# schmidtjonathan/pnmol-experiments

Measured on AMD Instinct MI355X. Metric: filter steps/sec, 1D heat N=512 nu=2 (white-noise EK1 predict+update), higher is better.
Workload: dtype f64; 1 GPU; 1-D heat equation, N=512 mesh, IWP(nu=2) EK1, Dirichlet, dt=2^-7, one problem per GPU (kappa sweep), D=1536, m=514; steps_in_one_call=4975, valid=True, problems_per_gpu=1

## Files before the change

### include/pnmol_hip.h

```cpp
#ifndef PNMOL_HIP_H
#define PNMOL_HIP_H

#ifdef __cplusplus
extern "C" {
#endif

typedef struct pnmol_ctx pnmol_ctx;
typedef struct pnmol_filter pnmol_filter;
typedef struct pnmol_state pnmol_state;
typedef struct pnmol_samples pnmol_samples;
typedef struct pnmol_bridge pnmol_bridge;

int pnmol_abi_version(void);
int pnmol_device_count(int* count);
int pnmol_ctx_create(int device, pnmol_ctx** out);
int pnmol_ctx_destroy(pnmol_ctx* ctx);
int pnmol_ctx_synchronize(pnmol_ctx* ctx);
const char* pnmol_last_error(pnmol_ctx* ctx);

int pnmol_fd_solve_batched(pnmol_ctx* ctx, const double* gram_nss, const double* lk_ns, const double* llk_n, int N, int s,
                           double* weights_ns, double* uncertainty_n);
int pnmol_cholesky_lower(pnmol_ctx* ctx, const double* A_nn, int n, double* L_nn);

typedef struct pnmol_filter_desc {
    int d;
    int num_derivatives;
    int nB;
    const double* L;
    const double* B;
    const double* E_sqrtm;
    const double* R_sqrtm;
    const double* Gamma;
    int d_state;
    int dtype;
    const double* K;
} pnmol_filter_desc;

int pnmol_filter_create(pnmol_ctx* ctx, const pnmol_filter_desc* desc, pnmol_filter** out);
int pnmol_filter_destroy(pnmol_filter* f);
int pnmol_filter_sweep_layout(const pnmol_filter* f, int* kernel, int* xcd_home);

int pnmol_filter_set_error_model(pnmol_filter* f, double dt, const double* Sq_inv,
                                 const double* Sq_diag);
int pnmol_filter_prepare_error_model(pnmol_filter* f, double dt);

int pnmol_filter_predict_mean(pnmol_filter* f, const pnmol_state* in, double dt, double* m_at_d);
int pnmol_filter_set_operator(pnmol_filter* f, const double* M_dds, const double* shift_d);
int pnmol_filter_set_operator_diagonal(pnmol_filter* f, const double* jdiag_d, const double* shift_d);

int pnmol_state_create(pnmol_filter* f, pnmol_state** out);
int pnmol_state_destroy(pnmol_state* s);
int pnmol_state_clone(const pnmol_state* s, pnmol_state** out);
int pnmol_state_set(pnmol_state* s, double t, const double* mean_nd, const double* cov_DD);
int pnmol_state_set_sqrtm(pnmol_state* s, double t, const double* mean_nd, const double* cov_sqrtm_DD);
int pnmol_state_get_time(const pnmol_state* s, double* t);
int pnmol_state_get_mean(const pnmol_state* s, double* mean_nd);
int pnmol_state_get_cov(const pnmol_state* s, double* cov_DD);
int pnmol_state_get_cov_sqrtm(const pnmol_state* s, double* C_DD);
int pnmol_state_get_marginal_var(const pnmol_state* s, double* var_nd);

typedef struct pnmol_step_out {
    double t_new;
    double diffusion_squared_local;
    double sigma2_whitened;
    double error_sigma2;
    int info;
} pnmol_step_out;

int pnmol_filter_step(pnmol_filter* f, const pnmol_state* in, double dt, pnmol_state* out,
                      pnmol_step_out* info, double* error_estimate_d);

int pnmol_smoother_step(pnmol_filter* f, const pnmol_state* filt_k, const pnmol_state* smooth_next, double dt,
                        pnmol_state* out);

typedef struct pnmol_observe_out {
    double log_likelihood;
    double mahalanobis;
    double logdet;
    int info;
} pnmol_observe_out;
int pnmol_state_observe(pnmol_filter* f, const pnmol_state* in, int q, const double* C_q_ds, const double* y_q,
                        const double* R_sqrtm_qq, pnmol_state* out, pnmol_observe_out* res);

int pnmol_state_predict(pnmol_filter* f, const pnmol_state* in, double dt, pnmol_state* out);
int pnmol_state_predict_marginals(pnmol_filter* f, const pnmol_state* in, int nq, const double* dt_q, double* means_qnd,
                                  double* stds_qnd);
int pnmol_smoother_step_bridge(pnmol_filter* f, const pnmol_state* filt_k, const pnmol_state* smooth_next, double dt,
                               pnmol_state* out, int keep_full, pnmol_bridge** bridge);
int pnmol_bridge_destroy(pnmol_bridge* b);
int pnmol_bridge_get_interval(const pnmol_bridge* b, double* t, double* dt, int* has_full);
int pnmol_bridge_eval(const pnmol_bridge* b, int nq, const double* t_q, double* means_qnd, double* stds_qnd);
int pnmol_bridge_state(const pnmol_bridge* b, const pnmol_state* smooth_k, const pnmol_state* smooth_next, double t,
                       pnmol_state* out);

int pnmol_samples_create(pnmol_filter* f, int num_samples, pnmol_samples** out);
int pnmol_samples_destroy(pnmol_samples* x);
int pnmol_samples_draw(pnmol_samples* x, const pnmol_state* s, const double* xi_SD, unsigned long long seed,
                       unsigned long long step_index, double scale);
int pnmol_samples_step_back(pnmol_samples* x, const pnmol_state* filt_k, double dt, const double* xi_S2D,
                            unsigned long long seed, unsigned long long step_index, double scale);
int pnmol_samples_interpolate(pnmol_samples* out, const pnmol_samples* left, const pnmol_samples* right, double t,
                              const double* xi_SD, unsigned long long seed, unsigned long long step_index, double scale);
int pnmol_samples_clone(const pnmol_samples* x, pnmol_samples** out);
int pnmol_samples_get(const pnmol_samples* x, double* x_Snd);
int pnmol_samples_get_time(const pnmol_samples* x, double* t);
int pnmol_sample_noise(pnmol_ctx* ctx, unsigned long long seed, unsigned long long step_index, int rows, int cols, double* out);

int pnmol_filter_steps(pnmol_filter* f, pnmol_state* s, int k, double dt, double* means_kd,
                       double* stds_kd, pnmol_step_out* info_k);

int pnmol_filter_steps_begin(pnmol_filter* f, pnmol_state* s, int k, double dt);
int pnmol_filter_steps_end(pnmol_filter* f, pnmol_state* s, double* means_kd, double* stds_kd,
                           pnmol_step_out* info_k);

int pnmol_filter_prepare_steps(pnmol_filter* f, pnmol_state* s, int k, double dt);

int pnmol_filter_last_steps_ms(pnmol_filter* f, float* ms);

int pnmol_filter_debug_read(pnmol_filter* f, int which, double* dst, long count);
int pnmol_filter_debug_poison(pnmol_filter* f);
int pnmol_filter_dims(const pnmol_filter* f, int* d, int* n, int* m, int* dp, int* mp);

#ifdef __cplusplus
}
#endif
#endif
```

### pnmol-experiments_amd/csrc/pnmol_hip.hip

```cpp
#include <hip/hip_runtime.h>

#include <algorithm>
#include <chrono>
#include <cmath>
#include <cstdio>
#include <cstdlib>
#include <cstring>
#include <string>
#include <utility>
#include <atomic>
#include <vector>

#include "pnmol_hip.h"
#include "pnmol_internal.hpp"

namespace {

constexpr int TLD = NB + 1;
typedef double d4 __attribute__((ext_vector_type(4)));

struct MeasModel {
    const int* ell_col;
    const double* ell_val;
    int w, d, m, dp, mp;
// ... 760 lines not shown
    for (int s = 0; s < NB / 4; ++s) {
        const double b = sI[(wc * 16 + fr) * TLD + 4 * s + fk];
        li = __builtin_amdgcn_mfma_f64_16x16x4f64(sA[(wr * 16 + fr) * TLD + 4 * s + fk], b, li, 0, 0, 0);
        if (trailing) lk = __builtin_amdgcn_mfma_f64_16x16x4f64(sB[(wr * 16 + fr) * TLD + 4 * s + fk], b, lk, 0, 0, 0);
    }
    __syncthreads();
#pragma unroll
    for (int r = 0; r < 4; ++r) {
        const int row = wr * 16 + fk + 4 * r, col = wc * 16 + fr;
        sA[row * TLD + col] = li[r];
        if (trailing) sB[row * TLD + col] = lk[r];
        if (c == 0) F[((long)I * NB + row) * ld + (long)j * NB + col] = li[r];
    }
    if (!trailing) return;
    __syncthreads();

#pragma unroll
    for (int s = 0; s < NB / 4; ++s)
        acc = __builtin_amdgcn_mfma_f64_16x16x4f64(-sA[(wr * 16 + fr) * TLD + 4 * s + fk],
                                                   sB[(wc * 16 + fr) * TLD + 4 * s + fk], acc, 0, 0, 0);
    if (!(blockIdx.x == 0 && c == 0)) {
#pragma unroll
        for (int r = 0; r < 4; ++r) gt[(long)(wr * 16 + fk + 4 * r) * ld + wc * 16 + fr] = acc[r];
        return;
    }
    __syncthreads();
#pragma unroll
    for (int r = 0; r < 4; ++r) sA[(wr * 16 + fk + 4 * r) * TLD + wc * 16 + fr] = acc[r];
    if (tid < NB) dlp->flag[tid] = 0;
    __syncthreads();
    if (w < 2)
        diag2w_from_lds(sA, F + ((long)(j + 1) * NB) * ld + (long)(j + 1) * NB, ld, Linv + (long)(j + 1) * NB * NB, w, l,
                        info_base + (*ctr - 1), (j + 1) * NB, sdiag + (j + 1) * NB, sdiag[ld], dlp);
}

constexpr int SWEEP_SPIN_LIMIT = 1 << 18;
#ifdef PNMOL_SWEEP_STAMP
__device__ long long pnmol_sweep_stamp[512][8];
#define SWEEP_STAMP(slot) do { if (tid == 0 && L.stamp_id < 256) pnmol_sweep_stamp[L.stamp_id][slot] = wall_clock64(); } while (0)
#define SWEEP_STAMP_L(slot) do { if (l == 0 && L.stamp_id < 256) pnmol_sweep_stamp[L.stamp_id][slot] = wall_clock64(); } while (0)
#ifndef PNMOL_SWEEP_TRACE_WG
#define PNMOL_SWEEP_TRACE_WG 16
#endif
#define SWEEP_TRACE(j, slot) do { if (tid == 0 && L.stamp_id == PNMOL_SWEEP_TRACE_WG) pnmol_sweep_stamp[256 + (j)][slot] = wall_clock64(); } while (0)
#define SWEEP_TRACE_W2(j, slot) do { if (w == 2 && l == 0 && L.stamp_id == PNMOL_SWEEP_TRACE_WG) pnmol_sweep_stamp[320 + (j)][slot] = wall_clock64(); } while (0)
#define SWEEP_TRACE_VM(j, slot) do { asm volatile("s_waitcnt vmcnt(0)" ::: "memory"); SWEEP_TRACE(j, slot); } while (0)
#define CHAIN_TRACE(J, slot) do { if (tid == 0) pnmol_sweep_stamp[384 + (J)][slot] = wall_clock64(); } while (0)
#define CHAIN_TRACE_W(J, slot, wave) do { if (l == 0 && w == (wave)) pnmol_sweep_stamp[384 + (J)][slot] = wall_clock64(); } while (0)
#define CHAIN_TRACE_CLK(J, slot) do { if (tid == 0) pnmol_sweep_stamp[384 + (J)][slot] = clock64(); } while (0)
#define PNMOL_DD_DBG 1
#define DD_TRACE(j, slot) do { if (tid == 0 && pair == 60) pnmol_sweep_stamp[448 + (j)][slot] = wall_clock64(); } while (0)
#else
#define DD_TRACE(j, slot) do {} while (0)
#define CHAIN_TRACE_CLK(J, slot) do {} while (0)
#define SWEEP_TRACE_VM(j, slot) do {} while (0)
#define SWEEP_TRACE_W2(j, slot) do {} while (0)
#define CHAIN_TRACE(J, slot) do {} while (0)
#define CHAIN_TRACE_W(J, slot, wave) do {} while (0)
#define SWEEP_TRACE(j, slot) do {} while (0)
#define SWEEP_STAMP(slot) do {} while (0)
#define SWEEP_STAMP_L(slot) do {} while (0)
#endif

struct SweepLds {
    double sS[2][NB * TLD];
    double sX[NB * TLD];
    double sP[4][NB * TLD];
    double sd[NB];
    double red[4];
    int seen[3];
    int dead, pub;
    int pubcnt;
    int rdiag, rnew, rcol, rzb;
    int stamp_id;
    Diag4Lds d4;
};
struct ChainLds {
    double sX[NB * TLD];
    double sLinv[NB * TLD];
    double sFeedS[NB * TLD];
    double sFeedD[NB * TLD];
    double sd[2][NB];
    double red[4];
    Diag4Lds d4[2];
};

__device__ __forceinline__ int flag_ld(const int* p) {
    return __hip_atomic_load(p, __ATOMIC_RELAXED, __HIP_MEMORY_SCOPE_AGENT);
}
__device__ __forceinline__ void flag_st(int* p, int v) {
    __hip_atomic_store(p, v, __ATOMIC_RELAXED, __HIP_MEMORY_SCOPE_AGENT);
}
__device__ __forceinline__ void wt_st(double* p, double v) {
    __hip_atomic_store(p, v, __ATOMIC_RELAXED, __HIP_MEMORY_SCOPE_AGENT);
}
typedef int v4i_t __attribute__((ext_vector_type(4)));
__device__ __forceinline__ __amdgpu_buffer_rsrc_t wt_rsrc(const void* base) {
    return __builtin_amdgcn_make_buffer_rsrc(const_cast<void*>(base), 0, 0x7ffffffc, 0x00020000);
}
template <int AUX = 16 >
__device__ __forceinline__ void wt_st2(__amdgpu_buffer_rsrc_t r, unsigned byte_off, double a, double b) {
    const v4i_t v = {__double2loint(a), __double2hiint(a), __double2loint(b), __double2hiint(b)};
    __builtin_amdgcn_raw_buffer_store_b128(v, r, byte_off, 0, AUX);
}
template <int NE, int AUX = 16>
__device__ __forceinline__ void wt_rows_from_lds(__amdgpu_buffer_rsrc_t r, unsigned org, long ld, const double* s, int row0, int l) {
#pragma unroll
    for (int e = 0; e < NE; ++e) {
        const int idx = l + 64 * e, row = row0 + (idx >> 4), c2 = 2 * (idx & 15);
        wt_st2<AUX>(r, org + (unsigned)((row * ld + c2) * 8), s[row * TLD + c2], s[row * TLD + c2 + 1]);
    }
}
struct TileRegs {
    double v[16];
};
__device__ __forceinline__ void tile_regs_from_lds(TileRegs& t, const double* s, int l) {
#pragma unroll
    for (int e = 0; e < 8; ++e) {
        const int idx = l + 64 * e, row = idx >> 4, c2 = 2 * (idx & 15);
        t.v[2 * e] = s[row * TLD + c2];
        t.v[2 * e + 1] = s[row * TLD + c2 + 1];
    }
}
template <int AUX>
__device__ __forceinline__ void tile_regs_store(const TileRegs& t, __amdgpu_buffer_rsrc_t r, unsigned org, long ld, int l) {
#pragma unroll
    for (int e = 0; e < 8; ++e) {
        const int idx = l + 64 * e, row = idx >> 4, c2 = 2 * (idx & 15);
        wt_st2<AUX>(r, org + (unsigned)((row * ld + c2) * 8), t.v[2 * e], t.v[2 * e + 1]);
    }
}
__device__ __forceinline__ void l2_flag_st(__amdgpu_buffer_rsrc_t rflags, int word, int v) {
    __builtin_amdgcn_raw_buffer_store_b32(v, rflags, (unsigned)word * 4u, 0, 0);
}
__device__ __forceinline__ void sc1_tile_to_lds(double* s, __amdgpu_buffer_rsrc_t r, unsigned org, int l) {
    v4i_t v[8];
#pragma unroll
    for (int e = 0; e < 8; ++e) {
        const int idx = l + 64 * e;
        v[e] = __builtin_amdgcn_raw_buffer_load_b128(r, org + (unsigned)(((idx >> 4) * NB + 2 * (idx & 15)) * 8), 0, 16 );
    }
#pragma unroll
    for (int e = 0; e < 8; ++e) {
        const int idx = l + 64 * e, row = idx >> 4, c2 = 2 * (idx & 15);
        s[row * TLD + c2] = __hiloint2double(v[e][1], v[e][0]);
        s[row * TLD + c2 + 1] = __hiloint2double(v[e][3], v[e][2]);
    }
}
__device__ __forceinline__ void drain_vmem() { asm volatile("s_waitcnt vmcnt(0) lgkmcnt(0)" ::: "memory"); }

struct SweepSeen {
    int rowj, rown, diag;
};

__device__ __forceinline__ void sweep_wait(SweepLds* L, const int* frow, const int* fdiag, int* fabort, int j, int jn_ok,
                                           int need_rowj, int need_rown, bool need_diag, SweepSeen& sn, int tid) {
    if (sn.rowj >= need_rowj && sn.rown >= need_rown && (!need_diag || sn.diag)) return;
    __syncthreads();
    if (tid == 0) {
        int r = sn.rowj, rn = sn.rown, d = sn.diag;
        if (!L->dead) {
            for (int spins = 0;; ++spins) {
                r = flag_ld(frow + j);
                rn = jn_ok ? flag_ld(frow + j + 1) : (1 << 30);
                d = flag_ld(fdiag + j);
                if (r >= need_rowj && rn >= need_rown && (!need_diag || d)) break;
// ... 127 lines not shown
        for (int o = 32; o > 0; o >>= 1) {
            a[q] += __shfl_xor(a[q], o);
            b[q] += __shfl_xor(b[q], o);
        }
        const long row = r0 + q;
        if (l == 0 && row < r1) {
            if (row < Dp) {
                va.mout[row] = va.mpred[row] - a[q];
            } else if (row < Dp + mp) {
                const long k = row - Dp;
                va.part[k] = va.r[k] * va.r[k];
                va.part[mp + k] = a[q] * a[q];
                va.part[2 * mp + k] = va.z[k] * b[q];
            }
        }
    }
}

__device__ __forceinline__ void ksplit_partial(double* sp, const double* __restrict__ Abase, const double* __restrict__ Bbase,
                                               int k0, int k1, long ld, int w, int l) {
    const int fr = l & 15, fk = l >> 4;
    d4 p00 = {0, 0, 0, 0}, p01 = p00, p10 = p00, p11 = p00;
    FragTile a0, b0, a1, b1;
    auto mfma32 = [&](const FragTile& a, const FragTile& b) {
#pragma unroll
        for (int s = 0; s < 8; ++s) {
            p00 = __builtin_amdgcn_mfma_f64_16x16x4f64(a.lo.v[s], b.lo.v[s], p00, 0, 0, 0);
            p01 = __builtin_amdgcn_mfma_f64_16x16x4f64(a.lo.v[s], b.hi.v[s], p01, 0, 0, 0);
            p10 = __builtin_amdgcn_mfma_f64_16x16x4f64(a.hi.v[s], b.lo.v[s], p10, 0, 0, 0);
            p11 = __builtin_amdgcn_mfma_f64_16x16x4f64(a.hi.v[s], b.hi.v[s], p11, 0, 0, 0);
        }
    };
    const int nk = (k0 + w < k1) ? (k1 - k0 - w + 3) >> 2 : 0;
    if (nk > 0) {
        tile_ld(a0, Abase + (long)(k0 + w) * NB, ld);
        tile_ld(b0, Bbase + (long)(k0 + w) * NB, ld);
    }
    int t = 0;
    for (; t + 2 <= nk; t += 2) {
        const long ka = k0 + w + 4 * (t + 1), kb = k0 + w + 4 * (t + 2 < nk ? t + 2 : nk - 1);
        tile_ld(a1, Abase + ka * NB, ld);
        tile_ld(b1, Bbase + ka * NB, ld);
        mfma32(a0, b0);
        tile_ld(a0, Abase + kb * NB, ld);
        tile_ld(b0, Bbase + kb * NB, ld);
        mfma32(a1, b1);
    }
    if (t < nk) mfma32(a0, b0);
#pragma unroll
    for (int r = 0; r < 4; ++r) {
        sp[(fk + 4 * r) * TLD + fr] = p00[r];
        sp[(fk + 4 * r) * TLD + 16 + fr] = p01[r];
        sp[(16 + fk + 4 * r) * TLD + fr] = p10[r];
        sp[(16 + fk + 4 * r) * TLD + 16 + fr] = p11[r];
    }
}

constexpr int HELP_KMAX = 8;
__device__ __forceinline__ int helper_share(int H, int t, int CB) {
    const int h = CB - 1 - H;
    if (h >= H - 1 || t < h + 3) return 0;
    const int kh = t - 1 - HELP_KMAX;
    return kh > 0 ? kh : 0;
}

__device__ __forceinline__ void vecops_rows4(const VecArgs& va, const double* __restrict__ W, int mp, long Dp, long r0,
                                             long r1, int l) {
    vecops_rowsR<4>(va, W, mp, Dp, r0, r1, l);
}

struct DowndateArgs {
    const void* Ppred;
    void* Pout;
    double* var;
    int dp;
    int vrows;
    VecArgs va;
    void* Pnext;
    const double* Kg;
    const int* last_ctr;
    double A1[MAXN * MAXN], Q1[MAXN * MAXN];
    int p32;
    int last_ksteps;
};

template <typename PT>
struct AccOf;
template <>
struct AccOf<double> {
    typedef d4 type;
    static __device__ __forceinline__ d4 mfma_neg(double a, double b, d4 c) {
        return __builtin_amdgcn_mfma_f64_16x16x4f64(-a, b, c, 0, 0, 0);
    }
    static __device__ __forceinline__ int row(int fk, int r) { return fk + 4 * r; }
};
template <>
struct AccOf<float> {
    typedef float type __attribute__((ext_vector_type(4)));
    static __device__ __forceinline__ type mfma_neg(double a, double b, type c) {
        return __builtin_amdgcn_mfma_f32_16x16x4f32(-(float)a, (float)b, c, 0, 0, 0);
    }
    static __device__ __forceinline__ int row(int fk, int r) { return 4 * fk + r; }
};

#ifdef PNMOL_DD_DBG
__device__ __forceinline__ void pnmol_dd_avail_dbg(int j, int avail, bool loaded) { pnmol_sweep_stamp[448 + j][3] = avail; pnmol_sweep_stamp[448 + j][4] = loaded; }
#else
__device__ __forceinline__ void pnmol_dd_avail_dbg(int, int, bool) {}
#endif
template <int N, typename PT, bool SHORT_LAST>
__device__ __forceinline__ void sweep_downdate_body(SweepLds& L, const DowndateArgs& dd, const double* F, int ld, int CB,
                                                    int RBS, const int* frow, int* fabort, int* info, int pair, int tid,
                                                    int l, int w, int slot) {
    const int fr = l & 15, fk = l >> 4, qr = w >> 1, qc = w & 1;
    const int T32 = dd.dp / NB;
    int J = (int)((sqrt(8.0 * pair + 1.0) - 1.0) * 0.5);
    while ((J + 1) * (J + 2) / 2 <= pair) ++J;
    while (J * (J + 1) / 2 > pair) --J;
    const int K = pair - J * (J + 1) / 2;
    const long Dp = (long)N * dd.dp;
    const double* W = F + (long)ld * ld;
    typedef typename AccOf<PT>::type acc_t;
    const PT* Ppred = static_cast<const PT*>(dd.Ppred);
    acc_t acc[N][N];
#pragma unroll
    for (int a = 0; a < N; ++a)
#pragma unroll
        for (int b = 0; b < N; ++b)
#pragma unroll
            for (int r = 0; r < 4; ++r)
                acc[a][b][r] = Ppred[((long)a * dd.dp + J * NB + qr * 16 + AccOf<PT>::row(fk, r)) * Dp + (long)b * dd.dp + K * NB + qc * 16 + fr];
    acc_t kjk = {0, 0, 0, 0};
    if (dd.Pnext) {
#pragma unroll
        for (int r = 0; r < 4; ++r) kjk[r] = (PT)dd.Kg[(long)(J * NB + qr * 16 + AccOf<PT>::row(fk, r)) * dd.dp + K * NB + qc * 16 + fr];
    }
    int avail = 0;
    auto wait_for = [&](int j) {
        if (j < avail) return;
        __syncthreads();
        if (w == 0) {
            int mn = 0;
            if (!L.dead) {
                for (int spins = 0;; ++spins) {
                    int v = 1 << 30;
                    if (l < 2 * N) {
                        const int a = l >> 1, tile = (l & 1) ? K : J;
                        v = flag_ld(frow + RBS + a * T32 + tile);
                    }
#pragma unroll
                    for (int o = 32; o > 0; o >>= 1) v = min(v, __shfl_xor(v, o));
                    mn = v;
                    if (mn > j) break;
                    if (spins > SWEEP_SPIN_LIMIT || flag_ld(fabort)) {
                        if (l == 0) {
                            L.dead = 1;
                            flag_st(fabort, 1);
                        }
                        mn = 1 << 30;
                        break;
                    }
                    __builtin_amdgcn_s_sleep(4);
                }
            } else {
                mn = 1 << 30;
            }
            if (l == 0) L.seen[0] = mn;
        }
        __syncthreads();
        avail = L.seen[0];
    };
    auto load_panel = [&](int j, Frag8 (&fa)[N], Frag8 (&fb)[N]) {
#pragma unroll
        for (int a = 0; a < N; ++a) {
            frag_ld(fa[a], W + ((long)a * dd.dp + J * NB + qr * 16 + fr) * ld + (long)j * NB + 8 * fk);
            frag_ld(fb[a], W + ((long)a * dd.dp + K * NB + qc * 16 + fr) * ld + (long)j * NB + 8 * fk);
        }
    };
    auto panel = [&](int j, bool loaded, Frag8 (&fa)[N], Frag8 (&fb)[N], Frag8 (&na)[N], Frag8 (&nb)[N]) {
        DD_TRACE(j, 0);
        if (!loaded) {
            wait_for(j);
            DD_TRACE(j, 1);
            load_panel(j, fa, fb);
        }
        const bool next = j + 1 < CB && j + 1 < avail;
        if (next) load_panel(j + 1, na, nb);
        const int smax = (SHORT_LAST && j + 1 == CB && dd.last_ksteps > 0) ? dd.last_ksteps : 8;
#pragma unroll
        for (int s = 0; s < 8; ++s)
            if (!SHORT_LAST || s < smax) {
#pragma unroll
                for (int a = 0; a < N; ++a)
#pragma unroll
                    for (int b = 0; b < N; ++b)
                        acc[a][b] = AccOf<PT>::mfma_neg(fa[a].v[s], fb[b].v[s], acc[a][b]);
            }
        DD_TRACE(j, 2);
#ifdef PNMOL_SWEEP_STAMP
        if (tid == 0 && pair == 60) pnmol_dd_avail_dbg(j, avail, loaded);
#endif
        return next;
    };
    if constexpr (SHORT_LAST) {
        (void)panel;
        (void)wait_for;
        bool wdead = false;
        int* relay = &L.seen[0];
        auto poll_min = [&]() {
            int v = 1 << 30;
            if (l < 2 * N) {
                const int a = l >> 1, tile = (l & 1) ? K : J;
                v = flag_ld(frow + RBS + a * T32 + tile);
            }
            return v;
        };
        auto reduce_min = [&](int v) {
#pragma unroll
            for (int o = 32; o > 0; o >>= 1) v = min(v, __shfl_xor(v, o));
            return v;
        };
        auto publish = [&](int v) {
            if (l == 0) __hip_atomic_store(relay, v, __ATOMIC_RELAXED, __HIP_MEMORY_SCOPE_WORKGROUP);
        };
        auto known = [&]() { return __hip_atomic_load(relay, __ATOMIC_RELAXED, __HIP_MEMORY_SCOPE_WORKGROUP); };
        auto wave_wait = [&](int j) {
            if (wdead) return;
            if (w == 0) {
                for (int spins = 0;; ++spins) {
                    const int v = reduce_min(poll_min());
                    if (v > j) {
                        publish(v);
                        return;
                    }
                    if (spins > SWEEP_SPIN_LIMIT || ((spins & 63) == 63 && flag_ld(fabort))) {
                        wdead = true;
                        flag_st(fabort, 1);
                        publish(1 << 30);
                        return;
                    }
                    __builtin_amdgcn_s_sleep(4);
                }
            } else {
                int v;
                while ((v = known()) <= j) __builtin_amdgcn_s_sleep(2);
                if (v == (1 << 30)) wdead = true;
            }
        };
        auto block = [&](int j, bool have, Frag8 (&fa)[N], Frag8 (&fb)[N], Frag8 (&na)[N], Frag8 (&nb)[N]) {
            DD_TRACE(j, 0);
            if (!have) {
                wave_wait(j);
                DD_TRACE(j, 1);
                load_panel(j, fa, fb);
            }
            const int pv = (w == 0 && j + 1 < CB) ? poll_min() : 0;
            const int smax = (j + 1 == CB && dd.last_ksteps > 0) ? dd.last_ksteps : 8;
            bool next = false;
#pragma unroll
            for (int s = 0; s < 8; ++s) {
                if (s == 2) {
                    if (w == 0 && j + 1 < CB && !wdead) {
                        const int v = reduce_min(pv);
                        if (v > known()) publish(v);
                    }
                    const int kv = known();
                    next = (j + 1 < CB) && !wdead && kv > j + 1 && kv != (1 << 30);
                    if (next) load_panel(j + 1, na, nb);
                }
                if (s < smax) {
#pragma unroll
                    for (int a = 0; a < N; ++a)
#pragma unroll
                        for (int b = 0; b < N; ++b)
                            acc[a][b] = AccOf<PT>::mfma_neg(fa[a].v[s], fb[b].v[s], acc[a][b]);
                }
            }
            DD_TRACE(j, 2);
            return next;
        };
        Frag8 fa0[N], fb0[N], fa1[N], fb1[N];
        bool have = false;
        for (int j = 0; j < CB; j += 2) {
            have = block(j, have, fa0, fb0, fa1, fb1);
            if (j + 1 < CB) have = block(j + 1, have, fa1, fb1, fa0, fb0);
        }
        if (wdead && l == 0) atomicMin(info, -2);
        __syncthreads();
    } else {
        for (int j = 0; j < CB; ++j) {
            wait_for(j);
            Frag8 fa[N], fb[N];
            load_panel(j, fa, fb);
#pragma unroll
            for (int s = 0; s < 8; ++s)
#pragma unroll
                for (int a = 0; a < N; ++a)
#pragma unroll
                    for (int b = 0; b < N; ++b)
                        acc[a][b] = AccOf<PT>::mfma_neg(fa[a].v[s], fb[b].v[s], acc[a][b]);
        }
    }
    SWEEP_STAMP(1);
    PT* stg = reinterpret_cast<PT*>(L.sP[w]);
    const bool write_p = dd.Pnext == nullptr || (slot + 1 == *dd.last_ctr);
    auto put_block = [&](PT* dst, const acc_t& v, long row0, long col0, bool mirror) {
#pragma unroll
        for (int r = 0; r < 4; ++r) {
            dst[(row0 + AccOf<PT>::row(fk, r)) * Dp + col0 + fr] = v[r];
            if (J != K && mirror) stg[AccOf<PT>::row(fk, r) * 17 + fr] = v[r];
        }
        if (J != K && mirror) {
            __builtin_amdgcn_wave_barrier();
#pragma unroll
            for (int r = 0; r < 4; ++r)
                dst[(col0 + fk + 4 * r) * Dp + row0 + fr] = stg[fr * 17 + fk + 4 * r];
            __builtin_amdgcn_wave_barrier();
        }
    };
#pragma unroll
    for (int a = 0; a < N; ++a) {
        const long row0 = (long)a * dd.dp + J * NB + qr * 16;
        if (J == K && qr == qc) {
#pragma unroll
            for (int r = 0; r < 4; ++r)
                if (AccOf<PT>::row(fk, r) == fr) dd.var[row0 + fr] = acc[a][a][r];
        }
        if (write_p) {
#pragma unroll
            for (int b = 0; b < N; ++b) put_block(static_cast<PT*>(dd.Pout), acc[a][b], row0, (long)b * dd.dp + K * NB + qc * 16, true);
        }
    }
    if (dd.Pnext) {
        acc_t T[N][N];
#pragma unroll
        for (int a = 0; a < N; ++a)
#pragma unroll
            for (int e = 0; e < N; ++e) {
                acc_t t = {0, 0, 0, 0};
#pragma unroll
                for (int q = 0; q < N; ++q) t += (PT)dd.A1[a * MAXN + q] * acc[q][e];
                T[a][e] = t;
            }
#pragma unroll
        for (int a = 0; a < N; ++a)
#pragma unroll
            for (int b = 0; b < N; ++b) {
                acc_t pn = (PT)dd.Q1[a * MAXN + b] * kjk;
#pragma unroll
                for (int e = 0; e < N; ++e) pn += T[a][e] * (PT)dd.A1[b * MAXN + e];
                put_block(static_cast<PT*>(dd.Pnext), pn, (long)a * dd.dp + J * NB + qr * 16, (long)b * dd.dp + K * NB + qc * 16, a < 2);
            }
    }
    SWEEP_STAMP(2);
    {
        const int RBW = (int)(Dp / NB);
        const long row_lo = (long)pair * dd.vrows, row_hi = min(row_lo + dd.vrows, Dp + (long)ld);
        __syncthreads();
        if (tid == 0 && !L.dead && row_lo < row_hi) {
            for (long rb = row_lo / NB; rb <= (row_hi - 1) / NB; ++rb) {
                const int need = rb < RBW ? RBS + (int)rb : RBS + RBW + 1 + (int)(rb - RBW);
                for (int spins = 0;; ++spins) {
                    if (flag_ld(frow + need) >= CB && flag_ld(frow + RBS + RBW) >= CB) break;
                    if (spins > SWEEP_SPIN_LIMIT || flag_ld(fabort)) {
                        L.dead = 1;
                        flag_st(fabort, 1);
                        break;
                    }
                    __builtin_amdgcn_s_sleep(2);
                }
                if (L.dead) break;
            }
        }
        __syncthreads();
        for (long rg = row_lo + 4 * w; rg < row_hi; rg += 16) vecops_rows4(dd.va, W, ld, Dp, rg, min(rg + 4, row_hi), l);
    }
    if (tid == 0 && L.dead) atomicMin(info, -2);
    SWEEP_STAMP(5);
}

template <int N, bool SHORT_LAST = false>
__device__ __forceinline__ void sweep_downdate_role(SweepLds& L, const DowndateArgs& dd, const double* F, int ld, int CB,
                                                    int RBS, const int* frow, int* fabort, int* info, int pair, int tid,
                                                    int l, int w, int slot) {
    if (dd.p32) sweep_downdate_body<N, float, SHORT_LAST>(L, dd, F, ld, CB, RBS, frow, fabort, info, pair, tid, l, w, slot);
    else sweep_downdate_body<N, double, SHORT_LAST>(L, dd, F, ld, CB, RBS, frow, fabort, info, pair, tid, l, w, slot);
}

template <int N, bool FUSED, bool CHAINHELP = FUSED>
__global__ __launch_bounds__(256) void k_sweep(const double* __restrict__ G, double* F, double* Linv, int ld, int CB,
                                               int RT, int* flags, int* info_base, const int* __restrict__ ctr,
                                               DowndateArgs dd, int* claim, double* hs_scratch, int lenient, int wskip) {
    __shared__ __attribute__((aligned(16))) SweepLds L;
    const int tid = threadIdx.x, l = tid & 63, w = __builtin_amdgcn_readfirstlane(tid >> 6);
    const int wr = w >> 1, wc = w & 1, fr = l & 15, fk = l >> 4;
    int I = blockIdx.x;
#ifdef PNMOL_SWEEP_STAMP
    if (tid == 0) L.stamp_id = blockIdx.x;
#endif
    {
        const int zb = RT - CB - 1;
        if (wskip) {
            if (I >= CB) I = zb + (I - CB);
        } else if (I >= CB && I <= zb) {
            I = (I == CB) ? zb : I - 1;
        }
    }
    const bool chain = I < CB;
    int* frow = flags;
    int* fdiag = flags + RT;
    int* fabort = flags + RT + CB;
    int* info = info_base + (*ctr - 1);
    if constexpr (FUSED) {
        if (I >= RT) {
            if (tid == 0) {
                L.dead = 0;
                __builtin_amdgcn_fence(__ATOMIC_ACQUIRE, "agent");
            }
            __syncthreads();
            SWEEP_STAMP(0);
            sweep_downdate_role<N>(L, dd, F, ld, CB, CB, frow, fabort, info, I - RT, tid, l, w, *ctr - 1);
            return;
        }
    }

    double smax = 0.0;
    if (chain) {
        for (int e = tid; e < ld; e += 256) smax = fmax(smax, fabs(G[(long)e * ld + e]));
#pragma unroll
        for (int o = 32; o > 0; o >>= 1) smax = fmax(smax, __shfl_xor(smax, o));
        if (l == 0) L.red[w] = smax;
        if (tid < NB) L.sd[tid] = G[(long)(I * NB + tid) * ld + I * NB + tid];
    }
    if (tid < 16) L.d4.flagA[tid] = 0;
    if (tid == 0) {
        L.dead = 0, L.pub = 0;
        __builtin_amdgcn_fence(__ATOMIC_ACQUIRE, "agent");
    }
    __syncthreads();
    SWEEP_STAMP(0);
    if (chain) smax = fmax(fmax(L.red[0], L.red[1]), fmax(L.red[2], L.red[3]));
    if (lenient) smax = __builtin_inf();

    const long rowC = (long)I * NB + wr * 16 + fk;
    const int colC = wc * 16 + fr;
    const int offC = (wr * 16 + fk) * TLD + colC;
    const double* Xown = F + ((long)I * NB + fr) * ld + 8 * fk;
    d4 accD = {0, 0, 0, 0};
    if (chain) {
#pragma unroll
        for (int r = 0; r < 4; ++r) {
            const int rl = wr * 16 + fk + 4 * r, cl = colC;
            accD[r] = -G[((long)I * NB + (rl >= cl ? rl : cl)) * ld + (long)I * NB + (rl >= cl ? cl : rl)];
        }
    }

    const int nsteps = chain ? I : CB;
    d4 gnext = {0, 0, 0, 0};
    if (nsteps > 0) {
#pragma unroll
        for (int r = 0; r < 4; ++r) gnext[r] = G[(rowC + 4 * r) * ld + colC];
    }
    SweepSeen sn{0, 0, 0};
    for (int j = 0; j < nsteps; ++j) {
        const int jn_ok = (j + 1 < CB);
        d4 acc = gnext;
        SWEEP_TRACE(j, 0);
        if (j >= 2) {
#pragma unroll
// ... 117 lines not shown
            }
        }
        if (tid == 0 && L.dead) atomicMin(info, -2);
        SWEEP_STAMP(5);
        return;
    }

    SWEEP_STAMP(3);
    if (w == 2 && I > 0) {
        drain_vmem();
        if (l == 0) flag_st(frow + I, I);
        __hip_atomic_store(&L.pub, 1, __ATOMIC_RELAXED, __HIP_MEMORY_SCOPE_WORKGROUP);
    }
    diag4_factor<true>(accD, &L.d4, w, l, F + ((long)I * NB) * ld + (long)I * NB, ld, Linv + (long)I * NB * NB, info, I * NB,
                       L.sd, smax, nullptr, pivot_tolerance(lenient));
    if (w == 1) {
        drain_vmem();
        if (I > 0) {
            int spins = 0;
            while (__hip_atomic_load(&L.pub, __ATOMIC_RELAXED, __HIP_MEMORY_SCOPE_WORKGROUP) == 0 && ++spins < (1 << 24))
                __builtin_amdgcn_s_sleep(1);
        }
        if (l == 0) flag_st(fdiag + I, 1);
        SWEEP_STAMP_L(4);
    }
    if (tid == 0 && L.dead) atomicMin(info, -2);
    if constexpr (CHAINHELP) {
        const int H = CB - 1 - I;
        if (I < H - 1) {
            const double* Xh = F + ((long)H * NB + fr) * ld + 8 * fk;
            for (int t = I + 3; t < H; ++t) {
                const int kh = helper_share(H, t, CB);
                if (kh <= 0) continue;
                int* cl = claim + (long)H * CB + t;
                __syncthreads();
                if (tid == 0) {
                    int got = 0;
                    for (int spins = 0;; ++spins) {
                        if (flag_ld(cl) != 0) break;
                        if (flag_ld(frow + H) >= kh && flag_ld(frow + t) >= kh) {
                            got = atomicCAS(cl, 0, 1) == 0;
                            break;
                        }
                        if (spins > 4096 || flag_ld(fabort)) {
                            got = -1;
                            break;
                        }
                        __builtin_amdgcn_s_sleep(8);
                    }
                    L.seen[0] = got;
                }
                __syncthreads();
                const int got = L.seen[0];
                if (got < 0) break;
                if (got == 0) continue;
                ksplit_partial(L.sP[w], Xh, F + ((long)t * NB + fr) * ld + 8 * fk, 0, kh, ld, w, l);
                __syncthreads();
                double* hs = hs_scratch + ((long)H * CB + t) * NB * NB;
#pragma unroll
                for (int r = 0; r < 4; ++r)
                    wt_st(&hs[(wr * 16 + fk + 4 * r) * NB + colC],
                          (L.sP[0][offC + 4 * r * TLD] + L.sP[1][offC + 4 * r * TLD]) +
                              (L.sP[2][offC + 4 * r * TLD] + L.sP[3][offC + 4 * r * TLD]));
                drain_vmem();
                __syncthreads();
                if (tid == 0) flag_st(cl, 2);
            }
        }
    }
}

constexpr int RL_REP = 8;
constexpr int S_SPLIT_FROM = 11, S_SPLIT_H = 9;
__host__ __device__ inline int s_split_count(int CB, bool xl) { return (xl && CB > S_SPLIT_FROM) ? CB - S_SPLIT_FROM : 0; }
constexpr int W_SPLIT_H = 11;
#ifndef PNMOL_W_SPLIT
#define PNMOL_W_SPLIT 0
#endif
__host__ __device__ inline int w_split_count(int RT, int CB) {
    const int RBW = RT - 2 * CB - 1;
    return (PNMOL_W_SPLIT && RBW > 0 && CB > W_SPLIT_H + 1) ? RBW : 0;
}
struct RlFlags {
    int frow, fabort, fxcc, ffeed, fdiag, fnew, fcol, fdiagL, fnewL, frowL, CBp, total;
};
__host__ __device__ inline RlFlags rl_flags(int RT, int CB) {
    const int RTp = (RT + 31) / 32 * 32, CBp = (CB + 31) / 32 * 32;
    RlFlags f;
    f.CBp = CBp;
    f.frow = 0;
    f.fabort = RTp;
    f.fxcc = RTp + 16;
    f.ffeed = RTp + 32;
    f.fdiag = f.ffeed + CBp;
    f.fnew = f.fdiag + RL_REP * CBp;
    f.fcol = f.fnew + RL_REP * CBp;
    f.fdiagL = f.fcol + RL_REP * CBp;
    f.fnewL = f.fdiagL + CBp;
    f.frowL = f.fnewL + CBp;
    f.total = f.frowL + CBp;
    return f;
}
__device__ __forceinline__ int xcc_id() { return __builtin_amdgcn_s_getreg((3 << 11) | 20) & 15; }
struct WaveWait {
    bool dead;
};
__device__ __forceinline__ void wave_wait_ge(const int* p, int need, int* fabort, WaveWait& ww) {
    if (ww.dead) return;
    for (int spins = 0;; ++spins) {
        if (flag_ld(p) >= need) return;
        if (spins > SWEEP_SPIN_LIMIT || ((spins & 63) == 63 && flag_ld(fabort))) {
            ww.dead = true;
            flag_st(fabort, 1);
            return;
        }
        __builtin_amdgcn_s_sleep(1);
    }
}
__device__ __forceinline__ void relay_wait_ge(const int* p, int need, int* relay, int tag, int* fabort, WaveWait& ww, int w) {
    if (w == 0) {
        wave_wait_ge(p, need, fabort, ww);
        __hip_atomic_store(relay, ww.dead ? (1 << 30) : tag, __ATOMIC_RELAXED, __HIP_MEMORY_SCOPE_WORKGROUP);
    } else {
        int v;
        while ((v = __hip_atomic_load(relay, __ATOMIC_RELAXED, __HIP_MEMORY_SCOPE_WORKGROUP)) < tag) __builtin_amdgcn_s_sleep(1);
        if (v == (1 << 30)) ww.dead = true;
    }
    asm volatile("" ::: "memory");
}

template <class Need>
__device__ __forceinline__ void relay_progress(const int* p, int cnt, Need need, int want, int& known, int* relay, int* fabort,
                                               WaveWait& ww, int w, int l) {
    if (w == 0) {
        if (known < want) {
            for (int spins = 0; !ww.dead; ++spins) {
                const int v = l < cnt ? flag_ld(p + l) : 0;
                const unsigned long long ok = __ballot(l < cnt && v >= need(l));
                known = __builtin_amdgcn_readfirstlane((int)__builtin_ctzll(~ok));
                if (known >= want) break;
                if (spins > SWEEP_SPIN_LIMIT || ((spins & 63) == 63 && flag_ld(fabort))) {
                    ww.dead = true;
                    flag_st(fabort, 1);
                    break;
                }
                __builtin_amdgcn_s_sleep(1);
            }
            __hip_atomic_store(relay, ww.dead ? (1 << 30) : known, __ATOMIC_RELAXED, __HIP_MEMORY_SCOPE_WORKGROUP);
        }
    } else {
        int v;
        while ((v = __hip_atomic_load(relay, __ATOMIC_RELAXED, __HIP_MEMORY_SCOPE_WORKGROUP)) < want) __builtin_amdgcn_s_sleep(1);
        if (v == (1 << 30)) ww.dead = true;
    }
    asm volatile("" ::: "memory");
}
__device__ __forceinline__ void relay_progress_min(const int* p, int cnt, int want, int& known, int* relay, int* fabort,
                                                   WaveWait& ww, int w, int l) {
    if (w == 0) {
        if (known < want) {
            for (int spins = 0; !ww.dead; ++spins) {
                int v = l < cnt ? flag_ld(p + l) : (1 << 29);
#pragma unroll
                for (int o = 32; o > 0; o >>= 1) v = min(v, __shfl_xor(v, o));
                known = __builtin_amdgcn_readfirstlane(v);
                if (known >= want) break;
                if (spins > SWEEP_SPIN_LIMIT || ((spins & 63) == 63 && flag_ld(fabort))) {
                    ww.dead = true;
                    flag_st(fabort, 1);
                    break;
                }
                __builtin_amdgcn_s_sleep(1);
            }
            __hip_atomic_store(relay, ww.dead ? (1 << 30) : known, __ATOMIC_RELAXED, __HIP_MEMORY_SCOPE_WORKGROUP);
        }
    } else {
        int v;
        while ((v = __hip_atomic_load(relay, __ATOMIC_RELAXED, __HIP_MEMORY_SCOPE_WORKGROUP)) < want) __builtin_amdgcn_s_sleep(1);
        if (v == (1 << 30)) ww.dead = true;
    }
    asm volatile("" ::: "memory");
}
__device__ __forceinline__ void relay_wait_range_ge(const int* p, int cnt, int need, int* relay, int tag, int* fabort,
                                                    WaveWait& ww, int w, int l) {
    if (w == 0) {
        if (!ww.dead) {
            for (int spins = 0;; ++spins) {
                const int v = l < cnt ? flag_ld(p + l) : need;
                if (__all(v >= need)) break;
                if (spins > SWEEP_SPIN_LIMIT || ((spins & 63) == 63 && flag_ld(fabort))) {
                    ww.dead = true;
                    flag_st(fabort, 1);
                    break;
                }
                __builtin_amdgcn_s_sleep(1);
            }
        }
        __hip_atomic_store(relay, ww.dead ? (1 << 30) : tag, __ATOMIC_RELAXED, __HIP_MEMORY_SCOPE_WORKGROUP);
    } else {
        int v;
        while ((v = __hip_atomic_load(relay, __ATOMIC_RELAXED, __HIP_MEMORY_SCOPE_WORKGROUP)) < tag) __builtin_amdgcn_s_sleep(1);
        if (v == (1 << 30)) ww.dead = true;
    }
    asm volatile("" ::: "memory");
}

__device__ __forceinline__ void rows8_dot(const double* __restrict__ base, long row0, int mp, const double* __restrict__ vec,
                                          double (&out)[8], int l) {
#pragma unroll
    for (int q = 0; q < 8; ++q) out[q] = 0.0;
    for (int i0 = l; i0 < mp; i0 += 256) {
        double wv[8][4], xv[4];
#pragma unroll
        for (int t = 0; t < 4; ++t) {
            const int i = i0 + 64 * t;
            const int ii = i < mp ? i : mp - 1;
            xv[t] = i < mp ? vec[ii] : 0.0;
#pragma unroll
            for (int q = 0; q < 8; ++q) wv[q][t] = base[(row0 + q) * mp + ii];
        }
#pragma unroll
        for (int t = 0; t < 4; ++t)
#pragma unroll
            for (int q = 0; q < 8; ++q) out[q] += wv[q][t] * xv[t];
    }
#pragma unroll
    for (int q = 0; q < 8; ++q)
#pragma unroll
        for (int o = 32; o > 0; o >>= 1) out[q] += __shfl_xor(out[q], o);
}
__device__ __forceinline__ void vecops_rows8(const VecArgs& va, const double* __restrict__ W, int mp, long Dp, long r0,
                                             const double* bq , int l) {
    double a[8];
    if (r0 < Dp) {
        rows8_dot(W, r0, mp, va.r, a, l);
        if (l < 8) {
            double mine = a[0];
#pragma unroll
            for (int q = 1; q < 8; ++q) mine = (l == q) ? a[q] : mine;
            va.mout[r0 + l] = va.mpred[r0 + l] - mine;
        }
    } else {
        const long k0 = r0 - Dp;
        rows8_dot(va.LinvT, k0, mp, va.z, a, l);
        if (l < 8) {
            double mine = a[0];
#pragma unroll
            for (int q = 1; q < 8; ++q) mine = (l == q) ? a[q] : mine;
            const double bm = bq[l];
            const long k = k0 + l;
            va.part[k] = va.r[k] * va.r[k];
            va.part[mp + k] = mine * mine;
            va.part[2 * mp + k] = va.z[k] * bm;
        }
    }
}
__device__ __forceinline__ void mfma_result_guard() {
#ifdef PNMOL_NO_MFMA_GUARD
    return;
#endif
    __builtin_amdgcn_sched_barrier(0);
    asm volatile("s_nop 15\n\ts_nop 7" ::: "memory");
    __builtin_amdgcn_sched_barrier(0);
}
constexpr int RING = 3;
constexpr int RING_LINV = RING, RING_NEWEST = RING + 1;
__device__ __forceinline__ void lds_dma16(const double* gsrc, unsigned lds_dst) {
    unsigned keep;
    asm volatile("s_mov_b32 %0, m0\n\ts_mov_b32 m0, %2\n\ts_nop 0\n\tglobal_load_lds_dwordx4 %1, off\n\ts_mov_b32 m0, %0"
                 : "=&s"(keep) : "v"(gsrc), "s"(lds_dst) : "memory");
}
__device__ __forceinline__ void ring_fill(const double* tile, const int (&off)[4], unsigned slot) {
#pragma unroll
    for (int c = 0; c < 4; ++c) lds_dma16(tile + off[c], slot + 1024u * c);
}
__device__ __forceinline__ void ring_wait(int tiles_behind) {
    switch (tiles_behind) {
        case 0: asm volatile("s_waitcnt vmcnt(0)" ::: "memory"); break;
        case 1: asm volatile("s_waitcnt vmcnt(4)" ::: "memory"); break;
        case 2: asm volatile("s_waitcnt vmcnt(8)" ::: "memory"); break;
        default: asm volatile("s_waitcnt vmcnt(12)" ::: "memory"); break;
    }
}
__device__ __forceinline__ void ring_frag(Frag8& f, const double* slot, int fr, int fk) {
#pragma unroll
    for (int e = 0; e < 4; ++e) {
        const double2 t = *reinterpret_cast<const double2*>(slot + (fr * 16 + ((4 * fk + e) ^ fr)) * 2);
        f.v[2 * e] = t.x;
        f.v[2 * e + 1] = t.y;
    }
}

template <bool XL>
__device__ __forceinline__ void sweep_chain_role(ChainLds& C, const double* __restrict__ G, double* F, double* Linv, int ld,
                                                 int CB, int* flags, const RlFlags& fl, int* info,
                                                 double* feed, int lenient, int tid, int l, int w) {
    int* fdiag_all = flags + fl.fdiag;
    int* fnew_all = flags + fl.fnew;
    const int CBp = fl.CBp;
    int* ffeed = flags + fl.ffeed;
    int* fabort = flags + fl.fabort;
    const int wr = w >> 1, wc = w & 1, fr = l & 15, fk = l >> 4;
    const int offC = (wr * 16 + fk) * TLD + wc * 16 + fr;
    const __amdgpu_buffer_rsrc_t rF = wt_rsrc(F), rlinv = wt_rsrc(Linv), rfeed = wt_rsrc(feed), rflags = wt_rsrc(flags);
    if (XL && tid == 0) flag_st(flags + fl.fxcc, 1 + xcc_id());
    WaveWait ww{false};
    double smax = 0.0;
    for (int e = tid; e < ld; e += 256) smax = fmax(smax, fabs(G[(long)e * ld + e]));
#pragma unroll
    for (int o = 32; o > 0; o >>= 1) smax = fmax(smax, __shfl_xor(smax, o));
    if (l == 0) C.red[w] = smax;
    if (tid < NB) C.sd[0][tid] = G[(long)tid * ld + tid];
    if (tid < 16) C.d4[0].flagA[tid] = 0, C.d4[1].flagA[tid] = 0;
    for (int e = tid; e < 16 * 16; e += 256) C.sLinv[(e >> 4) * TLD + 16 + (e & 15)] = 0.0;
    if (tid == 0) __builtin_amdgcn_fence(__ATOMIC_ACQUIRE, "agent");
    __syncthreads();
    smax = lenient ? __builtin_inf() : fmax(fmax(C.red[0], C.red[1]), fmax(C.red[2], C.red[3]));
    const double pivtol = pivot_tolerance(lenient);
    d4 accD;
#pragma unroll
    for (int r = 0; r < 4; ++r) {
        const int rl = wr * 16 + fk + 4 * r, cl = wc * 16 + fr;
        accD[r] = -G[(long)(rl >= cl ? rl : cl) * ld + (rl >= cl ? cl : rl)];
    }
    for (int J = 0; J < CB; ++J) {
        Diag4Lds* dl = &C.d4[J & 1];
        CHAIN_TRACE(J, 0);
        CHAIN_TRACE_CLK(J, 4);
        if (w == 2 && J > 0)
            diag4_output(&C.d4[(J - 1) & 1], l, F + ((long)(J - 1) * NB) * ld + (long)(J - 1) * NB, ld, info, (J - 1) * NB,
                         C.sd[(J - 1) & 1], smax, pivtol);
        diag4_factor<true, true, false, false>(accD, dl, w, l, F + ((long)J * NB) * ld + (long)J * NB, ld,
                                               Linv + (long)J * NB * NB, info, J * NB, C.sd[J & 1], smax, C.sLinv, pivtol);
        CHAIN_TRACE_W(J, 1, 3);
        CHAIN_TRACE_W(J, 6, 1);
        if (XL && w == 1 && J + 1 < CB) {
            TileRegs t1;
            tile_regs_from_lds(t1, C.sLinv, l);
            tile_regs_store<0>(t1, rlinv, (unsigned)(J * NB * NB * 8), NB, l);
            drain_vmem();
            if (l == 0) l2_flag_st(rflags, fl.fdiagL + J, 1);
        }
        if (J + 1 == CB) {
            __syncthreads();
            if (w == 2) {
                wt_rows_from_lds<8>(rlinv, (unsigned)(J * NB * NB * 8), NB, C.sLinv, 0, l);
                drain_vmem();
                if (l < RL_REP) flag_st(fdiag_all + l * CBp + J, 1);
                if (XL && l == 0) l2_flag_st(rflags, fl.fdiagL + J, 1);
            }
            break;
        }
        if (w == 0 || w == 2) {
            wave_wait_ge(ffeed + J + 1, 1, fabort, ww);
            sc1_tile_to_lds((w == 2) ? C.sFeedD : C.sFeedS, rfeed, (unsigned)((2 * (J + 1) + (w == 2 ? 1 : 0)) * NB * NB * 8), l);
            if (w == 2 && l < NB) C.sd[(J + 1) & 1][l] = G[(long)((J + 1) * NB + l) * ld + (J + 1) * NB + l];
        }
        __syncthreads();
        CHAIN_TRACE(J, 2);
        if (tid < 16) C.d4[(J + 1) & 1].flagA[tid] = 0;
        TileRegs tl;
        if (w == 2) {
            if constexpr (XL) {
                tile_regs_from_lds(tl, C.sLinv, l);
            } else {
                wt_rows_from_lds<8>(rlinv, (unsigned)(J * NB * NB * 8), NB, C.sLinv, 0, l);
            }
        }
        d4 x = {0, 0, 0, 0};
#pragma unroll
        for (int s = 0; s < 8; ++s)
            x = __builtin_amdgcn_mfma_f64_16x16x4f64(C.sFeedS[(wr * 16 + fr) * TLD + 8 * fk + s],
                                                     C.sLinv[(wc * 16 + fr) * TLD + 8 * fk + s], x, 0, 0, 0);
#pragma unroll
        for (int r = 0; r < 4; ++r) C.sX[offC + 4 * r * TLD] = x[r];
#pragma unroll
        for (int r = 0; r < 4; ++r) accD[r] = C.sFeedD[offC + 4 * r * TLD];
        __syncthreads();
        CHAIN_TRACE(J, 3);
        if (w == 2) {
            if constexpr (!XL) {
                drain_vmem();
                if (l < RL_REP) flag_st(fdiag_all + l * CBp + J, 1);
            }
        }
#pragma unroll
        for (int s = 0; s < 8; ++s)
            accD = __builtin_amdgcn_mfma_f64_16x16x4f64(C.sX[(wr * 16 + fr) * TLD + 8 * fk + s],
                                                        C.sX[(wc * 16 + fr) * TLD + 8 * fk + s], accD, 0, 0, 0);
        if (w == 2) {
            const unsigned orgX = (unsigned)((((long)(J + 1) * NB) * ld + (long)J * NB) * 8);
            if constexpr (XL) {
                TileRegs tx;
                tile_regs_from_lds(tx, C.sX, l);
                tile_regs_store<0>(tx, rF, orgX, ld, l);
                drain_vmem();
                if (l == 0) l2_flag_st(rflags, fl.fnewL + J, 1);
                tile_regs_store<16>(tl, rlinv, (unsigned)(J * NB * NB * 8), NB, l);
                tile_regs_store<16>(tx, rF, orgX, ld, l);
                drain_vmem();
                if (l < RL_REP) flag_st(fdiag_all + l * CBp + J, 1);
                if (l < RL_REP) flag_st(fnew_all + l * CBp + J, 1);
            } else {
                wt_rows_from_lds<8>(rF, orgX, ld, C.sX, 0, l);
                drain_vmem();
                if (l < RL_REP) flag_st(fnew_all + l * CBp + J, 1);
            }
        }
    }
    if (w == 2)
        diag4_output(&C.d4[(CB - 1) & 1], l, F + ((long)(CB - 1) * NB) * ld + (long)(CB - 1) * NB, ld, info, (CB - 1) * NB,
                     C.sd[(CB - 1) & 1], smax, pivtol);
    if (l == 0 && ww.dead) atomicMin(info, -2);
}

template <int N, bool FUSED, int MAXT, bool XL>
__global__ __launch_bounds__(256) void k_sweep_rl(const double* __restrict__ G, double* F, double* Linv, int ld, int CB,
                                                  int RT, int* flags, int* info_base, const int* __restrict__ ctr,
                                                  DowndateArgs dd, double* feed, int lenient, int home) {
    __shared__ __attribute__((aligned(16))) union {
        SweepLds L;
        ChainLds C;
    } lds;
    SweepLds& L = lds.L;
    __shared__ __attribute__((aligned(16))) double bulk_ring[4][RING + 2][16 * NB];
    const int tid = threadIdx.x, l = tid & 63, w = __builtin_amdgcn_readfirstlane(tid >> 6);
    const int wr = w >> 1, wc = w & 1, fr = l & 15, fk = l >> 4;
    const RlFlags fl = rl_flags(RT, CB);
    int* frow = flags + fl.frow;
    int* fabort = flags + fl.fabort;
    int* ffeed = flags + fl.ffeed;
    const int* fdiag = flags + fl.fdiag + (blockIdx.x % RL_REP) * fl.CBp;
    const int* fnew = flags + fl.fnew + (blockIdx.x % RL_REP) * fl.CBp;
    const int* fcol = flags + fl.fcol + (blockIdx.x % RL_REP) * fl.CBp;
    int* info = info_base + (*ctr - 1);
    const int bx = XL ? (int)blockIdx.x - home : (int)blockIdx.x;
    if (bx < 0) return;
    if (bx == 0) {
        sweep_chain_role<XL>(lds.C, G, F, Linv, ld, CB, flags, fl, info, feed, lenient, tid, l, w);
        return;
    }
    int I, part = 0;
    if constexpr (XL) {
        const int nsplit = s_split_count(CB, true);
        const int b = bx, nslot = 8 * (CB - 1 + nsplit) + 1;
        if (b < nslot) {
            if (b % 8 != 0) return;
            const int sidx = b / 8;
            if (sidx < CB) {
                I = sidx;
                part = (nsplit > 0 && I >= S_SPLIT_FROM) ? 1 : 0;
            } else {
                I = S_SPLIT_FROM + (sidx - CB);
                part = 2;
            }
        } else {
            if (b % 8 == 0) return;
            const int q = b - nslot;
            I = CB + q - (q + 1) / 8;
        }
    } else {
        I = bx - 1;
    }
#ifdef PNMOL_SWEEP_STAMP
    if (tid == 0) L.stamp_id = part == 1 ? 200 + I : 1 + I;
#endif
    {
        const int zb = RT - CB - 1;
        if (I >= CB && I <= zb) I = (I == CB) ? zb : I - 1;
    }
    const int nwsplit = w_split_count(RT, CB);
    if (I >= RT && I < RT + nwsplit) {
        I = CB + (I - RT);
        part = 2;
    } else if (I >= RT) {
        I -= nwsplit;
        if constexpr (FUSED) {
            if (tid == 0) {
                L.dead = 0, L.seen[0] = 0;
                __builtin_amdgcn_fence(__ATOMIC_ACQUIRE, "agent");
            }
            __syncthreads();
            SWEEP_STAMP(0);
            sweep_downdate_role<N, true>(L, dd, F, ld, CB, CB, frow, fabort, info, I - RT, tid, l, w, *ctr - 1);
        }
        return;
    } else if (nwsplit > 0 && I >= CB && I < RT - CB - 1) {
        part = 1;
    }
    const bool chain = I < CB;
    if (chain && I == 0) return;
    if (tid == 0) {
        L.dead = 0, L.pub = 0, L.pubcnt = part == 2 ? 4 * (I < CB ? S_SPLIT_H : W_SPLIT_H) : 0, L.rdiag = 0, L.rnew = 0, L.rcol = 0, L.rzb = 0;
        L.seen[0] = 0;
        __builtin_amdgcn_fence(__ATOMIC_ACQUIRE, "agent");
    }
    __syncthreads();
    SWEEP_STAMP(0);

    const long rowC = (long)I * NB + wr * 16 + fk;
    const int colC = wc * 16 + fr;
    const int offC = (wr * 16 + fk) * TLD + colC;
    const bool feeds = chain && part != 1;
    const int hsplit = chain ? S_SPLIT_H : W_SPLIT_H;
    const int t0 = part == 2 ? hsplit : 0;
    const int last = part == 1 ? hsplit - 1 : (chain ? I - 2 : CB - 1);
    const int ntiles = part == 1 ? hsplit : (chain ? I : CB);
    d4 n[MAXT];
#pragma unroll
    for (int t = 0; t < MAXT; ++t)
        if (t0 + t < ntiles) {
#pragma unroll
            for (int r = 0; r < 4; ++r) n[t][r] = -G[(rowC + 4 * r) * ld + (long)(t0 + t) * NB + colC];
        }
    d4 accD = {0, 0, 0, 0};
    if (feeds) {
#pragma unroll
        for (int r = 0; r < 4; ++r) {
            const int rl = wr * 16 + fk + 4 * r, cl = colC;
            accD[r] = -G[((long)I * NB + (rl >= cl ? rl : cl)) * ld + (long)I * NB + (rl >= cl ? cl : rl)];
        }
    }
    WaveWait ww{false};
    int known_diag = 0, known_new = 0, known_col = 0;
    const __amdgpu_buffer_rsrc_t rF = wt_rsrc(F), rfeed = wt_rsrc(feed), rflags = wt_rsrc(flags);
    const double* ringw = &bulk_ring[w][0][0];
    const unsigned ring0 = __builtin_amdgcn_readfirstlane((unsigned)(size_t)ringw);
    int roff[4], roffL[4];
#pragma unroll
    for (int c = 0; c < 4; ++c) {
        const int row = 4 * c + (l >> 4);
        roff[c] = (wc * 16 + row) * ld + 2 * ((l & 15) ^ row);
        roffL[c] = (wc * 16 + row) * NB + 2 * ((l & 15) ^ row);
    }
#ifndef PNMOL_EAGER_TILES
#define PNMOL_EAGER_TILES 6
#endif
    constexpr int EAGER_TILES = PNMOL_EAGER_TILES;
    bool pre_b0 = false;
    if constexpr (FUSED) {
        const int RBW = RT - 2 * CB - 1, zb = CB + RBW;
        if (!chain && I > zb) {
            double bq[8] = {0, 0, 0, 0, 0, 0, 0, 0};
            if (dd.va.Sqinv != nullptr) rows8_dot(dd.va.Sqinv, (long)(I - zb - 1) * NB + 8 * w, ld, dd.va.z, bq, l);
            if (l == 0) {
#pragma unroll
                for (int q = 0; q < 8; ++q) L.sd[8 * w + q] = bq[q];
            }
        }
    }
    bool local = false;
    if constexpr (XL) {
        if (chain) {
            if (tid == 0) {
                int v = 0;
                for (int spins = 0; spins < 4096 && (v = flag_ld(flags + fl.fxcc)) == 0; ++spins) __builtin_amdgcn_s_sleep(1);
                L.seen[0] = (v == 1 + xcc_id());
            }
            __syncthreads();
            local = L.seen[0] != 0;
            if (local) fdiag = flags + fl.fdiagL, fnew = flags + fl.fnewL;
        }
    }
    Frag8 ax;
    auto flag_tile = [&](int t) {
        drain_vmem();
        int lastw = 0;
        if (l == 0) lastw = __hip_atomic_fetch_add(&L.pubcnt, 1, __ATOMIC_RELAXED, __HIP_MEMORY_SCOPE_WORKGROUP) == 4 * t + 3;
        if (__builtin_amdgcn_readfirstlane(lastw)) {
            if (l == 0) flag_st(frow + I, t + 1);
            if (XL && chain && l == 0) {
                if (local) l2_flag_st(rflags, fl.frowL + I, t + 1);
                else flag_st(flags + fl.frowL + I, t + 1);
            }
            if (chain && l < RL_REP)
                __hip_atomic_fetch_add(flags + fl.fcol + l * fl.CBp + t, 1, __ATOMIC_RELAXED, __HIP_MEMORY_SCOPE_AGENT);
        }
    };
    if (part == 2) {
        const int* fsrc = (XL && local) ? flags + fl.frowL : frow;
        for (int k = 0; k < t0; ++k) {
            if (chain) {
                if (k + 1 < t0) {
                    relay_progress_min(fsrc + t0, I - t0 + 1, k + 1, known_col, &L.rcol, fabort, ww, w, l);
                } else {
                    relay_progress(fnew, CB - 1, [](int) { return 1; }, t0, known_new, &L.rnew, fabort, ww, w, l);
                    relay_progress_min(fsrc + t0 + 1, I - t0, t0, known_col, &L.rcol, fabort, ww, w, l);
                }
            } else {
                relay_progress(fnew, CB - 1, [](int) { return 1; }, k + 1, known_new, &L.rnew, fabort, ww, w, l);
                relay_progress(fcol, CB - 1, [CB](int q) { return CB - 2 - q; }, k + 1, known_col, &L.rcol, fabort, ww, w, l);
                relay_wait_ge(frow + I, k + 1, &L.rzb, k + 1, fabort, ww, w);
            }
            Frag8 bx;
            frag_ld(ax, F + ((long)I * NB + wr * 16 + fr) * ld + (long)k * NB + 8 * fk);
            frag_ld(bx, F + ((long)I * NB + wc * 16 + fr) * ld + (long)k * NB + 8 * fk);
#pragma unroll
            for (int u0 = 0; u0 < 8; u0 += 4) {
                Frag8 b[4];
#pragma unroll
                for (int q = 0; q < 4; ++q)
                    if (t0 + u0 + q < ntiles)
                        frag_ld(b[q], F + ((long)(t0 + u0 + q) * NB + wc * 16 + fr) * ld + (long)k * NB + 8 * fk);
#pragma unroll
                for (int q = 0; q < 4; ++q)
                    if (t0 + u0 + q < ntiles) {
#pragma unroll
                        for (int s = 0; s < 8; ++s)
                            n[u0 + q] = __builtin_amdgcn_mfma_f64_16x16x4f64(ax.v[s], b[q].v[s], n[u0 + q], 0, 0, 0);
                    }
            }
            if (chain) {
#pragma unroll
                for (int s = 0; s < 8; ++s) accD = __builtin_amdgcn_mfma_f64_16x16x4f64(ax.v[s], bx.v[s], accD, 0, 0, 0);
            }
            mfma_result_guard();
        }
    }
    const bool lastlocal = feeds && XL && local;
#pragma unroll
    for (int r = 0; r < 4; ++r) L.sS[t0 & 1][offC + 4 * r * TLD] = -n[0][r];
    __syncthreads();
    bool pre_l = false;
    for (int j = t0; j <= last; ++j) {
        const double* sS = L.sS[j & 1];
        SWEEP_TRACE(j, 0);
        relay_progress(fdiag, CB, [](int) { return 1; }, j + 1, known_diag, &L.rdiag, fabort, ww, w, l);
        SWEEP_TRACE(j, 5);
        Frag8 bl;
        if (pre_l) {
            ring_wait(0);
            ring_frag(bl, ringw + 512 * RING_LINV, fr, fk);
        } else {
            frag_ld(bl, Linv + (long)j * NB * NB + (wc * 16 + fr) * NB + 8 * fk);
        }
        d4 x = {0, 0, 0, 0};
#pragma unroll
        for (int s = 0; s < 8; ++s)
            x = __builtin_amdgcn_mfma_f64_16x16x4f64(sS[(wr * 16 + fr) * TLD + 8 * fk + s], bl.v[s], x, 0, 0, 0);
        double* sXj = (j & 1) ? L.sP[0] : L.sX;
#pragma unroll
        for (int r = 0; r < 4; ++r) sXj[offC + 4 * r * TLD] = x[r];
        __syncthreads();
        SWEEP_TRACE(j, 3);
        const bool llast = lastlocal && j == last;
        const unsigned orgX = (unsigned)((((long)I * NB) * ld + (long)j * NB) * 8);
        if (llast) wt_rows_from_lds<2, 0>(rF, orgX, ld, sXj, 8 * w, l);
        else wt_rows_from_lds<2>(rF, orgX, ld, sXj, 8 * w, l);
        if (feeds) {
#pragma unroll
            for (int s = 0; s < 8; ++s)
                accD = __builtin_amdgcn_mfma_f64_16x16x4f64(sXj[(wr * 16 + fr) * TLD + 8 * fk + s],
                                                            sXj[(wc * 16 + fr) * TLD + 8 * fk + s], accD, 0, 0, 0);
            mfma_result_guard();
        }
        const int cnt = ntiles - 1 - j;
        pre_l = false;
        if (cnt > 0) {
#pragma unroll
            for (int s = 0; s < 8; ++s) ax.v[s] = sXj[(wr * 16 + fr) * TLD + 8 * fk + s];
            relay_progress(fnew, CB - 1, [](int) { return 1; }, j + 1, known_new, &L.rnew, fabort, ww, w, l);
            if (llast) {
                drain_vmem();
                int lastw = 0;
                if (l == 0) lastw = __hip_atomic_fetch_add(&L.pub, 1, __ATOMIC_RELAXED, __HIP_MEMORY_SCOPE_WORKGROUP) == 3;
                if (__builtin_amdgcn_readfirstlane(lastw) && l == 0) l2_flag_st(rflags, fl.frowL + I, j + 1);
            } else if (chain) {
                flag_tile(j);
            }
            if (chain) {
                if (cnt > 1)
                    relay_progress_min((XL && local ? flags + fl.frowL : frow) + j + 2, cnt - 1, j + 1, known_col, &L.rcol, fabort, ww, w, l);
            } else {
                relay_progress(fcol, CB - 1, [CB](int k) { return CB - 2 - k; }, j + 1, known_col, &L.rcol, fabort, ww, w, l);
            }
            SWEEP_TRACE(j, 1);
            const double* Lt = F + (long)j * NB + (long)(j + 1) * NB * ld;
#pragma unroll
            for (int r = 0; r < RING; ++r)
                if (r < cnt) ring_fill(Lt + (long)r * NB * ld, roff, ring0 + 4096u * r);
            if (!chain) {
                const int seen = __builtin_amdgcn_readfirstlane(__hip_atomic_load(&L.rdiag, __ATOMIC_RELAXED, __HIP_MEMORY_SCOPE_WORKGROUP));
                if (seen >= j + 2 && seen != (1 << 30)) {
                    ring_fill(Linv + (long)(j + 1) * NB * NB, roffL, ring0 + 4096u * RING_LINV);
                    pre_l = true;
                }
            }
            if (!chain) flag_tile(j);
            else ring_wait(0);
            Frag8 b[2];
            ring_frag(b[0], ringw, fr, fk);
#pragma unroll
            for (int u = 1; u < MAXT; ++u) {
                if (u <= cnt) {
                    const int k = u - 1;
                    __builtin_amdgcn_s_waitcnt(0xc07f);
                    asm volatile("" ::: "memory");
                    if (k + RING < cnt) ring_fill(Lt + (long)(k + RING) * NB * ld, roff, ring0 + 4096u * (k % RING));
                    d4 a = __builtin_amdgcn_mfma_f64_16x16x4f64(ax.v[0], b[k & 1].v[0], n[u], 0, 0, 0);
                    __builtin_amdgcn_sched_barrier(0);
                    if (k + 1 < cnt) {
                        const int behind = (k + RING < cnt ? k + RING : cnt - 1) - (k + 1);
                        ring_wait(behind < RING - 1 ? behind : RING - 1);
                        ring_frag(b[(k + 1) & 1], ringw + 512 * ((k + 1) % RING), fr, fk);
                    }
                    __builtin_amdgcn_sched_barrier(0);
#pragma unroll
                    for (int s = 1; s < 8; ++s)
                        a = __builtin_amdgcn_mfma_f64_16x16x4f64(ax.v[s], b[k & 1].v[s], a, 0, 0, 0);
                    n[u - 1] = a;
                } else {
                    mfma_result_guard();
                    break;
                }
            }
            mfma_result_guard();
            SWEEP_TRACE(j, 4);
            if (!(feeds && j == last)) {
#pragma unroll
                for (int r = 0; r < 4; ++r) L.sS[(j + 1) & 1][offC + 4 * r * TLD] = -n[0][r];
                __syncthreads();
            }
        }
        SWEEP_TRACE(j, 6);
    }
    if (feeds) {
        const int j = I - 1;
#pragma unroll
        for (int r = 0; r < 4; ++r) {
            L.sS[0][offC + 4 * r * TLD] = -n[0][r];
            L.sS[1][offC + 4 * r * TLD] = accD[r];
        }
        __syncthreads();
        if (XL && local) {
            wt_rows_from_lds<2, 0>(rfeed, (unsigned)((2 * I) * NB * NB * 8), NB, L.sS[0], 8 * w, l);
            wt_rows_from_lds<2, 0>(rfeed, (unsigned)((2 * I + 1) * NB * NB * 8), NB, L.sS[1], 8 * w, l);
        } else {
            wt_rows_from_lds<2>(rfeed, (unsigned)((2 * I) * NB * NB * 8), NB, L.sS[0], 8 * w, l);
            wt_rows_from_lds<2>(rfeed, (unsigned)((2 * I + 1) * NB * NB * 8), NB, L.sS[1], 8 * w, l);
        }
        SWEEP_TRACE(j, 2);
        drain_vmem();
        SWEEP_TRACE(j, 3);
        __syncthreads();
        if (tid == 0) {
            if (XL && local) l2_flag_st(rflags, fl.ffeed + I, 1);
            else flag_st(ffeed + I, 1);
        }
        SWEEP_TRACE(j, 4);
        SWEEP_STAMP(1);
        if (last >= 0 && lastlocal) {
            const double* sXl = (last & 1) ? L.sP[0] : L.sX;
            wt_rows_from_lds<2>(rF, (unsigned)((((long)I * NB) * ld + (long)last * NB) * 8), ld, sXl, 8 * w, l);
            flag_tile(last);
        }
    }
    if (!feeds) flag_tile(ntiles - 1);
    if (!chain) {
        if constexpr (FUSED) {
            const int RBW = RT - 2 * CB - 1, zb = CB + RBW;
            if (I != zb && part != 1) {
                __syncthreads();
                relay_wait_ge(frow + zb, CB, &L.rzb, 1 << 24, fabort, ww, w);
                const long Dp = (long)RBW * NB;
                const long row0 = (I < zb ? (long)(I - CB) * NB : Dp + (long)(I - zb - 1) * NB) + 8 * w;
                const double* W = F + (long)ld * ld;
                SWEEP_STAMP(2);
                vecops_rows8(dd.va, W, ld, Dp, row0, L.sd + 8 * w, l);
            }
        }
    }
    if (l == 0 && ww.dead) atomicMin(info, -2);
    SWEEP_STAMP(5);
}

template <int N>
struct DowndateCfg {
    static constexpr int CW = 8;
    static constexpr int SLD = CW + 1;
    static constexpr int STG = 2 * N * 16 * SLD;
    static constexpr int RED = N * N * 4 * 64;
    static constexpr int TLD16 = 17;
    static constexpr int LDS_D = (4 * STG > 2 * RED) ? 4 * STG : 2 * RED;
};

template <int N, int WV>
__device__ __forceinline__ void downdate_finish(d4 (&acc)[N][N], double* smem, const double* Ppred, double* Pout,
                                                double* __restrict__ var, int dp, long Dp, int J, int K, int l) {
    using C = DowndateCfg<N>;
    const int fr = l & 15, fk = l >> 4;
    double* wr = smem + (1 - WV) * C::RED;
#pragma unroll
    for (int a = 0; a < N; ++a)
#pragma unroll
        for (int b = 0; b < N; ++b)
#pragma unroll
            for (int q = 0; q < 2; ++q) wr[((a * N + b) * 2 + q) * 64 + l] = acc[a][b][(1 - WV) * 2 + q];
    __syncthreads();
    const double* rdo = smem + WV * C::RED;
    double x[N][N][2];
#pragma unroll
    for (int a = 0; a < N; ++a)
#pragma unroll
        for (int b = 0; b < N; ++b)
#pragma unroll
            for (int q = 0; q < 2; ++q) {
                const int row = fk + 4 * (WV * 2 + q);
                const long gi = ((long)a * dp + J * 16 + row) * Dp + (long)b * dp + K * 16 + fr;
                x[a][b][q] = Ppred[gi] - (acc[a][b][WV * 2 + q] + rdo[((a * N + b) * 2 + q) * 64 + l]);
                Pout[gi] = x[a][b][q];
                if (J == K && a == b && row == fr) var[a * dp + J * 16 + row] = x[a][b][q];
            }
    if (J == K) return;
    __syncthreads();
    double* tp = smem;
#pragma unroll
    for (int a = 0; a < N; ++a)
#pragma unroll
        for (int b = 0; b < N; ++b)
#pragma unroll
            for (int q = 0; q < 2; ++q) tp[((a * N + b) * 16 + fr) * C::TLD16 + fk + 4 * (WV * 2 + q)] = x[a][b][q];
    __syncthreads();
    const int cc = 8 * WV + (l >> 3), rr0 = (l & 7) * 2;
#pragma unroll
    for (int a = 0; a < N; ++a)
#pragma unroll
        for (int b = 0; b < N; ++b) {
            double2 v2;
            v2.x = tp[((a * N + b) * 16 + cc) * C::TLD16 + rr0];
            v2.y = tp[((a * N + b) * 16 + cc) * C::TLD16 + rr0 + 1];
            *reinterpret_cast<double2*>(Pout + ((long)b * dp + K * 16 + cc) * Dp + (long)a * dp + J * 16 + rr0) = v2;
        }
}

template <int N>
__global__ __launch_bounds__(256, (N <= 3 ? 4 : 1)) void k_downdate(const double* Ppred, const double* __restrict__ W, double* Pout,
                                                     double* __restrict__ var, int dp, int mp, int c_begin,
                                                     int c_end, VecArgs va) {
    using C = DowndateCfg<N>;
    __shared__ __attribute__((aligned(16))) double smem[C::LDS_D];
    static_assert(N * N * 16 * C::TLD16 <= C::LDS_D, "transpose staging must fit");
    const int tid = threadIdx.x, l = tid & 63, w = tid >> 6;
    const long Dp = (long)N * dp;
    if ((int)blockIdx.y >= dp / 16) {
        vecops_rows(va, W, mp, Dp, ((long)(blockIdx.y - dp / 16) * (dp / 16) + blockIdx.x) * 4 + w, l);
        return;
    }
    const int J = blockIdx.y, K = blockIdx.x;
    if (K > J) return;
    double* st = smem + w * C::STG;
    const int fr = l & 15, fk = l >> 4;
    const int lr = l >> 2, lc = (l & 3) * 2;

    d4 acc[N][N];
#pragma unroll
    for (int a = 0; a < N; ++a)
// ... 327 lines not shown
    __shared__ __attribute__((aligned(16))) double sA[2][BDK][BDT];
    __shared__ __attribute__((aligned(16))) double sB[2][BDK][BDT];
    const int tid = threadIdx.x, l = tid & 63, w = __builtin_amdgcn_readfirstlane(tid >> 6);
    const int wr = w >> 1, wc = w & 1, fr = l & 15, fk = l >> 4;
    const int t = (int)blockIdx.x;
    if (t >= nt) return;
    const int nJ = nt / nI, J = nJ - 1 - t / nI, I = t % nI;
    d4 acc[4][4];
#pragma unroll
    for (int ti = 0; ti < 4; ++ti)
#pragma unroll
        for (int tj = 0; tj < 4; ++tj) acc[ti][tj] = (d4){0, 0, 0, 0};
    const int lrow = tid >> 1, lk = (tid & 1) * 8;
    const int bk = tid >> 4, bj = (tid & 15) * 8;
    const double* ga = A + ((long)I * BDT + lrow) * ld + lk;
    const double* gb = T + (long)bk * ld + (long)J * BDT + bj;
    double2 ra[4], rb[4];
    auto fetch = [&](int slab) {
#pragma unroll
        for (int q = 0; q < 4; ++q) {
            ra[q] = *reinterpret_cast<const double2*>(ga + (long)slab * BDK + 2 * q);
            rb[q] = *reinterpret_cast<const double2*>(gb + (long)slab * BDK * ld + 2 * q);
        }
    };
    auto park = [&](int buf) {
#pragma unroll
        for (int q = 0; q < 4; ++q) {
            sA[buf][lk + 2 * q][lrow] = ra[q].x;
            sA[buf][lk + 2 * q + 1][lrow] = ra[q].y;
            *reinterpret_cast<double2*>(&sB[buf][bk][bj + 2 * q]) = rb[q];
        }
    };
    const int nslab = (J + 1) * BDT / BDK;
    fetch(0);
    park(0);
    __syncthreads();
    for (int sl = 0; sl < nslab; ++sl) {
        const int buf = sl & 1;
        if (sl + 1 < nslab) fetch(sl + 1);
#pragma unroll
        for (int ks = 0; ks < BDK / 4; ++ks) {
            double a[4], b[4];
#pragma unroll
            for (int q = 0; q < 4; ++q) {
                a[q] = sA[buf][4 * ks + fk][wr * 64 + 16 * q + fr];
                b[q] = sB[buf][4 * ks + fk][wc * 64 + 16 * q + fr];
            }
#pragma unroll
            for (int ti = 0; ti < 4; ++ti)
#pragma unroll
                for (int tj = 0; tj < 4; ++tj)
                    acc[ti][tj] = __builtin_amdgcn_mfma_f64_16x16x4f64(a[ti], b[tj], acc[ti][tj], 0, 0, 0);
        }
        if (sl + 1 < nslab) park(buf ^ 1);
        __syncthreads();
    }
    const long row0 = (long)I * BDT + wr * 64, col0 = (long)J * BDT + wc * 64;
#pragma unroll
    for (int ti = 0; ti < 4; ++ti)
#pragma unroll
        for (int tj = 0; tj < 4; ++tj)
#pragma unroll
            for (int r = 0; r < 4; ++r) C[(row0 + 16 * ti + fk + 4 * r) * ld + col0 + 16 * tj + fr] = acc[ti][tj][r];
}
__global__ __launch_bounds__(256) void k_vecops(VecArgs va, const double* __restrict__ W, int mp, long Dp, int per_row) {
    vecops_rows(va, W, mp, Dp, ((long)blockIdx.y * per_row + blockIdx.x) * 4 + (threadIdx.x >> 6), threadIdx.x & 63);
}

namespace {

void drop_graphs(pnmol_filter* f);

enum StepKind { STEP_FULL = 0, STEP_FIRST = 1, STEP_STEADY = 2 };

inline bool fused_loop(const pnmol_filter* f) { return f->sweep_mode == 2 && f->n <= 3 && f->fuse_predict != 0; }

inline bool sweep_rl_enabled() {
    static const int on = [] {
        const char* e = std::getenv("PNMOL_HIP_SWEEP_RL");
        return e ? std::atoi(e) : 1;
    }();
    return on != 0;
}
inline int sweep_xl_mode() {
    static const int mode = [] {
        const char* e = std::getenv("PNMOL_HIP_SWEEP_XL");
        return e ? (std::atoi(e) != 0 ? 1 : 0) : -1;
    }();
    return mode;
}
constexpr int MAX_DEVICES = 64;
std::atomic<int> live_rl_filters[MAX_DEVICES];
template <int N, bool FUSED>
void launch_sweep(unsigned grid, hipStream_t st, const double* G, double* F, double* Linv, int ld, int CB, int RT, int* flags,
                  int* info, const int* ctr, const DowndateArgs& dd, int* claim, double* hs, int lenient, int home,
                  bool wskip = false) {
    const bool xl = home >= 0;
    const unsigned rgrid = grid + (unsigned)w_split_count(RT, CB);
    unsigned xgrid = 8u * (unsigned)(CB - 1 + s_split_count(CB, true)) + 1u;
    for (unsigned left = rgrid - (unsigned)CB; left > 0; ++xgrid)
        if (xgrid % 8u != 0u) --left;
    xgrid += (unsigned)(xl ? home : 0);
    if (sweep_rl_enabled() && CB <= 9) {
        if (xl) k_sweep_rl<N, FUSED, 9, true><<<xgrid, 256, 0, st>>>(G, F, Linv, ld, CB, RT, flags, info, ctr, dd, hs, lenient, home);
        else k_sweep_rl<N, FUSED, 9, false><<<rgrid + 1, 256, 0, st>>>(G, F, Linv, ld, CB, RT, flags, info, ctr, dd, hs, lenient, home);
    } else if (sweep_rl_enabled() && CB <= 17) {
        if (xl) k_sweep_rl<N, FUSED, 17, true><<<xgrid, 256, 0, st>>>(G, F, Linv, ld, CB, RT, flags, info, ctr, dd, hs, lenient, home);
        else k_sweep_rl<N, FUSED, 17, false><<<rgrid + 1, 256, 0, st>>>(G, F, Linv, ld, CB, RT, flags, info, ctr, dd, hs, lenient, home);
    }
    else
        k_sweep<N, FUSED><<<grid, 256, 0, st>>>(G, F, Linv, ld, CB, RT, flags, info, ctr, dd, claim, hs, lenient, wskip ? 1 : 0);
}

inline bool short_last_panel() {
    static const int on = [] {
        const char* e = std::getenv("PNMOL_HIP_SHORT_LAST");
        return e ? std::atoi(e) : 1;
    }();
    return on != 0;
}
template <int N>
int launch_step(pnmol_filter* f, const double* Pin, const double* min, double frame_dt, double dt, double* Pout,
                double* mout, double* varout, bool record, StepKind kind) {
    pnmol_ctx* ctx = f->ctx;
    hipStream_t st = ctx->stream;
    IwpConsts c = f->iwp;
    for (int a = 0; a < f->n; ++a) {
        const double so = frame_dt == 0.0 ? 1.0 : nordsieck_scale(f->nu, a, frame_dt);
        c.ts[a] = so / nordsieck_scale(f->nu, a, dt);
    }
    MeasModel mm{f->ell_col, f->ell_val, f->ellw, f->d, f->m, f->dp, f->mp,
                 nordsieck_scale(f->nu, 0, dt), nordsieck_scale(f->nu, 1, dt)};
    const int dp = f->dp, mp = f->mp;
    const long Dp = f->Dp;

    if (kind != STEP_STEADY)
        k_predict<N><<<dim3(dp / 32, dp / 8 + 1), dim3(32, 8), sizeof(double) * Dp, st>>>(
        Pin, f->Ppred, f->Kg, c, dp, min, f->mpred, f->shift, f->G, f->zbuf, mm, f->ctr, f->flags, f->nflags, f->p32);
    if (kind != STEP_STEADY) {
        if (f->ellw > HW && f->sweep_mode != 0) {
            k_front<<<dim3((mp + 255) / 256, (unsigned)Dp), 256, 0, st>>>(f->Ppred, f->G, f->rdiag, f->Rdense, mm, Dp, f->p32);
            k_front_s<<<dim3((mp + 255) / 256, (unsigned)mp), 256, 0, st>>>(f->G, f->rdiag, f->Rdense, mm);
        } else {
            k_front<<<dim3((mp + 255) / 256, (unsigned)(Dp + mp + (f->sweep_mode == 0 ? mp : 0))), 256, 0, st>>>(
                f->Ppred, f->G, f->rdiag, f->Rdense, mm, Dp, f->p32);
        }
    }
    const long rowI0 = (long)mp + Dp + NB;
    const double* W = f->F + (long)mp * mp;
    const bool have_sq = (f->Sqinv != nullptr && f->sq_dt == dt);
    VecArgs va{f->mpred, f->F + ((long)mp + Dp) * mp, f->F + rowI0 * mp, f->zbuf, have_sq ? f->Sqinv : nullptr,
               mout, f->part};
    const int nreal = f->m - NB * (f->CB - 1);
    DowndateArgs dd{f->Ppred, Pout, varout, dp, 0, va, kind == STEP_FULL ? nullptr : f->Ppred, f->Kg, f->last_ctr, {}, {}, f->p32,
                    (nreal < 8 && short_last_panel()) ? nreal : 0};
    std::memcpy(dd.A1, f->iwp.A1, sizeof(dd.A1));
    std::memcpy(dd.Q1, f->iwp.Q1, sizeof(dd.Q1));
    if (f->sweep_mode == 2) {
        const int t32 = dp / NB, pairs = t32 * (t32 + 1) / 2;
        dd.vrows = 0;
        if constexpr (N <= 3)
            launch_sweep<N, true>(f->RT + pairs, st, f->G, f->F, f->Linv, mp, f->CB, f->RT, f->flags, f->info, f->ctr, dd,
                                  f->flags + f->RT + f->CB + 1, f->hs_scratch, f->p32 ? 2 : 0, f->xcd_home);
    } else {
        if (f->sweep_mode == 1) {
            if (f->w_gemm) {
                launch_sweep<N, false>(2 * f->CB + 1, st, f->G, f->F, f->Linv, mp, f->CB, f->RT, f->flags, f->info, f->ctr, dd,
                                       f->flags + f->RT + f->CB + 1, f->hs_scratch, f->p32 ? 2 : 0, f->xcd_home, true);
                const int nI = (int)(Dp / BDT), nt = nI * (mp / BDT);
                k_w_gemm<<<8 * ((nt + 7) / 8), 256, 0, st>>>(f->G + (long)mp * mp, f->F + rowI0 * mp, f->F + (long)mp * mp, mp, nI, nt);
            } else
            launch_sweep<N, false>(f->RT, st, f->G, f->F, f->Linv, mp, f->CB, f->RT, f->flags, f->info, f->ctr, dd,
                                   f->flags + f->RT + f->CB + 1, f->hs_scratch, f->p32 ? 2 : 0, f->xcd_home);
        } else {
            k_diag0<<<1, 128, 0, st>>>(f->G, f->F, f->Linv, mp, f->info, f->sdiag, f->ctr);
            for (int j = 0; j < f->CB; ++j) {
                const int nrb = f->RT - (j + 1);
                const int ncb = f->CB - 1 - j > 0 ? f->CB - 1 - j : 1;
                k_panel<<<dim3(nrb, ncb), 256, 0, st>>>(f->G, f->F, f->Linv, mp, j, f->CB, f->RBS, f->info, f->sdiag, f->ctr);
            }
        }
        const int tiles = dp / 16;
        const int vrows = (int)(((Dp + mp + 3) / 4 + tiles - 1) / tiles);
        if (f->dd_big) {
            const int T = (int)(Dp / BDT), nt = T * (T + 1) / 2;
            if (f->p32)
                k_downdate_big<float><<<8 * ((nt + 7) / 8), 256, 0, st>>>(reinterpret_cast<const float*>(f->Ppred), W,
                                                                          reinterpret_cast<float*>(Pout), varout, Dp, mp, nt);
            else
                k_downdate_big<double><<<8 * ((nt + 7) / 8), 256, 0, st>>>(static_cast<const double*>(f->Ppred), W, Pout, varout,
                                                                           Dp, mp, nt);
            k_vecops<<<dim3(tiles, vrows), 256, 0, st>>>(va, W, mp, Dp, tiles);
        } else {
            k_downdate<N><<<dim3(tiles, tiles + vrows), 256, 0, st>>>(f->Ppred, W, Pout, varout, dp, mp, 0, mp / 8, va);
        }
    }
    IwpConsts cn = f->iwp;
    for (int a = 0; a < MAXN; ++a) cn.ts[a] = 1.0;
    RoleArgs ra{cn, dp, mout, f->mpred, f->shift, f->G, f->zbuf, mm, f->flags, f->nflags};
    const unsigned rblocks = (f->d + 255) / 256;
    if (kind == STEP_FULL)
        k_readout<N, false><<<rblocks, 256, 0, st>>>(mout, varout, record ? f->rec_means : nullptr,
                                                    record ? f->rec_stds : nullptr, nordsieck_scale(f->nu, 0, dt), f->d,
                                                    f->part, f->rec, mp, f->ctr, ra, f->tickets, (int)rblocks, f->Ppred, f->rdiag,
                                                    f->Rdense, f->p32);
    else
        k_readout<N, true><<<rblocks + 1 + (unsigned)front_tiled_blocks(Dp, mp), 256, sizeof(double) * Dp, st>>>(
            mout, varout, record ? f->rec_means : nullptr, record ? f->rec_stds : nullptr, nordsieck_scale(f->nu, 0, dt),
            f->d, f->part, f->rec, mp, f->ctr, ra, f->tickets, (int)rblocks, f->Ppred, f->rdiag, f->Rdense, f->p32);
    hipError_t e = hipGetLastError();
    if (e != hipSuccess) {
        ctx->err = std::string("kernel launch: ") + hipGetErrorString(e);
        return -2;
    }
    return 0;
}

int dispatch_step(pnmol_filter* f, const double* Pin, const double* min, double frame_dt, double dt, double* Pout,
                  double* mout, double* varout, bool record, StepKind kind = STEP_FULL) {
    switch (f->n) {
        case 2: return launch_step<2>(f, Pin, min, frame_dt, dt, Pout, mout, varout, record, kind);
        case 3: return launch_step<3>(f, Pin, min, frame_dt, dt, Pout, mout, varout, record, kind);
        case 4: return launch_step<4>(f, Pin, min, frame_dt, dt, Pout, mout, varout, record, kind);
    }
    return -1;
}

void drop_graphs(pnmol_filter* f) {
    for (auto& g : f->graphs)
        if (g.exec) (void)hipGraphExecDestroy(g.exec);
    f->graphs.clear();
}

int get_graph(pnmol_filter* f, double* P0, double* M0, double* P1, double* M1, double* var, double dt, int nsteps,
              hipGraphExec_t* out) {
    pnmol_ctx* ctx = f->ctx;
    const bool have_sq = (f->Sqinv != nullptr && f->sq_dt == dt);
    for (auto& g : f->graphs)
        if (g.P0 == P0 && g.P1 == P1 && g.var == var && g.dt == dt && g.nsteps == nsteps && g.have_sq == have_sq &&
            g.fused == fused_loop(f)) {
            *out = g.exec;
            return 0;
        }
    if (f->graphs.size() >= 8) drop_graphs(f);
    hipGraph_t graph = nullptr;
    HIPCHK(ctx, hipStreamBeginCapture(ctx->stream, hipStreamCaptureModeThreadLocal));
    int rc = 0;
    for (int it = 0; it < nsteps && rc == 0; ++it)
        rc = (it & 1) ? dispatch_step(f, P1, M1, dt, dt, P0, M0, var, true, fused_loop(f) ? STEP_STEADY : STEP_FULL)
                      : dispatch_step(f, P0, M0, dt, dt, P1, M1, var, true, fused_loop(f) ? STEP_STEADY : STEP_FULL);
    hipError_t e = hipStreamEndCapture(ctx->stream, &graph);
    if (rc != 0 || e != hipSuccess) {
        if (graph) (void)hipGraphDestroy(graph);
        if (rc == 0) ctx->err = std::string("hipStreamEndCapture: ") + hipGetErrorString(e);
        return rc != 0 ? rc : -2;
    }
    hipGraphExec_t exec = nullptr;
    e = hipGraphInstantiate(&exec, graph, nullptr, nullptr, 0);
    (void)hipGraphDestroy(graph);
    if (e != hipSuccess) {
        ctx->err = std::string("hipGraphInstantiate: ") + hipGetErrorString(e);
        return -2;
    }
    f->graphs.push_back({P0, P1, var, dt, nsteps, have_sq, fused_loop(f), exec, false});
    *out = exec;
    return 0;
}

int build_ell(const double* M, const double* B, int d, int ds, int nB, int mp, std::vector<int>& ecol,
              std::vector<double>& eval) {
    const int m = d + nB;
    int w = 1;
    for (int i = 0; i < m; ++i) {
        int c = 0;
        const double* row = i < d ? M + (long)i * ds : B + (long)(i - d) * ds;
        for (int k = 0; k < ds; ++k) c += row[k] != 0.0;
        w = c > w ? c : w;
    }
    ecol.assign((size_t)w * mp, -1);
    eval.assign((size_t)w * mp, 0.0);
    for (int i = 0; i < m; ++i) {
        int e = 0;
        for (int k = 0; k < ds; ++k) {
            const double v = i < d ? -M[(long)i * ds + k] : B[(long)(i - d) * ds + k];
            if (v != 0.0) {
                ecol[(size_t)e * mp + i] = k;
                eval[(size_t)e * mp + i] = v;
                ++e;
            }
        }
    }
    return w;
}

int prepare_graphs(pnmol_filter* f, pnmol_state* s, int k, double dt, hipGraphExec_t* gbig, hipGraphExec_t* gpair) {
    *gbig = *gpair = nullptr;
    if (f->graph_chunk < 2) return 0;
    double *curP = s->P, *curM = s->mean, *nxtP = f->tmpP, *nxtM = f->tmpMean;
    const int lead = (s->frame_dt != dt || fused_loop(f)) ? 1 : 0;
    const int rest = k - lead;
    double *gP0 = lead ? nxtP : curP, *gM0 = lead ? nxtM : curM, *gP1 = lead ? curP : nxtP, *gM1 = lead ? curM : nxtM;
    int rc = 0;
    if (rest >= f->graph_chunk) rc = get_graph(f, gP0, gM0, gP1, gM1, s->var, dt, f->graph_chunk, gbig);
    if (rc == 0 && (rest % f->graph_chunk) >= 2) rc = get_graph(f, gP0, gM0, gP1, gM1, s->var, dt, 2, gpair);
    return rc;
}

__global__ __launch_bounds__(256) void k_cov_reference_order(const void* __restrict__ P, double* __restrict__ Gc, int n,
                                                             int d, int dp, long Dq, const double* __restrict__ sc, int p32) {
    const long e = (long)blockIdx.x * 256 + threadIdx.x;
    if (e >= Dq * Dq) return;
    const long r = e / Dq, c = e % Dq, D = (long)n * d, Dp = (long)n * dp;
    double v = (r == c) ? 1.0 : 0.0;
    if (r < D && c < D) {
        const int j = (int)(r / n), a = (int)(r % n), k = (int)(c / n), b = (int)(c % n);
        const long idx = ((long)a * dp + j) * Dp + (long)b * dp + k;
        v = sc[a] * sc[b] * (p32 ? (double)static_cast<const float*>(P)[idx] : static_cast<const double*>(P)[idx]);
    }
    Gc[e] = v;
}

__global__ __launch_bounds__(256) void k_copy_out(const double* __restrict__ rec, const double* __restrict__ means,
                                                  const double* __restrict__ stds, const int* __restrict__ info,
                                                  double* __restrict__ out, int k, int d, int cap) {
    const long nm = (long)k * d;
    double* hm = out + (size_t)4 * cap;
    double* hs = hm + (size_t)cap * d;
    int* hi = reinterpret_cast<int*>(hs + (size_t)cap * d);
    for (long e = (long)blockIdx.x * 256 + threadIdx.x; e < nm; e += (long)gridDim.x * 256) {
        if (means) hm[e] = means[e];
        if (stds) hs[e] = stds[e];
    }
    if (blockIdx.x == 0) {
        for (int e = threadIdx.x; e < 4 * k; e += 256) out[e] = rec[e];
        for (int e = threadIdx.x; e < k; e += 256) hi[e] = info[e];
    }
}

__global__ void k_init_call(int* __restrict__ info, int k, int* __restrict__ ctr, int* __restrict__ last_ctr) {
    for (int e = threadIdx.x; e < k; e += blockDim.x) info[e] = 0x7f7f7f7f;
    if (threadIdx.x == 0) {
        *ctr = 0;
        *last_ctr = k;
    }
}

int ensure_rec(pnmol_filter* f, int k) {
// ... 312 lines not shown
    }
    std::vector<double> Kg((size_t)dp * dp, 0.0);
    if (desc->K) {
        for (int i = 0; i < ds; ++i)
            for (int k = 0; k <= i; ++k) Kg[(size_t)i * dp + k] = Kg[(size_t)k * dp + i] = desc->K[(size_t)i * ds + k];
    } else
    for (int i = 0; i < ds; ++i)
        for (int k = 0; k <= i; ++k) {
            double s = 0.0;
            for (int q = 0; q <= k; ++q) s += desc->Gamma[(long)i * ds + q] * desc->Gamma[(long)k * ds + q];
            Kg[(size_t)i * dp + k] = Kg[(size_t)k * dp + i] = s;
        }

    if (ds == d) {
        f->hGamma.assign((size_t)dp * dp, 0.0);
        for (int i = 0; i < d; ++i)
            for (int k = 0; k <= i; ++k) f->hGamma[(size_t)i * dp + k] = desc->Gamma[(size_t)i * d + k];
    }

    auto fail = [&](int code) {
        pnmol_filter_destroy(f);
        return code;
    };
#define FCHK(call)                                                                    \
    do {                                                                              \
        hipError_t e__ = (call);                                                      \
        if (e__ != hipSuccess) {                                                      \
            ctx->err = std::string(#call) + ": " + hipGetErrorString(e__);            \
            return fail(e__ == hipErrorOutOfMemory ? -4 : -2);                        \
        }                                                                             \
    } while (0)
    const size_t tall = (size_t)f->RT * NB * mp;
    FCHK(hipMalloc(&f->ell_col, sizeof(int) * ecol.size()));
    FCHK(hipMalloc(&f->ell_val, sizeof(double) * eval.size()));
    FCHK(hipMalloc(&f->Kg, sizeof(double) * Kg.size()));
    FCHK(hipMalloc(&f->rdiag, sizeof(double) * mp));
    FCHK(hipMalloc(&f->shift, sizeof(double) * mp));
    FCHK(hipMalloc(&f->G, sizeof(double) * tall));
    FCHK(hipMalloc(&f->F, sizeof(double) * tall));
    FCHK(hipMalloc(&f->Linv, sizeof(double) * (size_t)f->CB * NB * NB));
    FCHK(hipMemset(f->Linv, 0, sizeof(double) * (size_t)f->CB * NB * NB));
    FCHK(hipMalloc(&f->Ppred, f->psz * (size_t)Dp * Dp));
    FCHK(hipMalloc(&f->tmpP, f->psz * (size_t)Dp * Dp));
    FCHK(hipMalloc(&f->mpred, sizeof(double) * Dp));
    FCHK(hipMalloc(&f->tmpMean, sizeof(double) * Dp));
    FCHK(hipMalloc(&f->var, sizeof(double) * Dp));
    FCHK(hipMalloc(&f->zbuf, sizeof(double) * mp));
    FCHK(hipMalloc(&f->part, sizeof(double) * 3 * mp));
    FCHK(hipMalloc(&f->ctr, sizeof(int)));
    {
        const int h1 = 1;
        FCHK(hipMalloc(&f->one, sizeof(int)));
        FCHK(hipMalloc(&f->info_err, sizeof(int)));
        FCHK(hipMemcpy(f->one, &h1, sizeof(int), hipMemcpyHostToDevice));
    }
    if (const char* gc = std::getenv("PNMOL_HIP_GRAPH_CHUNK")) f->graph_chunk = std::atoi(gc) / 2 * 2;
    if (const char* e = std::getenv("PNMOL_HIP_SWEEP")) f->sweep_mode = std::atoi(e);
    if (f->sweep_mode == 2 && n > 3) f->sweep_mode = 1;
    {
        const char* e = std::getenv("PNMOL_HIP_DD_BIG");
        const bool fits = f->Dp % BDT == 0 && f->mp % BDK == 0 && f->sweep_mode >= 1 && (!f->p32 || f->sweep_mode == 2);
        const bool want = e ? std::atoi(e) != 0 : (f->Dp >= 8192 && f->CB > 17);
        if (fits && want) {
            f->dd_big = 1;
            f->sweep_mode = 1;
            const char* g = std::getenv("PNMOL_HIP_W_GEMM");
            f->w_gemm = (g ? std::atoi(g) != 0 : 1) && f->mp % BDT == 0 && f->CB > 17;
        }
    }
    {
        static std::atomic<int> next_home[MAX_DEVICES];
        const bool rl = sweep_rl_enabled() && f->CB <= 17 && f->sweep_mode >= 1;
        if (rl) {
            const int dv = ctx->device % MAX_DEVICES;
            const int others = live_rl_filters[dv].fetch_add(1);
            f->counted = true;
            const bool xl = sweep_xl_mode() < 0 ? others == 0 : sweep_xl_mode() == 1;
            f->xcd_home = xl ? next_home[dv].fetch_add(1) % 8 : -1;
        }
    }
    FCHK(hipMalloc(&f->sdiag, sizeof(double) * (mp + 1)));
    f->nflags = std::max({f->RT + f->CB + 1 + f->CB * f->CB, rl_flags(f->RT, f->CB).total,
                          rl_flags((int)(f->Dp / NB) + 1, (int)(f->Dp / NB) + 1).total});
    FCHK(hipMalloc(&f->flags, sizeof(int) * f->nflags));
    FCHK(hipMemset(f->flags, 0, sizeof(int) * f->nflags));
    FCHK(hipMalloc(&f->hs_scratch, sizeof(double) * (size_t)std::max(f->CB * f->CB, 2 * f->CB + 2) * NB * NB));
    if (const char* e = std::getenv("PNMOL_HIP_FUSE_PREDICT")) f->fuse_predict = std::atoi(e);
    FCHK(hipMalloc(&f->last_ctr, sizeof(int)));
    FCHK(hipMemset(f->last_ctr, 0, sizeof(int)));
    FCHK(hipMalloc(&f->tickets, sizeof(int)));
    FCHK(hipMemset(f->tickets, 0, sizeof(int)));
    if (f->p32 && f->sweep_mode != 2 && !f->dd_big) {
        ctx->err = "pnmol_filter_create: dtype = fp32 covariance needs the fused sweep (num_derivatives <= 2, PNMOL_HIP_SWEEP unset)";
        return fail(-1);
    }
    FCHK(hipMemcpy(f->ell_col, ecol.data(), sizeof(int) * ecol.size(), hipMemcpyHostToDevice));
    FCHK(hipMemcpy(f->ell_val, eval.data(), sizeof(double) * eval.size(), hipMemcpyHostToDevice));
    {
        std::vector<int> slot((size_t)mp, 0);
        f->base_has_diag = 1;
        for (int i = 0; i < d; ++i) {
            int e = 0;
            while (e < w && ecol[(size_t)e * mp + i] != i) ++e;
            if (e == w) f->base_has_diag = 0, e = 0;
            slot[i] = e;
        }
        f->base_w = w;
        FCHK(hipMalloc(&f->ell_col_base, sizeof(int) * ecol.size()));
        FCHK(hipMalloc(&f->ell_val_base, sizeof(double) * eval.size()));
        FCHK(hipMalloc(&f->ell_diag_slot, sizeof(int) * mp));
        FCHK(hipMemcpy(f->ell_col_base, ecol.data(), sizeof(int) * ecol.size(), hipMemcpyHostToDevice));
        FCHK(hipMemcpy(f->ell_val_base, eval.data(), sizeof(double) * eval.size(), hipMemcpyHostToDevice));
        FCHK(hipMemcpy(f->ell_diag_slot, slot.data(), sizeof(int) * mp, hipMemcpyHostToDevice));
        FCHK(hipHostMalloc(&f->h_op, sizeof(double) * (size_t)(d + mp), hipHostMallocMapped));
        FCHK(hipHostGetDevicePointer(reinterpret_cast<void**>(&f->h_op_dev), f->h_op, 0));
        FCHK(hipEventCreate(&f->ev_op));
    }
    FCHK(hipMemcpy(f->Kg, Kg.data(), sizeof(double) * Kg.size(), hipMemcpyHostToDevice));
    FCHK(hipMemcpy(f->rdiag, rdiag.data(), sizeof(double) * mp, hipMemcpyHostToDevice));
    if (!diag) {
        FCHK(hipMalloc(&f->Rdense, sizeof(double) * Rd.size()));
        FCHK(hipMemcpy(f->Rdense, Rd.data(), sizeof(double) * Rd.size(), hipMemcpyHostToDevice));
    }
    FCHK(hipMemset(f->shift, 0, sizeof(double) * mp));
    FCHK(hipMemset(f->G, 0, sizeof(double) * tall));
    k_set_identity<<<(mp + 255) / 256, 256>>>(f->G + ((size_t)mp + Dp + NB) * mp, mp);
    FCHK(hipDeviceSynchronize());
    FCHK(hipMemset(f->F, 0, sizeof(double) * tall));
    FCHK(hipMemset(f->var, 0, sizeof(double) * Dp));
    FCHK(hipMemset(f->tmpP, 0, f->psz * (size_t)Dp * Dp));
    FCHK(hipMemset(f->tmpMean, 0, sizeof(double) * Dp));
    FCHK(hipEventCreate(&f->ev0));
    FCHK(hipEventCreate(&f->ev1));
#undef FCHK
    if (ensure_rec(f, 128) != 0) return fail(-2);
    *out = f;
    return 0;
}

int pnmol_filter_destroy(pnmol_filter* f) {
    if (!f) return -1;
    if (f->states.load() != 0) {
        f->ctx->err = "pnmol_filter_destroy: " + std::to_string(f->states.load()) + " state(s) of this filter are still alive";
        return -1;
    }
    if (f->samples.load() != 0) {
        f->ctx->err = "pnmol_filter_destroy: " + std::to_string(f->samples.load()) + " sample block(s) of this filter are still alive";
        return -1;
    }
    if (f->bridges.load() != 0) {
        f->ctx->err = "pnmol_filter_destroy: " + std::to_string(f->bridges.load()) + " bridge(s) of this filter are still alive";
        return -1;
    }
    if (f->counted) live_rl_filters[f->ctx->device % MAX_DEVICES].fetch_sub(1);
    if (f->registered) f->ctx->children.fetch_sub(1);
    hipSetDevice(f->ctx->device);
    drop_graphs(f);
    if (f->ctr) hipFree(f->ctr);
    if (f->h_pin) hipHostFree(f->h_pin);
    void* ptrs[] = {f->ell_col, f->ell_val, f->Kg,   f->rdiag,   f->Rdense, f->shift,     f->G,        f->F,
                    f->Linv,    f->Ppred,   f->mpred, f->zbuf,   f->var,    f->Sqinv,     f->rec,      f->part,  f->sdiag,
                    f->info,    f->tmpP,    f->tmpMean, f->rec_means, f->rec_stds, f->flags, f->Qfull, f->one, f->info_err, f->hs_scratch, f->last_ctr, f->tickets};
    for (void* p : ptrs)
        if (p) hipFree(p);
    if (f->h_op) hipHostFree(f->h_op);
    if (f->ev_op) hipEventDestroy(f->ev_op);
    for (void* q : {(void*)f->ell_col_base, (void*)f->ell_val_base, (void*)f->ell_diag_slot})
        if (q) hipFree(q);
    pnmol_smooth_free_ws(f);
    pnmol_sample_free_ws(f);
    pnmol_dense_free_ws(f);
    pnmol_observe_free_ws(f);
    if (f->ev0) hipEventDestroy(f->ev0);
    if (f->ev1) hipEventDestroy(f->ev1);
    delete f;
    return 0;
}

int pnmol_filter_dims(const pnmol_filter* f, int* d, int* n, int* m, int* dp, int* mp) {
    if (!f) return -1;
    if (d) *d = f->d;
    if (n) *n = f->n;
    if (m) *m = f->m;
    if (dp) *dp = f->dp;
    if (mp) *mp = f->mp;
    return 0;
}

int pnmol_filter_sweep_layout(const pnmol_filter* f, int* kernel, int* xcd_home) {
    if (!f) return -1;
    if (kernel) *kernel = f->sweep_mode == 0 ? 0 : (sweep_rl_enabled() && f->CB <= 17 ? 2 : 1);
    if (xcd_home) *xcd_home = f->xcd_home;
    return 0;
}

int pnmol_filter_set_error_model(pnmol_filter* f, double dt, const double* Sq_inv, const double* Sq_diag) {
    if (!f || !Sq_inv || !Sq_diag || !(dt > 0.0)) return -1;
    pnmol_ctx* ctx = f->ctx;
    HIPCHK(ctx, hipSetDevice(ctx->device));
    const int m = f->m, mp = f->mp;
    std::vector<double> pad((size_t)mp * mp, 0.0);
    for (int i = 0; i < m; ++i) std::memcpy(&pad[(size_t)i * mp], Sq_inv + (size_t)i * m, sizeof(double) * m);
    HIPCHK(ctx, hipStreamSynchronize(ctx->stream));
    if (!f->Sqinv) HIPCHK(ctx, hipMalloc(&f->Sqinv, sizeof(double) * pad.size()));
    HIPCHK(ctx, hipMemcpy(f->Sqinv, pad.data(), sizeof(double) * pad.size(), hipMemcpyHostToDevice));
    f->sqdiag.assign(Sq_diag, Sq_diag + m);
    f->sq_dt = dt;
    drop_graphs(f);
    return 0;
}

int pnmol_filter_prepare_error_model(pnmol_filter* f, double dt) {
    if (!f || !(dt > 0.0)) return -1;
    pnmol_ctx* ctx = f->ctx;
    HIPCHK(ctx, hipSetDevice(ctx->device));
    hipStream_t st = ctx->stream;
    const int mp = f->mp, m = f->m, dp = f->dp;
    const long Dp = f->Dp;
    if (!f->Qfull) {
        HIPCHK(ctx, hipMalloc(&f->Qfull, f->psz * (size_t)Dp * Dp));
        k_fill_q<<<(unsigned)((Dp * Dp + 255) / 256), 256, 0, st>>>(f->Qfull, f->Kg, f->iwp, f->n, dp, f->p32);
    }
    const bool fresh = (f->Sqinv == nullptr);
    if (fresh) HIPCHK(ctx, hipMalloc(&f->Sqinv, sizeof(double) * (size_t)mp * mp));
    HIPCHK(ctx, hipMemsetAsync(f->flags, 0, sizeof(int) * f->nflags, st));
    HIPCHK(ctx, hipMemsetAsync(f->info_err, 0x7f, sizeof(int), st));
    MeasModel mm{f->ell_col, f->ell_val, f->ellw, f->d, f->m, f->dp, f->mp,
                 nordsieck_scale(f->nu, 0, dt), nordsieck_scale(f->nu, 1, dt)};
    switch (f->n) {
        case 2: run_error_model_sweep<2>(f, mm); break;
        case 3: run_error_model_sweep<3>(f, mm); break;
        case 4: run_error_model_sweep<4>(f, mm); break;
        default: return -1;
    }
    const double* T = f->F + ((long)mp + Dp + NB) * mp;
    k_ttt<<<dim3(mp / 16, mp / 16), 256, 0, st>>>(T, f->Sqinv, mp);
    std::vector<double> hd((size_t)m);
    int inf = 0;
    HIPCHK(ctx, hipMemcpy2DAsync(hd.data(), sizeof(double), f->G, sizeof(double) * (mp + 1), sizeof(double), m,
                                 hipMemcpyDeviceToHost, st));
    HIPCHK(ctx, hipMemcpyAsync(&inf, f->info_err, sizeof(int), hipMemcpyDeviceToHost, st));
    HIPCHK(ctx, hipStreamSynchronize(st));
    hipError_t e = hipGetLastError();
    if (e != hipSuccess) {
        ctx->err = std::string("prepare_error_model: ") + hipGetErrorString(e);
        return -2;
    }
    if (int rc = sweep_info_result(ctx, inf, mp, "prepare_error_model", "Sq not positive definite")) return rc;
    f->sqdiag = hd;
    f->sq_dt = dt;
    if (fresh) drop_graphs(f);
    return 0;
}

int pnmol_filter_set_operator(pnmol_filter* f, const double* M_dd, const double* shift_d) {
    if (!f || !M_dd) return -1;
    pnmol_ctx* ctx = f->ctx;
    HIPCHK(ctx, hipSetDevice(ctx->device));
    std::vector<int> ecol;
    std::vector<double> eval;
    const int w = build_ell(M_dd, f->hB.data(), f->d, f->ds, f->nB, f->mp, ecol, eval);
    HIPCHK(ctx, hipStreamSynchronize(ctx->stream));
    if (w != f->ellw || w > f->ell_cap) drop_graphs(f);
    if (w > f->ell_cap) {
        if (f->ell_col) (void)hipFree(f->ell_col);
        if (f->ell_val) (void)hipFree(f->ell_val);
        f->ell_col = nullptr, f->ell_val = nullptr, f->ell_cap = 0;
        HIPCHK(ctx, hipMalloc(&f->ell_col, sizeof(int) * ecol.size()));
        HIPCHK(ctx, hipMalloc(&f->ell_val, sizeof(double) * eval.size()));
        f->ell_cap = w;
    }
    f->ellw = w;
    f->ell_is_base = 0;
    HIPCHK(ctx, hipMemcpy(f->ell_col, ecol.data(), sizeof(int) * ecol.size(), hipMemcpyHostToDevice));
    HIPCHK(ctx, hipMemcpy(f->ell_val, eval.data(), sizeof(double) * eval.size(), hipMemcpyHostToDevice));
// ... 424 lines not shown
    const double* hm = rec + (size_t)4 * f->rec_cap;
    const double* hs = hm + (size_t)f->rec_cap * f->d;
    const int* inf = reinterpret_cast<const int*>(hs + (size_t)f->rec_cap * f->d);
    if (means_kd) std::memcpy(means_kd, hm, sizeof(double) * (size_t)k * f->d);
    if (stds_kd) std::memcpy(stds_kd, hs, sizeof(double) * (size_t)k * f->d);
    const bool have_sq = (f->Sqinv != nullptr && f->sq_dt == dt);
    int bad = -1, stuck = -1;
    double t = s->t;
    for (int it = 0; it < k; ++it) {
        t += dt;
        pnmol_step_out o;
        fill_out(f, &rec[(size_t)4 * it], inf[it], t, have_sq, &o);
        if (info_k) info_k[it] = o;
        if (o.info >= 0 && bad < 0) bad = it;
        if (o.info == -2 && stuck < 0) stuck = it;
    }
    s->t = t;
    s->frame_dt = dt;
    if (stuck >= 0) {
        ctx->err = "sweep kernel: a dependency wait timed out in step " + std::to_string(stuck);
        return -2;
    }
    if (bad >= 0) {
        ctx->err = "innovation matrix not positive definite in step " + std::to_string(bad);
        return -3;
    }
    return 0;
}

int pnmol_filter_steps(pnmol_filter* f, pnmol_state* s, int k, double dt, double* means_kd, double* stds_kd,
                       pnmol_step_out* info_k) {
    const int rc = pnmol_filter_steps_begin(f, s, k, dt);
    if (rc != 0) return rc;
    return pnmol_filter_steps_end(f, s, means_kd, stds_kd, info_k);
}

int pnmol_filter_prepare_steps(pnmol_filter* f, pnmol_state* s, int k, double dt) {
    if (!f || !s || s->f != f || k < 1 || !(dt > 0.0)) return -1;
    pnmol_ctx* ctx = f->ctx;
    HIPCHK(ctx, hipSetDevice(ctx->device));
    int rc = ensure_rec(f, k);
    if (rc != 0) return rc;
    const size_t Dp = (size_t)f->Dp, nP = Dp * Dp * f->psz / sizeof(double);
    double* bak = nullptr;
    HIPCHK(ctx, hipMalloc(&bak, sizeof(double) * (nP + 2 * Dp)));
    hipStream_t st = ctx->stream;
    const double t0 = s->t, frame0 = s->frame_dt;
    hipError_t e = hipMemcpyAsync(bak, s->P, sizeof(double) * nP, hipMemcpyDeviceToDevice, st);
    if (e == hipSuccess) e = hipMemcpyAsync(bak + nP, s->mean, sizeof(double) * Dp, hipMemcpyDeviceToDevice, st);
    if (e == hipSuccess) e = hipMemcpyAsync(bak + nP + Dp, s->var, sizeof(double) * Dp, hipMemcpyDeviceToDevice, st);
    if (e == hipSuccess) {
        rc = pnmol_filter_steps(f, s, k, dt, nullptr, nullptr, nullptr);
        if (rc == -3) rc = 0;
        if ((k & 1) && rc == 0) {
            double* t;
            t = s->P, s->P = f->tmpP, f->tmpP = t;
            t = s->mean, s->mean = f->tmpMean, f->tmpMean = t;
        }
        e = hipMemcpyAsync(s->P, bak, sizeof(double) * nP, hipMemcpyDeviceToDevice, st);
        if (e == hipSuccess) e = hipMemcpyAsync(s->mean, bak + nP, sizeof(double) * Dp, hipMemcpyDeviceToDevice, st);
        if (e == hipSuccess) e = hipMemcpyAsync(s->var, bak + nP + Dp, sizeof(double) * Dp, hipMemcpyDeviceToDevice, st);
        s->t = t0, s->frame_dt = frame0;
    }
    if (e == hipSuccess) e = hipStreamSynchronize(st);
    (void)hipFree(bak);
    if (e != hipSuccess) {
        ctx->err = std::string("pnmol_filter_prepare_steps: ") + hipGetErrorString(e);
        return -2;
    }
    return rc;
}

int pnmol_filter_debug_poison(pnmol_filter* f) {
    if (!f) return -1;
    pnmol_ctx* ctx = f->ctx;
    HIPCHK(ctx, hipSetDevice(ctx->device));
    const long nF = (long)f->RT * NB * f->mp, nL = (long)f->CB * NB * NB;
    const long nH = (long)std::max(f->CB * f->CB, 2 * f->CB + 2) * NB * NB;
    k_poison<<<1024, 256, 0, ctx->stream>>>(f->F, nF, f->Linv, nL, f->hs_scratch, nH);
    HIPCHK(ctx, hipGetLastError());
    return 0;
}

int pnmol_filter_last_steps_ms(pnmol_filter* f, float* ms) {
    if (!f || !ms) return -1;
    *ms = f->last_ms;
    return 0;
}

int pnmol_filter_debug_read(pnmol_filter* f, int which, double* dst, long count) {
#ifdef PNMOL_SWEEP_STAMP
    if (f && which == 5) {
        hipStreamSynchronize(f->ctx->stream);
        std::vector<long long> h(512 * 8);
        if (hipMemcpyFromSymbol(h.data(), HIP_SYMBOL(pnmol_sweep_stamp), sizeof(long long) * 512 * 8) != hipSuccess) return -2;
        for (long i = 0; i < count && i < 512 * 8; ++i) dst[i] = (double)h[i];
        return 0;
    }
#endif
    if (!f || !dst || count < 0) return -1;
    pnmol_ctx* ctx = f->ctx;
    HIPCHK(ctx, hipSetDevice(ctx->device));
    const double* src = nullptr;
    long avail = 0;
    const long tall = (long)f->RT * NB * f->mp;
    switch (which) {
        case 0: src = f->Ppred, avail = f->Dp * f->Dp; break;
        case 1: src = f->G, avail = tall; break;
        case 2: src = f->F, avail = tall; break;
        case 3: src = f->mpred, avail = f->Dp; break;
        case 4: src = f->zbuf, avail = f->mp; break;
        default: return -1;
    }
    if (count > avail) return -1;
    HIPCHK(ctx, hipStreamSynchronize(ctx->stream));
    if (which == 0 && f->p32) {
        std::vector<float> h((size_t)count);
        HIPCHK(ctx, hipMemcpy(h.data(), src, sizeof(float) * count, hipMemcpyDeviceToHost));
        std::copy(h.begin(), h.end(), dst);
        return 0;
    }
    HIPCHK(ctx, hipMemcpy(dst, src, sizeof(double) * count, hipMemcpyDeviceToHost));
    return 0;
}

}
```

### pnmol-experiments_amd/csrc/pnmol_internal.hpp

```cpp
#pragma once
#include <hip/hip_runtime.h>

#include <algorithm>
#include <atomic>
#include <cmath>
#include <string>
#include <vector>

#include "pnmol_hip.h"

constexpr int NB = 32;
constexpr int MAXN = 4;

namespace {
struct IwpConsts {
    double A1[MAXN * MAXN];
    double Q1[MAXN * MAXN];
    double ts[MAXN];
};
}

#define HIPCHK(ctx, call)                                                                        \
    do {                                                                                         \
        hipError_t e__ = (call);                                                                 \
        if (e__ != hipSuccess) {                                                                 \
            (ctx)->err = std::string(#call) + ": " + hipGetErrorString(e__);                     \
            return -2;                                                                           \
        }                                                                                        \
    } while (0)

inline int round_up(int x, int q) { return (x + q - 1) / q * q; }

inline double nordsieck_scale(int nu, int a, double dt) {
    double fact = 1.0;
    for (int q = 2; q <= nu - a; ++q) fact *= q;
    return std::pow(std::fabs(dt), nu - a + 0.5) / fact;
}

struct pnmol_ctx {
    int device = 0;
    hipStream_t stream = nullptr;
    std::string err;
    std::atomic<int> children{0};
};

struct SweepWs {
    double *G = nullptr, *F = nullptr, *Linv = nullptr, *feed = nullptr;
    int *flags = nullptr, *info = nullptr;
    int nflags = 0;
    int rt = 0, cb = 0, ld = 0;
    bool left_looking = false;
};
hipError_t sweep_ws_alloc(SweepWs* w, pnmol_ctx* ctx, int rt, int cb);
void sweep_ws_free(SweepWs* w);
int sweep_ws_enqueue(pnmol_filter* f, const SweepWs& w, hipStream_t st, int lenient, const char* who);
int sweep_info_result(pnmol_ctx* ctx, int inf, long limit, const char* who, const char* what,
                      const char* wait = "a dependency wait timed out");

struct ObserveWs {
    int qp = 0;
    SweepWs sweep;
    double* dev = nullptr;
    std::vector<double> host;
};

struct pnmol_filter {
    pnmol_ctx* ctx = nullptr;
    int d = 0, n = 0, nu = 0, nB = 0, m = 0, dp = 0, mp = 0, CB = 0, RBS = 0, RBW = 0, RT = 0, ellw = 0;
    int* tickets = nullptr;
    int* last_ctr = nullptr;
    int fuse_predict = 1;
    int* flags = nullptr;
    int nflags = 0;
    double* hs_scratch = nullptr;
    int w_gemm = 0;
    int dd_big = 0;
    int sweep_mode = 2;
    int ds = 0;
    bool counted = false;
    bool registered = false;
    std::atomic<int> states{0};
    int xcd_home = -1;
    int p32 = 0;
    size_t psz = 8;
    long Dp = 0;
    IwpConsts iwp{};
    int* ell_col = nullptr;
    double* ell_val = nullptr;
    int* ell_col_base = nullptr;
    double* ell_val_base = nullptr;
    int* ell_diag_slot = nullptr;
    int base_w = 0, base_has_diag = 0;
    int ell_is_base = 1;
    double* h_op = nullptr;
    double* h_op_dev = nullptr;
    hipEvent_t ev_op = nullptr;
    double *Kg = nullptr, *rdiag = nullptr, *Rdense = nullptr, *shift = nullptr;
    double *G = nullptr, *F = nullptr, *Linv = nullptr, *Ppred = nullptr, *mpred = nullptr, *zbuf = nullptr;
    double *var = nullptr, *Sqinv = nullptr, *rec = nullptr, *part = nullptr, *sdiag = nullptr;
    int* info = nullptr;
    std::vector<double> sqdiag;
    double* Qfull = nullptr;
    int* one = nullptr;
    int* info_err = nullptr;
    double sq_dt = -1.0;
    std::vector<double> hB;
    int ell_cap = 0;
    double *tmpP = nullptr, *tmpMean = nullptr;
    double *rec_means = nullptr, *rec_stds = nullptr;
    double* h_pin = nullptr;
    double* h_pin_dev = nullptr;
    int rec_cap = 0;
    hipEvent_t ev0 = nullptr, ev1 = nullptr;
    float last_ms = 0.f;
    int* ctr = nullptr;
    int pending_k = 0;
    double pending_dt = 0.0;
    pnmol_state* pending_state = nullptr;
    struct GraphEntry {
        double *P0, *P1, *var;
        double dt;
        int nsteps;
        bool have_sq;
        bool fused;
        hipGraphExec_t exec;
        bool launched;
    };
    std::vector<GraphEntry> graphs;
    int graph_chunk = 10;
    SweepWs sm_sweep;
    double *sm_gain = nullptr, *sm_C = nullptr, *sm_Psh = nullptr, *sm_vec = nullptr;
    SweepWs sp_sweep;
    double *sp_Gamma = nullptr, *sp_mh = nullptr;
    hipStream_t sp_stream = nullptr;
    hipEvent_t sp_ev_built = nullptr, sp_ev_swept = nullptr;
    std::vector<double> hGamma;
    std::atomic<int> samples{0};
    std::atomic<int> bridges{0};
    void* dn_scratch = nullptr;
    size_t dn_cap = 0;
    struct BridgeSlab* dn_slab = nullptr;
    std::vector<ObserveWs*> ob_ws;
};

struct pnmol_state {
    pnmol_filter* f = nullptr;
    double* mean = nullptr;
    double* P = nullptr;
    double* var = nullptr;
    double t = 0.0;
    double frame_dt = 0.0;
};

constexpr int BRIDGE_SLAB_SLOTS = 64;
struct BridgeSlab {
    double* base = nullptr;
    int used = 0;
    int live = 0;
};

struct pnmol_bridge {
    pnmol_filter* f = nullptr;
    BridgeSlab* slab = nullptr;
    double* blk = nullptr;
    double* Cfull = nullptr;
    double t = 0.0, dt = 0.0;
};

struct pnmol_samples {
    pnmol_filter* f = nullptr;
    int S = 0, Sp = 0;
    double* X = nullptr;
    double* Xi = nullptr;
    double* Xt = nullptr;
    double* R = nullptr;
    double* Y = nullptr;
    double* stage = nullptr;
    double t = 0.0, frame_dt = 0.0;
    bool drawn = false;
};

inline void frame_scales(const pnmol_filter* f, double frame_dt, double* sc) {
    for (int a = 0; a < f->n; ++a) sc[a] = frame_dt == 0.0 ? 1.0 : nordsieck_scale(f->nu, a, frame_dt);
}
inline void frame_scales(const pnmol_state* s, double* sc) { frame_scales(s->f, s->frame_dt, sc); }
inline double frame_ratio(const pnmol_filter* f, int a, double from_dt, double to_dt) {
    return (from_dt == 0.0 ? 1.0 : nordsieck_scale(f->nu, a, from_dt)) / nordsieck_scale(f->nu, a, to_dt);
}
inline bool times_agree(double a, double b, double dt) {
    return std::fabs(a - b) <= 16.0 * 2.220446049250313e-16 * std::max({std::fabs(a), std::fabs(b), std::fabs(dt)});
}
inline void small_cholesky(int n, const double* A, double* L, bool semidefinite = false) {
    for (int a = 0; a < n; ++a)
        for (int b = 0; b <= a; ++b) {
            double v = A[a * MAXN + b];
            for (int e = 0; e < b; ++e) v -= L[a * MAXN + e] * L[b * MAXN + e];
            if (!semidefinite) L[a * MAXN + b] = (a == b) ? std::sqrt(v) : v / L[b * MAXN + b];
            else if (a == b) L[a * MAXN + a] = v > 0.0 ? std::sqrt(v) : 0.0;
            else L[a * MAXN + b] = L[b * MAXN + b] > 0.0 ? v / L[b * MAXN + b] : 0.0;
        }
}

void pnmol_smooth_free_ws(pnmol_filter* f);
void pnmol_sample_free_ws(pnmol_filter* f);
void pnmol_dense_free_ws(pnmol_filter* f);
void pnmol_observe_free_ws(pnmol_filter* f);
int pnmol_smooth_ensure_ws(pnmol_filter* f);
// ... 42 lines not shown
```

### pnmol-experiments_amd/pnmol/_hip.py

```python

import ctypes
import os
import pathlib

import numpy as np


_c_double_p = ctypes.POINTER(ctypes.c_double)
_HERE = pathlib.Path(__file__).resolve().parent
LIB_PATH = pathlib.Path(os.environ.get("PNMOL_HIP_LIB", _HERE.parent / "lib" / "libpnmol_hip.so"))


class PnmolHipError(RuntimeError):
    """A call into libpnmol_hip.so failed."""


class StepOut(ctypes.Structure):
    _fields_ = [
        ("t_new", ctypes.c_double),
        ("diffusion_squared_local", ctypes.c_double),
        ("sigma2_whitened", ctypes.c_double),
        ("error_sigma2", ctypes.c_double),
        ("info", ctypes.c_int),
    ]
# ... 4 lines not shown
    _fields_ = [
        ("log_likelihood", ctypes.c_double),
        ("mahalanobis", ctypes.c_double),
        ("logdet", ctypes.c_double),
        ("info", ctypes.c_int),
    ]


class FilterDesc(ctypes.Structure):
    _fields_ = [
        ("d", ctypes.c_int),
        ("num_derivatives", ctypes.c_int),
        ("nB", ctypes.c_int),
        ("L", _c_double_p),
        ("B", _c_double_p),
        ("E_sqrtm", _c_double_p),
        ("R_sqrtm", _c_double_p),
        ("Gamma", _c_double_p),
        ("d_state", ctypes.c_int),
        ("dtype", ctypes.c_int),
        ("K", _c_double_p),
    ]


_vp = ctypes.c_void_p
SYMBOLS = {
    "pnmol_abi_version": (ctypes.c_int, []),
    "pnmol_device_count": (ctypes.c_int, [ctypes.POINTER(ctypes.c_int)]),
    "pnmol_ctx_create": (ctypes.c_int, [ctypes.c_int, ctypes.POINTER(_vp)]),
    "pnmol_ctx_destroy": (ctypes.c_int, [_vp]),
    "pnmol_ctx_synchronize": (ctypes.c_int, [_vp]),
    "pnmol_fd_solve_batched": (ctypes.c_int, [_vp, _c_double_p, _c_double_p, _c_double_p, ctypes.c_int, ctypes.c_int,
                                              _c_double_p, _c_double_p]),
    "pnmol_cholesky_lower": (ctypes.c_int, [_vp, _c_double_p, ctypes.c_int, _c_double_p]),
    "pnmol_last_error": (ctypes.c_char_p, [_vp]),
    "pnmol_filter_create": (ctypes.c_int, [_vp, ctypes.POINTER(FilterDesc), ctypes.POINTER(_vp)]),
    "pnmol_filter_destroy": (ctypes.c_int, [_vp]),
    "pnmol_filter_set_error_model": (ctypes.c_int, [_vp, ctypes.c_double, _c_double_p, _c_double_p]),
    "pnmol_filter_predict_mean": (ctypes.c_int, [_vp, _vp, ctypes.c_double, _c_double_p]),
    "pnmol_filter_set_operator": (ctypes.c_int, [_vp, _c_double_p, _c_double_p]),
    "pnmol_filter_set_operator_diagonal": (ctypes.c_int, [_vp, _c_double_p, _c_double_p]),
    "pnmol_state_create": (ctypes.c_int, [_vp, ctypes.POINTER(_vp)]),
    "pnmol_state_destroy": (ctypes.c_int, [_vp]),
    "pnmol_state_clone": (ctypes.c_int, [_vp, ctypes.POINTER(_vp)]),
    "pnmol_state_set": (ctypes.c_int, [_vp, ctypes.c_double, _c_double_p, _c_double_p]),
    "pnmol_state_set_sqrtm": (ctypes.c_int, [_vp, ctypes.c_double, _c_double_p, _c_double_p]),
    "pnmol_state_get_time": (ctypes.c_int, [_vp, _c_double_p]),
    "pnmol_state_get_mean": (ctypes.c_int, [_vp, _c_double_p]),
    "pnmol_state_get_cov_sqrtm": (ctypes.c_int, [_vp, _c_double_p]),
    "pnmol_state_get_cov": (ctypes.c_int, [_vp, _c_double_p]),
    "pnmol_state_get_marginal_var": (ctypes.c_int, [_vp, _c_double_p]),
    "pnmol_filter_step": (ctypes.c_int, [_vp, _vp, ctypes.c_double, _vp, ctypes.POINTER(StepOut), _c_double_p]),
    "pnmol_smoother_step": (ctypes.c_int, [_vp, _vp, _vp, ctypes.c_double, _vp]),
    "pnmol_state_predict": (ctypes.c_int, [_vp, _vp, ctypes.c_double, _vp]),
    "pnmol_state_observe": (ctypes.c_int, [_vp, _vp, ctypes.c_int, _c_double_p, _c_double_p, _c_double_p, _vp,
                                           ctypes.POINTER(ObserveOut)]),
    "pnmol_state_predict_marginals": (ctypes.c_int, [_vp, _vp, ctypes.c_int, _c_double_p, _c_double_p, _c_double_p]),
    "pnmol_smoother_step_bridge": (ctypes.c_int, [_vp, _vp, _vp, ctypes.c_double, _vp, ctypes.c_int, ctypes.POINTER(_vp)]),
    "pnmol_bridge_destroy": (ctypes.c_int, [_vp]),
    "pnmol_bridge_get_interval": (ctypes.c_int, [_vp, _c_double_p, _c_double_p, ctypes.POINTER(ctypes.c_int)]),
    "pnmol_bridge_eval": (ctypes.c_int, [_vp, ctypes.c_int, _c_double_p, _c_double_p, _c_double_p]),
    "pnmol_bridge_state": (ctypes.c_int, [_vp, _vp, _vp, ctypes.c_double, _vp]),
    "pnmol_samples_create": (ctypes.c_int, [_vp, ctypes.c_int, ctypes.POINTER(_vp)]),
    "pnmol_samples_destroy": (ctypes.c_int, [_vp]),
    "pnmol_samples_draw": (ctypes.c_int, [_vp, _vp, _c_double_p, ctypes.c_ulonglong, ctypes.c_ulonglong, ctypes.c_double]),
    "pnmol_samples_step_back": (ctypes.c_int, [_vp, _vp, ctypes.c_double, _c_double_p, ctypes.c_ulonglong, ctypes.c_ulonglong,
                                               ctypes.c_double]),
    "pnmol_samples_interpolate": (ctypes.c_int, [_vp, _vp, _vp, ctypes.c_double, _c_double_p, ctypes.c_ulonglong,
                                                 ctypes.c_ulonglong, ctypes.c_double]),
    "pnmol_samples_clone": (ctypes.c_int, [_vp, ctypes.POINTER(_vp)]),
    "pnmol_samples_get": (ctypes.c_int, [_vp, _c_double_p]),
    "pnmol_samples_get_time": (ctypes.c_int, [_vp, _c_double_p]),
    "pnmol_sample_noise": (ctypes.c_int, [_vp, ctypes.c_ulonglong, ctypes.c_ulonglong, ctypes.c_int, ctypes.c_int,
                                          _c_double_p]),
    "pnmol_filter_steps": (ctypes.c_int, [_vp, _vp, ctypes.c_int, ctypes.c_double, _c_double_p, _c_double_p,
                                          ctypes.POINTER(StepOut)]),
    "pnmol_filter_steps_begin": (ctypes.c_int, [_vp, _vp, ctypes.c_int, ctypes.c_double]),
    "pnmol_filter_steps_end": (ctypes.c_int, [_vp, _vp, _c_double_p, _c_double_p, ctypes.POINTER(StepOut)]),
    "pnmol_filter_prepare_steps": (ctypes.c_int, [_vp, _vp, ctypes.c_int, ctypes.c_double]),
    "pnmol_filter_last_steps_ms": (ctypes.c_int, [_vp, ctypes.POINTER(ctypes.c_float)]),
    "pnmol_filter_prepare_error_model": (ctypes.c_int, [_vp, ctypes.c_double]),
    "pnmol_filter_debug_read": (ctypes.c_int, [_vp, ctypes.c_int, _c_double_p, ctypes.c_long]),
    "pnmol_filter_debug_poison": (ctypes.c_int, [_vp]),
    "pnmol_filter_dims": (ctypes.c_int, [_vp] + [ctypes.POINTER(ctypes.c_int)] * 5),
    "pnmol_filter_sweep_layout": (ctypes.c_int, [_vp] + [ctypes.POINTER(ctypes.c_int)] * 2),
    "pnmol_qr_r": (ctypes.c_int, [_vp, _c_double_p, ctypes.c_int, ctypes.c_int, _c_double_p]),
    "pnmol_qr_last_ms": (ctypes.c_int, [ctypes.POINTER(ctypes.c_float)]),
    "pnmol_sqrt_propagate_cholesky_factor": (ctypes.c_int, [_vp, _c_double_p, ctypes.c_int, ctypes.c_int, _c_double_p,
                                                             ctypes.c_int, _c_double_p]),
    "pnmol_sqrt_update": (ctypes.c_int, [_vp, _c_double_p, ctypes.c_int, ctypes.c_int, _c_double_p, _c_double_p,
                                         _c_double_p, _c_double_p, _c_double_p]),
    "pnmol_sqrt_filter_create": (ctypes.c_int, [_vp, ctypes.POINTER(FilterDesc), ctypes.POINTER(_vp)]),
    "pnmol_sqrt_filter_destroy": (ctypes.c_int, [_vp]),
    "pnmol_sqrt_filter_set_state": (ctypes.c_int, [_vp, ctypes.c_double, _c_double_p, _c_double_p]),
    "pnmol_sqrt_filter_get_state": (ctypes.c_int, [_vp, _c_double_p, _c_double_p, _c_double_p]),
    "pnmol_sqrt_filter_predict_mean": (ctypes.c_int, [_vp, ctypes.c_double, _c_double_p]),
    "pnmol_sqrt_filter_set_operator": (ctypes.c_int, [_vp, _c_double_p, _c_double_p]),
    "pnmol_sqrt_filter_prepare_error_model": (ctypes.c_int, [_vp, ctypes.c_double]),
    "pnmol_sqrt_filter_step": (ctypes.c_int, [_vp, ctypes.c_double, ctypes.POINTER(StepOut), _c_double_p]),
    "pnmol_sqrt_filter_steps": (ctypes.c_int, [_vp, ctypes.c_int, ctypes.c_double, _c_double_p, _c_double_p,
                                               ctypes.POINTER(StepOut)]),
    "pnmol_sqrt_filter_last_steps_ms": (ctypes.c_int, [_vp, ctypes.POINTER(ctypes.c_float)]),
    "pnmol_sqrt_update_no_meascov": (ctypes.c_int, [_vp, _c_double_p, ctypes.c_int, ctypes.c_int, _c_double_p,
                                                    _c_double_p, _c_double_p, _c_double_p]),
}

_lib = None


def load_library():
    global _lib
    if _lib is None:
        if not LIB_PATH.exists():
            raise PnmolHipError(
                f"{LIB_PATH} not found: build it with `python __graft_entry__.py` (hipcc --offload-arch=gfx950). "
                "pnmol has no CPU fallback for the filter step."
            )
        lib = ctypes.CDLL(str(LIB_PATH))
        for name, (res, args) in SYMBOLS.items():
            fn = getattr(lib, name)
            fn.restype, fn.argtypes = res, args
        _lib = lib
    return _lib


def _dp(a):
    return a.ctypes.data_as(_c_double_p)


def _f64(a, shape=None):
    a = np.ascontiguousarray(np.asarray(a, dtype=np.float64))
    if shape is not None and a.shape != shape:
        raise ValueError(f"expected shape {shape}, got {a.shape}")
    return a


class Context:

    _cache = {}

    def __init__(self, device=0):
        self.lib = load_library()
        n = ctypes.c_int(0)
        rc = self.lib.pnmol_device_count(ctypes.byref(n))
        if rc != 0 or n.value < 1:
            raise PnmolHipError("no HIP device visible: the PNMOL filter step needs an AMD GPU (MI355X / gfx950)")
        h = _vp()
        rc = self.lib.pnmol_ctx_create(int(device), ctypes.byref(h))
        if rc != 0:
            raise PnmolHipError(f"pnmol_ctx_create(device={device}) failed with {rc}")
        self.handle, self.device = h, int(device)

    @classmethod
    def default(cls, device=None):
        if device is None:
            device = int(os.environ.get("PNMOL_HIP_DEVICE", os.environ.get("LOCAL_RANK", "0")))
            n = ctypes.c_int(0)
            load_library().pnmol_device_count(ctypes.byref(n))
            if n.value > 0:
                device %= n.value
        if device not in cls._cache:
            cls._cache[device] = cls(device)
        return cls._cache[device]

    def cholesky(self, A):
        A = _f64(A)
# ... 34 lines not shown
            rc = self.lib.pnmol_sqrt_propagate_cholesky_factor(self.handle, _dp(S1), n, k1, _dp(S2), S2.shape[1], _dp(out))
        self.check(rc, "pnmol_sqrt_propagate_cholesky_factor")
        return out

    def sqrt_update(self, H, C, meascov_sqrtm=None):
        H, C = _f64(H), _f64(C)
        m, D = H.shape
        if C.shape != (D, D):
            raise ValueError(f"cov_cholesky must be {(D, D)}, got {C.shape}")
        if m > D:
            raise ValueError("update_sqrt needs output_dim <= input_dim (base/sqrt.py:56-58)")
        C_new, gain, Sl = np.empty((D, D)), np.empty((D, m)), np.empty((m, m))
        if meascov_sqrtm is None:
            rc = self.lib.pnmol_sqrt_update_no_meascov(self.handle, _dp(H), m, D, _dp(C), _dp(C_new), _dp(gain), _dp(Sl))
        else:
            E = _f64(meascov_sqrtm, (m, m))
            rc = self.lib.pnmol_sqrt_update(self.handle, _dp(H), m, D, _dp(C), _dp(E), _dp(C_new), _dp(gain), _dp(Sl))
        self.check(rc, "pnmol_sqrt_update")
        return C_new, gain, Sl

    def qr_last_ms(self):
        ms = ctypes.c_float(0)
        self.lib.pnmol_qr_last_ms(ctypes.byref(ms))
        return ms.value

    def sample_noise(self, seed, step_index, rows, cols):
        out = np.empty((int(rows), int(cols)))
        self.check(self.lib.pnmol_sample_noise(self.handle, int(seed), int(step_index), int(rows), int(cols), _dp(out)),
                   "pnmol_sample_noise")
        return out

    def check(self, rc, what):
        if rc != 0:
            msg = self.lib.pnmol_last_error(self.handle)
            raise PnmolHipError(f"{what} failed ({rc}): {msg.decode() if msg else ''}")

    def synchronize(self):
        self.check(self.lib.pnmol_ctx_synchronize(self.handle), "pnmol_ctx_synchronize")


class Filter:

    DTYPES = {"f64": 0, "f32": 1}

    def __init__(self, ctx, *, L, B, E_sqrtm, R_sqrtm, Gamma, num_derivatives, dtype="f64", K=None):
        self.ctx, self.lib = ctx, ctx.lib
        d, ds = L.shape
        nB = B.shape[0]
        self._keep = [_f64(L, (d, ds)), _f64(B, (nB, ds)), _f64(E_sqrtm, (d, d)), _f64(R_sqrtm, (nB, nB)),
                      _f64(Gamma, (ds, ds))]
        gram = _f64(self._keep[4] @ self._keep[4].T if K is None else K, (ds, ds))
        desc = FilterDesc(d, int(num_derivatives), nB, *[_dp(a) for a in self._keep], ds, self.DTYPES[dtype], _dp(gram))
        self.dtype = dtype
        self.ds = ds
        h = _vp()
        ctx.check(self.lib.pnmol_filter_create(ctx.handle, ctypes.byref(desc), ctypes.byref(h)), "pnmol_filter_create")
        self.handle = h
        self.d, self.n, self.nB, self.m = d, int(num_derivatives) + 1, nB, d + nB
        self.error_model_dt = None
        self._live = {}
        self._live_samples = {}
        self._live_bridges = {}

    def __del__(self):
        live = getattr(self, "_live", None)
        while live:
            _, sh = live.popitem()
            self.lib.pnmol_state_destroy(sh)
        live = getattr(self, "_live_samples", None)
        while live:
            _, sh = live.popitem()
            self.lib.pnmol_samples_destroy(sh)
        live = getattr(self, "_live_bridges", None)
        while live:
            _, sh = live.popitem()
            self.lib.pnmol_bridge_destroy(sh)
        h, self.handle = getattr(self, "handle", None), None
        if h:
            self.lib.pnmol_filter_destroy(h)

    def sweep_layout(self):
        k, x = ctypes.c_int(0), ctypes.c_int(0)
        self.lib.pnmol_filter_sweep_layout(self.handle, ctypes.byref(k), ctypes.byref(x))
        return {"kernel": ("per_panel", "k_sweep", "k_sweep_rl")[k.value], "xcd_home": x.value}

    def dims(self):
        v = [ctypes.c_int(0) for _ in range(5)]
        self.lib.pnmol_filter_dims(self.handle, *[ctypes.byref(x) for x in v])
        return dict(zip(("d", "n", "m", "dp", "mp"), (x.value for x in v)))

    def prepare_error_model(self, dt):
        self.ctx.check(self.lib.pnmol_filter_prepare_error_model(self.handle, float(dt)), "pnmol_filter_prepare_error_model")
        self.error_model_dt = float(dt)

    def set_error_model(self, dt, Sq_inv, Sq_diag):
        a, b = _f64(Sq_inv, (self.m, self.m)), _f64(Sq_diag, (self.m,))
        self.ctx.check(self.lib.pnmol_filter_set_error_model(self.handle, float(dt), _dp(a), _dp(b)),
                       "pnmol_filter_set_error_model")
        self.error_model_dt = float(dt)

    def new_state(self):
        return State(self)

    def new_samples(self, num_samples):
        return Samples(self, num_samples)

    def predict_mean(self, state_in, dt):
        out = np.empty(self.d)
        self.ctx.check(self.lib.pnmol_filter_predict_mean(self.handle, state_in.handle, float(dt), _dp(out)),
                       "pnmol_filter_predict_mean")
        return out

    def set_operator(self, M, shift=None):
        a = _f64(M, (self.d, self.ds))
        b = _f64(shift, (self.d,)) if shift is not None else None
        self.ctx.check(self.lib.pnmol_filter_set_operator(self.handle, _dp(a), _dp(b) if b is not None else None),
                       "pnmol_filter_set_operator")
        self.error_model_dt = None

    def set_operator_diagonal(self, jdiag, shift=None):
        a = _f64(jdiag, (self.d,))
        b = _f64(shift, (self.d,)) if shift is not None else None
        self.ctx.check(self.lib.pnmol_filter_set_operator_diagonal(self.handle, _dp(a), _dp(b) if b is not None else None),
                       "pnmol_filter_set_operator_diagonal")
        self.error_model_dt = None

    def step(self, state_in, dt, want_error=True):
        out = State(self)
        info = StepOut()
        err = np.empty(self.d) if want_error else None
        rc = self.lib.pnmol_filter_step(self.handle, state_in.handle, float(dt), out.handle, ctypes.byref(info),
                                        _dp(err) if want_error else None)
        self.ctx.check(rc, "pnmol_filter_step")
        return out, info, err

    def smoother_step(self, filt_k, smooth_next, dt, bridge=None):
        out = State(self)
        if bridge is None:
            rc = self.lib.pnmol_smoother_step(self.handle, filt_k.handle, smooth_next.handle, float(dt), out.handle)
            self.ctx.check(rc, "pnmol_smoother_step")
            return out
        if bridge not in ("marginal", "full"):
            raise ValueError(f'bridge must be None, "marginal" or "full", got {bridge!r}')
        h = _vp()
        rc = self.lib.pnmol_smoother_step_bridge(self.handle, filt_k.handle, smooth_next.handle, float(dt), out.handle,
                                                 int(bridge == "full"), ctypes.byref(h))
        self.ctx.check(rc, "pnmol_smoother_step_bridge")
        t = ctypes.c_double(0.0)
        self.lib.pnmol_state_get_time(out.handle, ctypes.byref(t))
        return out, Bridge(self, h, (t.value, float(dt), bridge == "full"))

    def observe(self, state, C, y, R_sqrtm=None):
        C = _f64(C)
        if C.ndim != 2 or C.shape[1] != self.ds or not 1 <= C.shape[0] <= self.ds:
            raise ValueError(f"C must be (q, {self.ds}) with 1 <= q <= {self.ds}, got {C.shape}")
        q = C.shape[0]
        y = _f64(y, (q,))
        R = None if R_sqrtm is None else _f64(R_sqrtm, (q, q))
        out, res = State(self), ObserveOut()
        rc = self.lib.pnmol_state_observe(self.handle, state.handle, q, _dp(C), _dp(y), None if R is None else _dp(R),
                                          out.handle, ctypes.byref(res))
        self.ctx.check(rc, "pnmol_state_observe")
        return out, res

    def predict(self, state, dt):
        out = State(self)
        self.ctx.check(self.lib.pnmol_state_predict(self.handle, state.handle, float(dt), out.handle), "pnmol_state_predict")
        return out

    def predict_marginals(self, state, dts):
        dts = _f64(np.atleast_1d(dts))
        if dts.ndim != 1 or dts.size < 1:
            raise ValueError(f"expected a non-empty 1-d array of step sizes, got shape {dts.shape}")
        means, stds = np.empty((dts.size, self.n, self.d)), np.empty((dts.size, self.n, self.d))
        rc = self.lib.pnmol_state_predict_marginals(self.handle, state.handle, dts.size, _dp(dts), _dp(means), _dp(stds))
        self.ctx.check(rc, "pnmol_state_predict_marginals")
        return means, stds

    def steps(self, state, k, dt, want_means=True, want_stds=True):
        means = np.empty((k, self.d)) if want_means else None
        stds = np.empty((k, self.d)) if want_stds else None
        infos = (StepOut * k)()
        rc = self.lib.pnmol_filter_steps(self.handle, state.handle, int(k), float(dt),
                                         _dp(means) if want_means else None, _dp(stds) if want_stds else None, infos)
        self.ctx.check(rc, "pnmol_filter_steps")
        return means, stds, infos

    def steps_begin(self, state, k, dt):
        self.ctx.check(self.lib.pnmol_filter_steps_begin(self.handle, state.handle, int(k), float(dt)),
                       "pnmol_filter_steps_begin")
        self._pending_k = int(k)

    def steps_end(self, state, want_means=True, want_stds=True):
        k = self._pending_k
        means = np.empty((k, self.d)) if want_means else None
        stds = np.empty((k, self.d)) if want_stds else None
        infos = (StepOut * k)()
        rc = self.lib.pnmol_filter_steps_end(self.handle, state.handle, _dp(means) if want_means else None,
                                             _dp(stds) if want_stds else None, infos)
        self.ctx.check(rc, "pnmol_filter_steps_end")
        return means, stds, infos

    def prepare_steps(self, state, k, dt):
        self.ctx.check(self.lib.pnmol_filter_prepare_steps(self.handle, state.handle, int(k), float(dt)),
                       "pnmol_filter_prepare_steps")

    def last_steps_ms(self):
        ms = ctypes.c_float(0.0)
        self.lib.pnmol_filter_last_steps_ms(self.handle, ctypes.byref(ms))
        return float(ms.value)

    def debug_poison(self):
        self.ctx.check(self.lib.pnmol_filter_debug_poison(self.handle), "pnmol_filter_debug_poison")

    def debug_read(self, which, count):
        out = np.empty(int(count))
        self.ctx.check(self.lib.pnmol_filter_debug_read(self.handle, int(which), _dp(out), int(count)),
                       "pnmol_filter_debug_read")
        return out


class State:

    def __init__(self, flt, _handle=None):
        self.filter, self.lib, self.ctx = flt, flt.lib, flt.ctx
        if _handle is None:
            _handle = _vp()
            self.ctx.check(self.lib.pnmol_state_create(flt.handle, ctypes.byref(_handle)), "pnmol_state_create")
        self.handle = _handle
        flt._live[id(self)] = _handle

    def _destroy(self):
        h, self.handle = getattr(self, "handle", None), None
        flt = getattr(self, "filter", None)
        if h and flt is not None and flt._live.pop(id(self), None) is not None:
            self.lib.pnmol_state_destroy(h)

    def __del__(self):
        self._destroy()

    def clone(self):
        h = _vp()
        self.ctx.check(self.lib.pnmol_state_clone(self.handle, ctypes.byref(h)), "pnmol_state_clone")
        return State(self.filter, h)

    def set(self, t, mean_nd, cov_DD):
        f = self.filter
        D = f.n * f.ds
        a, b = _f64(mean_nd, (f.n, f.ds)), _f64(cov_DD, (D, D))
        self.ctx.check(self.lib.pnmol_state_set(self.handle, float(t), _dp(a), _dp(b)), "pnmol_state_set")

    def set_sqrtm(self, t, mean_nd, cov_sqrtm_DD):
        f = self.filter
        D = f.n * f.ds
        a, b = _f64(mean_nd, (f.n, f.ds)), _f64(cov_sqrtm_DD, (D, D))
        self.ctx.check(self.lib.pnmol_state_set_sqrtm(self.handle, float(t), _dp(a), _dp(b)), "pnmol_state_set_sqrtm")

    @property
    def t(self):
        t = ctypes.c_double(0.0)
        self.lib.pnmol_state_get_time(self.handle, ctypes.byref(t))
        return t.value

    def mean(self):
        out = np.empty((self.filter.n, self.filter.ds))
        self.ctx.check(self.lib.pnmol_state_get_mean(self.handle, _dp(out)), "pnmol_state_get_mean")
        return out

    def marginal_var(self):
        out = np.empty((self.filter.n, self.filter.ds))
        self.ctx.check(self.lib.pnmol_state_get_marginal_var(self.handle, _dp(out)), "pnmol_state_get_marginal_var")
        return out

    def cov_sqrtm(self):
        D = self.filter.n * self.filter.ds
        out = np.empty((D, D))
        self.ctx.check(self.lib.pnmol_state_get_cov_sqrtm(self.handle, _dp(out)), "pnmol_state_get_cov_sqrtm")
        return out

    def cov(self):
        D = self.filter.n * self.filter.ds
        out = np.empty((D, D))
        self.ctx.check(self.lib.pnmol_state_get_cov(self.handle, _dp(out)), "pnmol_state_get_cov")
        return out


class Bridge:

    def __init__(self, flt, handle, interval=None):
        self.filter, self.lib, self.ctx = flt, flt.lib, flt.ctx
        self.handle = handle
        flt._live_bridges[id(self)] = handle
        if interval is None:
            t, dt, full = ctypes.c_double(0.0), ctypes.c_double(0.0), ctypes.c_int(0)
            self.lib.pnmol_bridge_get_interval(handle, ctypes.byref(t), ctypes.byref(dt), ctypes.byref(full))
            interval = (t.value, dt.value, bool(full.value))
        self.t, self.dt, self.full = interval
# ... 160 lines not shown
```

Baseline: 7991 steps/s.

## Fuse front Gram assembly and vector ops into single persistent sweep launch per step

Adds a one-launch loop mode, on by default through PNMOL_HIP_ONE_LAUNCH=1, in which the right-looking sweep kernel gathers the Gram/S entries directly from the predicted covariance and the measurement model. It no longer reads a G matrix built by separate k_front kernels. Standard deviations are written from the downdate body, and gather-completion flags let the downdate wait on the remaining work. This removes the front kernels and the second launch per step, and so also the kernel-boundary synchronisation. In exchange, S entries are computed redundantly inside chain and panel roles, flag buffers double in size, and the recomputation may add arithmetic latency on the critical chain.

```diff
diff --git a/include/pnmol_hip.h b/include/pnmol_hip.h
--- a/include/pnmol_hip.h
+++ b/include/pnmol_hip.h
@@ -39,6 +39,7 @@
 int pnmol_filter_create(pnmol_ctx* ctx, const pnmol_filter_desc* desc, pnmol_filter** out);
 int pnmol_filter_destroy(pnmol_filter* f);
 int pnmol_filter_sweep_layout(const pnmol_filter* f, int* kernel, int* xcd_home);
+int pnmol_filter_loop_launches(const pnmol_filter* f, int* launches);
 
 int pnmol_filter_set_error_model(pnmol_filter* f, double dt, const double* Sq_inv,
                                  const double* Sq_diag);
@@ -119,6 +120,7 @@
 
 int pnmol_filter_debug_read(pnmol_filter* f, int which, double* dst, long count);
 int pnmol_filter_debug_poison(pnmol_filter* f);
+int pnmol_filter_debug_poison_g(pnmol_filter* f);
 int pnmol_filter_dims(const pnmol_filter* f, int* d, int* n, int* m, int* dp, int* mp);
 
 #ifdef __cplusplus
diff --git a/pnmol-experiments_amd/csrc/pnmol_hip.hip b/pnmol-experiments_amd/csrc/pnmol_hip.hip
--- a/pnmol-experiments_amd/csrc/pnmol_hip.hip
+++ b/pnmol-experiments_amd/csrc/pnmol_hip.hip
@@ -866,6 +866,7 @@
     double sFeedD[NB * TLD];
     double sd[2][NB];
     double red[4];
+    double sdall[17 * NB];
     Diag4Lds d4[2];
 };
 
@@ -1159,6 +1160,9 @@
     double A1[MAXN * MAXN], Q1[MAXN * MAXN];
     int p32;
     int last_ksteps;
+    double* stds;
+    double s0;
+    int d;
 };
 
 template <typename PT>
@@ -1188,7 +1192,7 @@
 template <int N, typename PT, bool SHORT_LAST>
 __device__ __forceinline__ void sweep_downdate_body(SweepLds& L, const DowndateArgs& dd, const double* F, int ld, int CB,
                                                     int RBS, const int* frow, int* fabort, int* info, int pair, int tid,
-                                                    int l, int w, int slot) {
+                                                    int l, int w, int slot, const int* fgath = nullptr, int ngath = 0) {
     const int fr = l & 15, fk = l >> 4, qr = w >> 1, qc = w & 1;
     const int T32 = dd.dp / NB;
     int J = (int)((sqrt(8.0 * pair + 1.0) - 1.0) * 0.5);
@@ -1289,6 +1293,8 @@
             if (l < 2 * N) {
                 const int a = l >> 1, tile = (l & 1) ? K : J;
                 v = flag_ld(frow + RBS + a * T32 + tile);
+            } else if (fgath != nullptr && l == 2 * N) {
+                v = flag_ld(fgath) >= ngath ? (1 << 30) : CB - 1;
             }
             return v;
         };
@@ -1401,7 +1407,11 @@
         if (J == K && qr == qc) {
 #pragma unroll
             for (int r = 0; r < 4; ++r)
-                if (AccOf<PT>::row(fk, r) == fr) dd.var[row0 + fr] = acc[a][a][r];
+                if (AccOf<PT>::row(fk, r) == fr) {
+                    dd.var[row0 + fr] = acc[a][a][r];
+                    if (a == 0 && dd.stds != nullptr && J * NB + qr * 16 + fr < dd.d)
+                        dd.stds[(size_t)slot * dd.d + J * NB + qr * 16 + fr] = dd.s0 * sqrt(fmax((double)acc[a][a][r], 0.0));
+                }
         }
         if (write_p) {
 #pragma unroll
@@ -1459,9 +1469,9 @@
 template <int N, bool SHORT_LAST = false>
 __device__ __forceinline__ void sweep_downdate_role(SweepLds& L, const DowndateArgs& dd, const double* F, int ld, int CB,
                                                     int RBS, const int* frow, int* fabort, int* info, int pair, int tid,
-                                                    int l, int w, int slot) {
-    if (dd.p32) sweep_downdate_body<N, float, SHORT_LAST>(L, dd, F, ld, CB, RBS, frow, fabort, info, pair, tid, l, w, slot);
-    else sweep_downdate_body<N, double, SHORT_LAST>(L, dd, F, ld, CB, RBS, frow, fabort, info, pair, tid, l, w, slot);
+                                                    int l, int w, int slot, const int* fgath = nullptr, int ngath = 0) {
+    if (dd.p32) sweep_downdate_body<N, float, SHORT_LAST>(L, dd, F, ld, CB, RBS, frow, fabort, info, pair, tid, l, w, slot, fgath, ngath);
+    else sweep_downdate_body<N, double, SHORT_LAST>(L, dd, F, ld, CB, RBS, frow, fabort, info, pair, tid, l, w, slot, fgath, ngath);
 }
 
 template <int N, bool FUSED, bool CHAINHELP = FUSED>
@@ -1745,7 +1755,7 @@
     return (PNMOL_W_SPLIT && RBW > 0 && CB > W_SPLIT_H + 1) ? RBW : 0;
 }
 struct RlFlags {
-    int frow, fabort, fxcc, ffeed, fdiag, fnew, fcol, fdiagL, fnewL, frowL, CBp, total;
+    int frow, fabort, fxcc, ffeed, fdiag, fnew, fcol, fdiagL, fnewL, frowL, fgath, CBp, total;
 };
 __host__ __device__ inline RlFlags rl_flags(int RT, int CB) {
     const int RTp = (RT + 31) / 32 * 32, CBp = (CB + 31) / 32 * 32;
@@ -1761,7 +1771,8 @@
     f.fdiagL = f.fcol + RL_REP * CBp;
     f.fnewL = f.fdiagL + CBp;
     f.frowL = f.fnewL + CBp;
-    f.total = f.frowL + CBp;
+    f.fgath = f.frowL + CBp;
+    f.total = f.fgath + 32 * RL_REP;
     return f;
 }
 __device__ __forceinline__ int xcc_id() { return __builtin_amdgcn_s_getreg((3 << 11) | 20) & 15; }
@@ -1892,6 +1903,7 @@
 #pragma unroll
         for (int o = 32; o > 0; o >>= 1) out[q] += __shfl_xor(out[q], o);
 }
+template <bool WT = false>
 __device__ __forceinline__ void vecops_rows8(const VecArgs& va, const double* __restrict__ W, int mp, long Dp, long r0,
                                              const double* bq , int l) {
     double a[8];
@@ -1901,7 +1913,8 @@
             double mine = a[0];
 #pragma unroll
             for (int q = 1; q < 8; ++q) mine = (l == q) ? a[q] : mine;
-            va.mout[r0 + l] = va.mpred[r0 + l] - mine;
+            if constexpr (WT) wt_st(va.mout + r0 + l, va.mpred[r0 + l] - mine);
+            else va.mout[r0 + l] = va.mpred[r0 + l] - mine;
         }
     } else {
         const long k0 = r0 - Dp;
@@ -1912,9 +1925,15 @@
             for (int q = 1; q < 8; ++q) mine = (l == q) ? a[q] : mine;
             const double bm = bq[l];
             const long k = k0 + l;
-            va.part[k] = va.r[k] * va.r[k];
-            va.part[mp + k] = mine * mine;
-            va.part[2 * mp + k] = va.z[k] * bm;
+            if constexpr (WT) {
+                wt_st(va.part + k, va.r[k] * va.r[k]);
+                wt_st(va.part + mp + k, mine * mine);
+                wt_st(va.part + 2 * mp + k, va.z[k] * bm);
+            } else {
+                va.part[k] = va.r[k] * va.r[k];
+                va.part[mp + k] = mine * mine;
+                va.part[2 * mp + k] = va.z[k] * bm;
+            }
         }
     }
 }
@@ -1954,10 +1973,93 @@
     }
 }
 
-template <bool XL>
+struct OneArgs {
+    MeasModel mm;
+    const double* rdiag;
+    const double* Rdense;
+    IwpConsts c;
+    const double* shift;
+    double* G;
+    double* zbuf;
+    double* mpred;
+    double* means_base;
+    double* rec_base;
+    double s0;
+    int d;
+    int* tickets;
+    int* ctr;
+    int* flags_base;
+    int nflags;
+};
+template <typename PT>
+__device__ __forceinline__ double s_gather(const PT* __restrict__ Ppred, long Dp, const OneArgs& oa, int ip, int i) {
+    if (ip >= oa.mm.m || i >= oa.mm.m) return (ip == i) ? 1.0 : 0.0;
+    HRow rr, rc;
+    h_row_load(oa.mm, ip, rr);
+    h_row_load(oa.mm, i, rc);
+    return s_entry_w<HW>(Ppred, Dp, oa.mm, rr, rc, ip, i, oa.rdiag, oa.Rdense);
+}
+template <int MAXT, typename PT>
+__device__ __forceinline__ void gather_w_tiles(d4 (&n)[MAXT], int ulo, int uhi, int t0, int ntiles, const PT* __restrict__ Ppred,
+                                               long Dp, const OneArgs& oa, long y0, int colC) {
+#pragma unroll
+    for (int u = 0; u < MAXT; ++u)
+        if (u >= ulo && u < uhi && t0 + u < ntiles) {
+            const int i = (t0 + u) * NB + colC;
+            HRow rc;
+            if (i < oa.mm.m) h_row_load(oa.mm, i, rc);
+#pragma unroll
+            for (int r = 0; r < 4; ++r) {
+                const double v = (i < oa.mm.m) ? h_row_dot_w<HW>(rc, Ppred + (y0 + 4 * r) * Dp) : 0.0;
+                n[u][r] = -v;
+            }
+        }
+}
+template <int MAXT, typename PT>
+__device__ __forceinline__ void gather_s_tiles(d4 (&n)[MAXT], int ulo, int uhi, int t0, int ntiles, const PT* __restrict__ Ppred,
+                                               long Dp, const OneArgs& oa, int ip0, int colC) {
+    if (uhi > ntiles - t0) uhi = ntiles - t0;
+    if (ulo >= uhi) return;
+    HRow rr[4];
+#pragma unroll
+    for (int r = 0; r < 4; ++r) h_row_load(oa.mm, ip0 + 4 * r, rr[r]);
+    HRow rc;
+    h_row_load(oa.mm, (t0 + ulo) * NB + colC, rc);
+    for (int u = ulo; u < uhi; ++u) {
+        const int i = (t0 + u) * NB + colC;
+        HRow rcn;
+        h_row_load(oa.mm, (t0 + (u + 1 < uhi ? u + 1 : u)) * NB + colC, rcn);
+        d4 v;
+#pragma unroll
+        for (int r = 0; r < 4; ++r) {
+            const int ip = ip0 + 4 * r;
+            const double e = (ip < oa.mm.m && i < oa.mm.m) ? s_entry_w<HW>(Ppred, Dp, oa.mm, rr[r], rc, ip, i, oa.rdiag, oa.Rdense)
+                                                          : ((ip == i) ? 1.0 : 0.0);
+            v[r] = -e;
+        }
+#pragma unroll
+        for (int q = 0; q < MAXT; ++q)
+            if (q == u) n[q] = v;
+        rc = rcn;
+    }
+}
+template <typename PT>
+__device__ __forceinline__ d4 gather_s_diag(const PT* __restrict__ Ppred, long Dp, const OneArgs& oa, int I, int wr, int wc,
+                                            int fr, int fk) {
+    d4 a;
+#pragma unroll
+    for (int r = 0; r < 4; ++r) {
+        const int rl = wr * 16 + fk + 4 * r, cl = wc * 16 + fr;
+        a[r] = -s_gather(Ppred, Dp, oa, I * NB + (rl >= cl ? rl : cl), I * NB + (rl >= cl ? cl : rl));
+    }
+    return a;
+}
+
+template <bool XL, bool ONE>
 __device__ __forceinline__ void sweep_chain_role(ChainLds& C, const double* __restrict__ G, double* F, double* Linv, int ld,
                                                  int CB, int* flags, const RlFlags& fl, int* info,
-                                                 double* feed, int lenient, int tid, int l, int w) {
+                                                 double* feed, int lenient, int tid, int l, int w, const OneArgs& oa,
+                                                 const void* Ppred, long Dp, int p32) {
     int* fdiag_all = flags + fl.fdiag;
     int* fnew_all = flags + fl.fnew;
     const int CBp = fl.CBp;
@@ -1969,22 +2071,36 @@
     if (XL && tid == 0) flag_st(flags + fl.fxcc, 1 + xcc_id());
     WaveWait ww{false};
     double smax = 0.0;
-    for (int e = tid; e < ld; e += 256) smax = fmax(smax, fabs(G[(long)e * ld + e]));
+    d4 accD;
+    if constexpr (ONE) {
+        for (int e = tid; e < ld; e += 256) {
+            const double v = p32 ? s_gather(static_cast<const float*>(Ppred), Dp, oa, e, e)
+                                 : s_gather(static_cast<const double*>(Ppred), Dp, oa, e, e);
+            C.sdall[e] = v;
+            if (e < NB) C.sd[0][e] = v;
+            smax = fmax(smax, fabs(v));
+        }
+        accD = p32 ? gather_s_diag(static_cast<const float*>(Ppred), Dp, oa, 0, wr, wc, fr, fk)
+                   : gather_s_diag(static_cast<const double*>(Ppred), Dp, oa, 0, wr, wc, fr, fk);
+    } else {
+        for (int e = tid; e < ld; e += 256) smax = fmax(smax, fabs(G[(long)e * ld + e]));
+        if (tid < NB) C.sd[0][tid] = G[(long)tid * ld + tid];
+    }
 #pragma unroll
     for (int o = 32; o > 0; o >>= 1) smax = fmax(smax, __shfl_xor(smax, o));
     if (l == 0) C.red[w] = smax;
-    if (tid < NB) C.sd[0][tid] = G[(long)tid * ld + tid];
     if (tid < 16) C.d4[0].flagA[tid] = 0, C.d4[1].flagA[tid] = 0;
     for (int e = tid; e < 16 * 16; e += 256) C.sLinv[(e >> 4) * TLD + 16 + (e & 15)] = 0.0;
     if (tid == 0) __builtin_amdgcn_fence(__ATOMIC_ACQUIRE, "agent");
     __syncthreads();
     smax = lenient ? __builtin_inf() : fmax(fmax(C.red[0], C.red[1]), fmax(C.red[2], C.red[3]));
     const double pivtol = pivot_tolerance(lenient);
-    d4 accD;
-#pragma unroll
-    for (int r = 0; r < 4; ++r) {
-        const int rl = wr * 16 + fk + 4 * r, cl = wc * 16 + fr;
-        accD[r] = -G[(long)(rl >= cl ? rl : cl) * ld + (rl >= cl ? cl : rl)];
+    if constexpr (!ONE) {
+#pragma unroll
+        for (int r = 0; r < 4; ++r) {
+            const int rl = wr * 16 + fk + 4 * r, cl = wc * 16 + fr;
+            accD[r] = -G[(long)(rl >= cl ? rl : cl) * ld + (rl >= cl ? cl : rl)];
+        }
     }
     for (int J = 0; J < CB; ++J) {
         Diag4Lds* dl = &C.d4[J & 1];
@@ -2017,7 +2133,8 @@
         if (w == 0 || w == 2) {
             wave_wait_ge(ffeed + J + 1, 1, fabort, ww);
             sc1_tile_to_lds((w == 2) ? C.sFeedD : C.sFeedS, rfeed, (unsigned)((2 * (J + 1) + (w == 2 ? 1 : 0)) * NB * NB * 8), l);
-            if (w == 2 && l < NB) C.sd[(J + 1) & 1][l] = G[(long)((J + 1) * NB + l) * ld + (J + 1) * NB + l];
+            if (w == 2 && l < NB)
+                C.sd[(J + 1) & 1][l] = ONE ? C.sdall[(J + 1) * NB + l] : G[(long)((J + 1) * NB + l) * ld + (J + 1) * NB + l];
         }
         __syncthreads();
         CHAIN_TRACE(J, 2);
@@ -2077,10 +2194,10 @@
     if (l == 0 && ww.dead) atomicMin(info, -2);
 }
 
-template <int N, bool FUSED, int MAXT, bool XL>
-__global__ __launch_bounds__(256) void k_sweep_rl(const double* __restrict__ G, double* F, double* Linv, int ld, int CB,
-                                                  int RT, int* flags, int* info_base, const int* __restrict__ ctr,
-                                                  DowndateArgs dd, double* feed, int lenient, int home) {
+template <int N, bool FUSED, int MAXT, bool XL, bool ONE>
+__device__ __forceinline__ void sweep_rl_body(const double* __restrict__ G, double* F, double* Linv, int ld, int CB,
+                                              int RT, int* flags, int* info_base, const int slot,
+                                              const DowndateArgs& dd, double* feed, int lenient, int home, const OneArgs& oa) {
     __shared__ __attribute__((aligned(16))) union {
         SweepLds L;
         ChainLds C;
@@ -2096,11 +2213,12 @@
     const int* fdiag = flags + fl.fdiag + (blockIdx.x % RL_REP) * fl.CBp;
     const int* fnew = flags + fl.fnew + (blockIdx.x % RL_REP) * fl.CBp;
     const int* fcol = flags + fl.fcol + (blockIdx.x % RL_REP) * fl.CBp;
-    int* info = info_base + (*ctr - 1);
+    int* info = info_base + slot;
     const int bx = XL ? (int)blockIdx.x - home : (int)blockIdx.x;
     if (bx < 0) return;
     if (bx == 0) {
-        sweep_chain_role<XL>(lds.C, G, F, Linv, ld, CB, flags, fl, info, feed, lenient, tid, l, w);
+        sweep_chain_role<XL, ONE>(lds.C, G, F, Linv, ld, CB, flags, fl, info, feed, lenient, tid, l, w, oa, dd.Ppred,
+                                  (long)N * dd.dp, dd.p32);
         return;
     }
     int I, part = 0;
@@ -2145,7 +2263,9 @@
             }
             __syncthreads();
             SWEEP_STAMP(0);
-            sweep_downdate_role<N, true>(L, dd, F, ld, CB, CB, frow, fabort, info, I - RT, tid, l, w, *ctr - 1);
+            sweep_downdate_role<N, true>(L, dd, F, ld, CB, CB, frow, fabort, info, I - RT, tid, l, w, slot,
+                                         ONE ? flags + fl.fgath + 32 * ((I - RT) % RL_REP) : nullptr,
+                                         RT - 2 * CB - 1 + nwsplit);
         }
         return;
     } else if (nwsplit > 0 && I >= CB && I < RT - CB - 1) {
@@ -2170,19 +2290,46 @@
     const int last = part == 1 ? hsplit - 1 : (chain ? I - 2 : CB - 1);
     const int ntiles = part == 1 ? hsplit : (chain ? I : CB);
     d4 n[MAXT];
-#pragma unroll
-    for (int t = 0; t < MAXT; ++t)
-        if (t0 + t < ntiles) {
-#pragma unroll
-            for (int r = 0; r < 4; ++r) n[t][r] = -G[(rowC + 4 * r) * ld + (long)(t0 + t) * NB + colC];
-        }
     d4 accD = {0, 0, 0, 0};
-    if (feeds) {
-#pragma unroll
-        for (int r = 0; r < 4; ++r) {
-            const int rl = wr * 16 + fk + 4 * r, cl = colC;
-            accD[r] = -G[((long)I * NB + (rl >= cl ? rl : cl)) * ld + (long)I * NB + (rl >= cl ? cl : rl)];
-        }
+    constexpr int ONE_EARLY = 4;
+    const long DpN = (long)N * dd.dp;
+    const bool gather = ONE && I < RT - CB - 1;
+    const bool gdefer = gather && chain && part != 2 && ntiles > ONE_EARLY;
+    auto gather_tiles = [&](int ulo, int uhi, bool with_d) {
+        if (chain) {
+            const int ip0 = I * NB + wr * 16 + fk;
+            if (dd.p32) gather_s_tiles<MAXT>(n, ulo, uhi, t0, ntiles, static_cast<const float*>(dd.Ppred), DpN, oa, ip0, colC);
+            else gather_s_tiles<MAXT>(n, ulo, uhi, t0, ntiles, static_cast<const double*>(dd.Ppred), DpN, oa, ip0, colC);
+            if (with_d && feeds)
+                accD = dd.p32 ? gather_s_diag(static_cast<const float*>(dd.Ppred), DpN, oa, I, wr, wc, fr, fk)
+                              : gather_s_diag(static_cast<const double*>(dd.Ppred), DpN, oa, I, wr, wc, fr, fk);
+        } else {
+            const long y0 = rowC - ld;
+            if (dd.p32) gather_w_tiles<MAXT>(n, ulo, uhi, t0, ntiles, static_cast<const float*>(dd.Ppred), DpN, oa, y0, colC);
+            else gather_w_tiles<MAXT>(n, ulo, uhi, t0, ntiles, static_cast<const double*>(dd.Ppred), DpN, oa, y0, colC);
+        }
+    };
+    if (gather) {
+        gather_tiles(0, gdefer ? ONE_EARLY : MAXT, !gdefer);
+    } else {
+#pragma unroll
+        for (int t = 0; t < MAXT; ++t)
+            if (t0 + t < ntiles) {
+#pragma unroll
+                for (int r = 0; r < 4; ++r) n[t][r] = -G[(rowC + 4 * r) * ld + (long)(t0 + t) * NB + colC];
+            }
+        if (feeds) {
+#pragma unroll
+            for (int r = 0; r < 4; ++r) {
+                const int rl = wr * 16 + fk + 4 * r, cl = colC;
+                accD[r] = -G[((long)I * NB + (rl >= cl ? rl : cl)) * ld + (long)I * NB + (rl >= cl ? cl : rl)];
+            }
+        }
+    }
+    if (gather && !chain) {
+        drain_vmem();
+        __syncthreads();
+        if (tid < RL_REP) __hip_atomic_fetch_add(flags + fl.fgath + 32 * tid, 1, __ATOMIC_RELAXED, __HIP_MEMORY_SCOPE_AGENT);
     }
     WaveWait ww{false};
     int known_diag = 0, known_new = 0, known_col = 0;
@@ -2310,6 +2457,7 @@
         const unsigned orgX = (unsigned)((((long)I * NB) * ld + (long)j * NB) * 8);
         if (llast) wt_rows_from_lds<2, 0>(rF, orgX, ld, sXj, 8 * w, l);
         else wt_rows_from_lds<2>(rF, orgX, ld, sXj, 8 * w, l);
+        if (gdefer && j == t0) gather_tiles(ONE_EARLY, MAXT, true);
         if (feeds) {
 #pragma unroll
             for (int s = 0; s < 8; ++s)
@@ -2429,12 +2577,63 @@
                 const long row0 = (I < zb ? (long)(I - CB) * NB : Dp + (long)(I - zb - 1) * NB) + 8 * w;
                 const double* W = F + (long)ld * ld;
                 SWEEP_STAMP(2);
-                vecops_rows8(dd.va, W, ld, Dp, row0, L.sd + 8 * w, l);
+                vecops_rows8<ONE>(dd.va, W, ld, Dp, row0, L.sd + 8 * w, l);
+            }
+            if constexpr (ONE) {
+                drain_vmem();
+                __syncthreads();
+                const int nrow = RT - CB + nwsplit;
+                if (tid == 0)
+                    L.seen[1] = __hip_atomic_fetch_add(oa.tickets, 1, __ATOMIC_RELAXED, __HIP_MEMORY_SCOPE_AGENT) == nrow - 1;
+                __syncthreads();
+                if (L.seen[1]) {
+                    __builtin_amdgcn_fence(__ATOMIC_ACQUIRE, "agent");
+                    if (tid == 0) __hip_atomic_store(oa.tickets, 0, __ATOMIC_RELAXED, __HIP_MEMORY_SCOPE_AGENT);
+                    const double* m = dd.va.mout;
+                    if (oa.means_base != nullptr)
+                        for (int j = tid; j < oa.d; j += 256) oa.means_base[(size_t)slot * oa.d + j] = oa.s0 * m[j];
+                    {
+                        double* sred = L.sd;
+                        double a[3] = {0.0, 0.0, 0.0};
+                        for (int i = tid; i < ld; i += 256)
+#pragma unroll
+                            for (int q = 0; q < 3; ++q) a[q] += dd.va.part[q * ld + i];
+#pragma unroll
+                        for (int q = 0; q < 3; ++q)
+#pragma unroll
+                            for (int o = 32; o > 0; o >>= 1) a[q] += __shfl_xor(a[q], o);
+                        if (l == 0)
+                            for (int q = 0; q < 3; ++q) sred[q * 4 + w] = a[q];
+                        __syncthreads();
+                        if (tid < 3) oa.rec_base[4 * (size_t)slot + tid] = sred[tid * 4] + sred[tid * 4 + 1] + sred[tid * 4 + 2] + sred[tid * 4 + 3];
+                    }
+                    predict_vectors<N>(&L.sS[0][0], tid, oa.c, dd.dp, m, oa.mpred, oa.shift, oa.G, oa.zbuf, oa.mm,
+                                       oa.flags_base + ((slot + 1) & 1) * oa.nflags, oa.nflags);
+                }
             }
         }
     }
     if (l == 0 && ww.dead) atomicMin(info, -2);
     SWEEP_STAMP(5);
+}
+
+template <int N, bool FUSED, int MAXT, bool XL, bool ONE = false>
+__global__ __launch_bounds__(256) void k_sweep_rl(const double* __restrict__ G, double* F, double* Linv, int ld, int CB,
+                                                  int RT, int* flags, int* info_base, const int* __restrict__ ctr,
+                                                  DowndateArgs dd, double* feed, int lenient, int home, OneArgs oa) {
+    if constexpr (ONE) {
+        const int slot = __builtin_amdgcn_readfirstlane(flag_ld(ctr)) - 1;
+        sweep_rl_body<N, FUSED, MAXT, XL, true>(G, F, Linv, ld, CB, RT, oa.flags_base + (slot & 1) * oa.nflags, info_base, slot, dd,
+                                                feed, lenient, home, oa);
+        __syncthreads();
+        if (threadIdx.x == 0 &&
+            __hip_atomic_fetch_add(oa.tickets + 1, 1, __ATOMIC_RELAXED, __HIP_MEMORY_SCOPE_AGENT) == (int)gridDim.x - 1) {
+            *oa.ctr = slot + 2;
+            __hip_atomic_store(oa.tickets + 1, 0, __ATOMIC_RELAXED, __HIP_MEMORY_SCOPE_AGENT);
+        }
+    } else {
+        sweep_rl_body<N, FUSED, MAXT, XL, false>(G, F, Linv, ld, CB, RT, flags, info_base, *ctr - 1, dd, feed, lenient, home, oa);
+    }
 }
 
 template <int N>
@@ -2928,6 +3127,10 @@
     }();
     return on != 0;
 }
+constexpr int ONE_MAX_CB = 9;
+inline bool one_loop(const pnmol_filter* f) {
+    return f->one_launch != 0 && fused_loop(f) && sweep_rl_enabled() && f->CB <= ONE_MAX_CB && f->ellw <= HW;
+}
 inline int sweep_xl_mode() {
     static const int mode = [] {
         const char* e = std::getenv("PNMOL_HIP_SWEEP_XL");
@@ -2940,19 +3143,27 @@
 template <int N, bool FUSED>
 void launch_sweep(unsigned grid, hipStream_t st, const double* G, double* F, double* Linv, int ld, int CB, int RT, int* flags,
                   int* info, const int* ctr, const DowndateArgs& dd, int* claim, double* hs, int lenient, int home,
-                  bool wskip = false) {
+                  bool wskip = false, const OneArgs* one = nullptr) {
     const bool xl = home >= 0;
     const unsigned rgrid = grid + (unsigned)w_split_count(RT, CB);
     unsigned xgrid = 8u * (unsigned)(CB - 1 + s_split_count(CB, true)) + 1u;
     for (unsigned left = rgrid - (unsigned)CB; left > 0; ++xgrid)
         if (xgrid % 8u != 0u) --left;
     xgrid += (unsigned)(xl ? home : 0);
+    const OneArgs none{};
+    if constexpr (FUSED) {
+        if (one != nullptr && sweep_rl_enabled() && CB <= ONE_MAX_CB) {
+            if (xl) k_sweep_rl<N, true, 9, true, true><<<xgrid, 256, 0, st>>>(G, F, Linv, ld, CB, RT, flags, info, ctr, dd, hs, lenient, home, *one);
+            else k_sweep_rl<N, true, 9, false, true><<<rgrid + 1, 256, 0, st>>>(G, F, Linv, ld, CB, RT, flags, info, ctr, dd, hs, lenient, home, *one);
+            return;
+        }
+    }
     if (sweep_rl_enabled() && CB <= 9) {
-        if (xl) k_sweep_rl<N, FUSED, 9, true><<<xgrid, 256, 0, st>>>(G, F, Linv, ld, CB, RT, flags, info, ctr, dd, hs, lenient, home);
-        else k_sweep_rl<N, FUSED, 9, false><<<rgrid + 1, 256, 0, st>>>(G, F, Linv, ld, CB, RT, flags, info, ctr, dd, hs, lenient, home);
+        if (xl) k_sweep_rl<N, FUSED, 9, true><<<xgrid, 256, 0, st>>>(G, F, Linv, ld, CB, RT, flags, info, ctr, dd, hs, lenient, home, none);
+        else k_sweep_rl<N, FUSED, 9, false><<<rgrid + 1, 256, 0, st>>>(G, F, Linv, ld, CB, RT, flags, info, ctr, dd, hs, lenient, home, none);
     } else if (sweep_rl_enabled() && CB <= 17) {
-        if (xl) k_sweep_rl<N, FUSED, 17, true><<<xgrid, 256, 0, st>>>(G, F, Linv, ld, CB, RT, flags, info, ctr, dd, hs, lenient, home);
-        else k_sweep_rl<N, FUSED, 17, false><<<rgrid + 1, 256, 0, st>>>(G, F, Linv, ld, CB, RT, flags, info, ctr, dd, hs, lenient, home);
+        if (xl) k_sweep_rl<N, FUSED, 17, true><<<xgrid, 256, 0, st>>>(G, F, Linv, ld, CB, RT, flags, info, ctr, dd, hs, lenient, home, none);
+        else k_sweep_rl<N, FUSED, 17, false><<<rgrid + 1, 256, 0, st>>>(G, F, Linv, ld, CB, RT, flags, info, ctr, dd, hs, lenient, home, none);
     }
     else
         k_sweep<N, FUSED><<<grid, 256, 0, st>>>(G, F, Linv, ld, CB, RT, flags, info, ctr, dd, claim, hs, lenient, wskip ? 1 : 0);
@@ -2983,7 +3194,8 @@
     if (kind != STEP_STEADY)
         k_predict<N><<<dim3(dp / 32, dp / 8 + 1), dim3(32, 8), sizeof(double) * Dp, st>>>(
         Pin, f->Ppred, f->Kg, c, dp, min, f->mpred, f->shift, f->G, f->zbuf, mm, f->ctr, f->flags, f->nflags, f->p32);
-    if (kind != STEP_STEADY) {
+    const bool one = kind != STEP_FULL && one_loop(f);
+    if (kind != STEP_STEADY && !one) {
         if (f->ellw > HW && f->sweep_mode != 0) {
             k_front<<<dim3((mp + 255) / 256, (unsigned)Dp), 256, 0, st>>>(f->Ppred, f->G, f->rdiag, f->Rdense, mm, Dp, f->p32);
             k_front_s<<<dim3((mp + 255) / 256, (unsigned)mp), 256, 0, st>>>(f->G, f->rdiag, f->Rdense, mm);
@@ -3002,12 +3214,29 @@
                     (nreal < 8 && short_last_panel()) ? nreal : 0};
     std::memcpy(dd.A1, f->iwp.A1, sizeof(dd.A1));
     std::memcpy(dd.Q1, f->iwp.Q1, sizeof(dd.Q1));
+    IwpConsts cn = f->iwp;
+    for (int a = 0; a < MAXN; ++a) cn.ts[a] = 1.0;
+    const double s0 = nordsieck_scale(f->nu, 0, dt);
+    OneArgs oa{};
+    if (one) {
+        dd.stds = record ? f->rec_stds : nullptr, dd.s0 = s0, dd.d = f->d;
+        oa = OneArgs{mm, f->rdiag, f->Rdense, cn, f->shift, f->G, f->zbuf, f->mpred, record ? f->rec_means : nullptr, f->rec, s0, f->d,
+                     f->tickets, f->ctr, f->flags, f->nflags};
+    }
     if (f->sweep_mode == 2) {
         const int t32 = dp / NB, pairs = t32 * (t32 + 1) / 2;
         dd.vrows = 0;
         if constexpr (N <= 3)
             launch_sweep<N, true>(f->RT + pairs, st, f->G, f->F, f->Linv, mp, f->CB, f->RT, f->flags, f->info, f->ctr, dd,
-                                  f->flags + f->RT + f->CB + 1, f->hs_scratch, f->p32 ? 2 : 0, f->xcd_home);
+                                  f->flags + f->RT + f->CB + 1, f->hs_scratch, f->p32 ? 2 : 0, f->xcd_home, false, one ? &oa : nullptr);
+        if (one) {
+            hipError_t e1 = hipGetLastError();
+            if (e1 != hipSuccess) {
+                ctx->err = std::string("kernel launch: ") + hipGetErrorString(e1);
+                return -2;
+            }
+            return 0;
+        }
     } else {
         if (f->sweep_mode == 1) {
             if (f->w_gemm) {
@@ -3041,8 +3270,6 @@
             k_downdate<N><<<dim3(tiles, tiles + vrows), 256, 0, st>>>(f->Ppred, W, Pout, varout, dp, mp, 0, mp / 8, va);
         }
     }
-    IwpConsts cn = f->iwp;
-    for (int a = 0; a < MAXN; ++a) cn.ts[a] = 1.0;
     RoleArgs ra{cn, dp, mout, f->mpred, f->shift, f->G, f->zbuf, mm, f->flags, f->nflags};
     const unsigned rblocks = (f->d + 255) / 256;
     if (kind == STEP_FULL)
@@ -3084,7 +3311,7 @@
     const bool have_sq = (f->Sqinv != nullptr && f->sq_dt == dt);
     for (auto& g : f->graphs)
         if (g.P0 == P0 && g.P1 == P1 && g.var == var && g.dt == dt && g.nsteps == nsteps && g.have_sq == have_sq &&
-            g.fused == fused_loop(f)) {
+            g.fused == fused_loop(f) && g.one == one_loop(f)) {
             *out = g.exec;
             return 0;
         }
@@ -3108,7 +3335,7 @@
         ctx->err = std::string("hipGraphInstantiate: ") + hipGetErrorString(e);
         return -2;
     }
-    f->graphs.push_back({P0, P1, var, dt, nsteps, have_sq, fused_loop(f), exec, false});
+    f->graphs.push_back({P0, P1, var, dt, nsteps, have_sq, fused_loop(f), one_loop(f), exec, false});
     *out = exec;
     return 0;
 }
@@ -3587,14 +3814,15 @@
     FCHK(hipMalloc(&f->sdiag, sizeof(double) * (mp + 1)));
     f->nflags = std::max({f->RT + f->CB + 1 + f->CB * f->CB, rl_flags(f->RT, f->CB).total,
                           rl_flags((int)(f->Dp / NB) + 1, (int)(f->Dp / NB) + 1).total});
-    FCHK(hipMalloc(&f->flags, sizeof(int) * f->nflags));
-    FCHK(hipMemset(f->flags, 0, sizeof(int) * f->nflags));
+    FCHK(hipMalloc(&f->flags, sizeof(int) * 2 * f->nflags));
+    FCHK(hipMemset(f->flags, 0, sizeof(int) * 2 * f->nflags));
     FCHK(hipMalloc(&f->hs_scratch, sizeof(double) * (size_t)std::max(f->CB * f->CB, 2 * f->CB + 2) * NB * NB));
     if (const char* e = std::getenv("PNMOL_HIP_FUSE_PREDICT")) f->fuse_predict = std::atoi(e);
+    if (const char* e = std::getenv("PNMOL_HIP_ONE_LAUNCH")) f->one_launch = std::atoi(e);
     FCHK(hipMalloc(&f->last_ctr, sizeof(int)));
     FCHK(hipMemset(f->last_ctr, 0, sizeof(int)));
-    FCHK(hipMalloc(&f->tickets, sizeof(int)));
-    FCHK(hipMemset(f->tickets, 0, sizeof(int)));
+    FCHK(hipMalloc(&f->tickets, sizeof(int) * 2));
+    FCHK(hipMemset(f->tickets, 0, sizeof(int) * 2));
     if (f->p32 && f->sweep_mode != 2 && !f->dd_big) {
         ctx->err = "pnmol_filter_create: dtype = fp32 covariance needs the fused sweep (num_derivatives <= 2, PNMOL_HIP_SWEEP unset)";
         return fail(-1);
@@ -3696,6 +3924,12 @@
     if (!f) return -1;
     if (kernel) *kernel = f->sweep_mode == 0 ? 0 : (sweep_rl_enabled() && f->CB <= 17 ? 2 : 1);
     if (xcd_home) *xcd_home = f->xcd_home;
+    return 0;
+}
+
+int pnmol_filter_loop_launches(const pnmol_filter* f, int* launches) {
+    if (!f || !launches) return -1;
+    *launches = !fused_loop(f) ? 0 : (one_loop(f) ? 1 : 2);
     return 0;
 }
 
@@ -4286,6 +4520,15 @@
     return 0;
 }
 
+int pnmol_filter_debug_poison_g(pnmol_filter* f) {
+    if (!f) return -1;
+    pnmol_ctx* ctx = f->ctx;
+    HIPCHK(ctx, hipSetDevice(ctx->device));
+    k_poison<<<1024, 256, 0, ctx->stream>>>(f->G, ((long)f->mp + f->Dp) * f->mp, nullptr, 0, nullptr, 0);
+    HIPCHK(ctx, hipGetLastError());
+    return 0;
+}
+
 int pnmol_filter_last_steps_ms(pnmol_filter* f, float* ms) {
     if (!f || !ms) return -1;
     *ms = f->last_ms;
diff --git a/pnmol-experiments_amd/csrc/pnmol_internal.hpp b/pnmol-experiments_amd/csrc/pnmol_internal.hpp
--- a/pnmol-experiments_amd/csrc/pnmol_internal.hpp
+++ b/pnmol-experiments_amd/csrc/pnmol_internal.hpp
@@ -70,6 +70,7 @@
     int* tickets = nullptr;
     int* last_ctr = nullptr;
     int fuse_predict = 1;
+    int one_launch = 1;
     int* flags = nullptr;
     int nflags = 0;
     double* hs_scratch = nullptr;
@@ -123,6 +124,7 @@
         int nsteps;
         bool have_sq;
         bool fused;
+        bool one;
         hipGraphExec_t exec;
         bool launched;
     };
diff --git a/pnmol-experiments_amd/pnmol/_hip.py b/pnmol-experiments_amd/pnmol/_hip.py
--- a/pnmol-experiments_amd/pnmol/_hip.py
+++ b/pnmol-experiments_amd/pnmol/_hip.py
@@ -110,6 +110,8 @@
     "pnmol_filter_prepare_error_model": (ctypes.c_int, [_vp, ctypes.c_double]),
     "pnmol_filter_debug_read": (ctypes.c_int, [_vp, ctypes.c_int, _c_double_p, ctypes.c_long]),
     "pnmol_filter_debug_poison": (ctypes.c_int, [_vp]),
+    "pnmol_filter_debug_poison_g": (ctypes.c_int, [_vp]),
+    "pnmol_filter_loop_launches": (ctypes.c_int, [_vp, ctypes.POINTER(ctypes.c_int)]),
     "pnmol_filter_dims": (ctypes.c_int, [_vp] + [ctypes.POINTER(ctypes.c_int)] * 5),
     "pnmol_filter_sweep_layout": (ctypes.c_int, [_vp] + [ctypes.POINTER(ctypes.c_int)] * 2),
     "pnmol_qr_r": (ctypes.c_int, [_vp, _c_double_p, ctypes.c_int, ctypes.c_int, _c_double_p]),
@@ -310,7 +312,10 @@
     def sweep_layout(self):
         k, x = ctypes.c_int(0), ctypes.c_int(0)
         self.lib.pnmol_filter_sweep_layout(self.handle, ctypes.byref(k), ctypes.byref(x))
-        return {"kernel": ("per_panel", "k_sweep", "k_sweep_rl")[k.value], "xcd_home": x.value}
+        n = ctypes.c_int(0)
+        self.lib.pnmol_filter_loop_launches(self.handle, ctypes.byref(n))
+        return {"kernel": ("per_panel", "k_sweep", "k_sweep_rl")[k.value], "xcd_home": x.value,
+                "loop": ("unfused", "one_launch", "two_launch")[n.value]}
 
     def dims(self):
         v = [ctypes.c_int(0) for _ in range(5)]
@@ -441,6 +446,9 @@
     def debug_poison(self):
         self.ctx.check(self.lib.pnmol_filter_debug_poison(self.handle), "pnmol_filter_debug_poison")
 
+    def debug_poison_g(self):
+        self.ctx.check(self.lib.pnmol_filter_debug_poison_g(self.handle), "pnmol_filter_debug_poison_g")
+
     def debug_read(self, which, count):
         out = np.empty(int(count))
         self.ctx.check(self.lib.pnmol_filter_debug_read(self.handle, int(which), _dp(out), int(count)),
```

Result: no change. 7979 steps/s, median of 2 (-0.2%).
